# TrevorS/qwen3-tts-rs

Hardware: AMD Instinct MI355X
Metric: acoustic_frames_per_sec (higher is better)
Workload: dtype bf16

## Files before the change

include/q3tts.h:

```cpp
#ifndef Q3TTS_H
#define Q3TTS_H

#include <stddef.h>
#include <stdint.h>

#ifdef __cplusplus
extern "C" {
#endif

#define Q3_ABI_VERSION 1
#define Q3_MAX_BATCH 64

typedef enum q3_status {
    Q3_OK = 0,
    Q3_INVALID_ARG = 1,
    Q3_IO = 2,
    Q3_MISSING_WEIGHT = 3,
    Q3_KV_OVERFLOW = 4,
    Q3_HIP_ERROR = 5,
    Q3_RCCL_ERROR = 6,
    Q3_UNSUPPORTED = 7,
    Q3_OOM = 8
} q3_status;

// ... 141 lines not shown
q3_status q3_session_open_text(q3_session* s, int b);
q3_status q3_session_append_text(q3_session* s, int b, const uint32_t* ids, int n, int last);
q3_status q3_session_text_state(q3_session* s, int b, int* n_text, int* frames_committed, int* frames_runnable, int* closed,
                                int* frames_replayed);

enum {
    Q3_GET_PREFILL_EMBEDS = 0,
    Q3_GET_LAST_HIDDEN = 1,
    Q3_GET_LOGITS = 2,
    Q3_GET_TRAILING = 3,
    Q3_GET_PAD_EMBED = 4,
    Q3_GET_LOGITS_HIST = 5,
    Q3_GET_CP_LOGITS = 6,
    Q3_GET_TOKEN = 7,
    Q3_GET_CP_LOGITS_HIST = 8
};
q3_status q3_session_set_kv_dtype(q3_session* s, int dtype);
q3_status q3_session_set_debug(q3_session* s, int capture_logits);
q3_status q3_session_prefill_len(q3_session* s, int b, int* prefill_len, int* trailing_len);
q3_status q3_session_get(q3_session* s, int what, int b, void* out_host, size_t bytes);
q3_status q3_talker_step(q3_session* s, const float* embeds_host, float* hidden_host, float* logits_host);
q3_status q3_cp_generate(q3_session* s, const float* last_hidden_host, const float* sem_embed_host,
                         uint32_t* codes15_host, float* cp_logits_host );
q3_status q3_frame_embed(q3_model* m, uint32_t sem_token, const uint32_t* codes15, const float* text_add_host,
                         float* out_host);
q3_status q3_sample(int device, const float* logits_host, const uint8_t* seen_host, const float* u_host,
                    int rows, int vocab, const q3_options* opts, int token_count, uint32_t* tokens_host);
void      q3_rng_seed(uint64_t seed, uint64_t* state);
float     q3_rng_next(uint64_t* state);
q3_status q3_fused_residual_rmsnorm(int device, int dtype, const void* x_host, const void* res_host,
                                    const void* w_host, int rows, int cols, float eps,
                                    void* normed_host, void* sum_host);
q3_status q3_linear(int device, const float* x_host, const uint16_t* w_bf16_host, const float* bias_host,
                    int M, int N, int K, float* y_host);
typedef struct q3_linear_ex_args {
    int M, N, K, ldx, ldy, ldr, M_alloc;
    int epi, tiled, ksplit, use_ws, zero_n, zero_guard;
    float eps;
    const float* x; const uint16_t* w; const uint16_t* w2;
    const float* bias; const float* norm_w; const float* resid;
    float* y; float* zero_buf;
} q3_linear_ex_args;
q3_status q3_linear_ex(int device, const q3_linear_ex_args* args);
typedef struct q3_attn_step_args {
    int variant, B, nh, nkv, n_splits, max_seq;
    float eps; int reserved;
    const int* pos; const float* qkv; const float* q_norm_w; const float* k_norm_w;
    const float* rope_cos; const float* rope_sin;
    float* kcache; float* vcache; float* out;
} q3_attn_step_args;
q3_status q3_attn_step(int device, const q3_attn_step_args* args);
typedef struct q3_attn_step_ex_args {
    int variant, layout, B, nh, nkv, n_splits, max_seq, rows_per_seq;
    int n_layers, layer, n_slabs, kv_row_pages;
    int qkv_S, qkv_K, g_vocab, g_proj_dim, g_ldx, g_max_frames, g_code_slot, zero_n, zero_guard;
    float eps, qkv_eps; int reserved;
    const int* pos; const float* qkv; const float* q_norm_w; const float* k_norm_w;
    const float* rope_cos; const float* rope_sin;
    float* kcache; float* vcache; float* out;
    const int* page_slots; int* rot_used; long long* stray;
    const float* qkv_part; const float* qkv_ssq;
    const float* g_logits; const uint32_t* g_tok; const float* g_qkv_tab; const float* g_proj_tab;
    float* g_x; uint32_t* g_codes; const int* g_frame_idx;
    float* zero_buf;
} q3_attn_step_ex_args;
q3_status q3_attn_step_ex(int device, const q3_attn_step_ex_args* args);
q3_status q3_kv_pages_to_bf16_ex(int device, int n_layers, int nkv, int n_pages, const int* src_slots, const int* dst_slots,
                                 const float* src, uint16_t* dst, int* rot_used, long long* stray);
int         q3_conv_path(int cout, int cin, int L, int k, int dil, int phases, int packed, int has_resid, int planes, int aligned16);
int         q3_resunit_path(int C, int L, int dil, int packed, int ya_is_xa, int planes);
const char* q3_conv_path_name(int code);
typedef struct q3_conv_ex_args {
    int kind, cin, cout, L, k, dil, stride;
    int act, planes, packed, resid_in_place, snake_raw, y2_is_x;
    int y_front, y_elems;
    int* path;
    const float* x; const float* w; const float* b;
    const float* snake_a; const float* snake_b; const float* resid; const float* scale;
    const float* post_a; const float* post_ib;
    const float* w2; const float* b2; const float* mid_a; const float* mid_ib;
    float* y; float* y2;
} q3_conv_ex_args;
q3_status q3_conv_ex(int device, const q3_conv_ex_args* args);
int q3_gemm_path(int M, int N, int K, int epi, int norm, int w2, int planes, int* path);
typedef struct q3_gemm_ex_args {
    int M, N, K, ldx, ldy, ldr, M_alloc;
    int epi, geometry, k_split, sup_m, sup_n;
    float eps;
    int* path;
    const float* x; const uint16_t* w; const uint16_t* w2;
    const float* bias; const float* norm_w; const float* resid;
    float* y;
} q3_gemm_ex_args;
q3_status q3_gemm_ex(int device, const q3_gemm_ex_args* args);
int q3_attn_prefill_path(int nh, int nkv, int use_planes, int halves, int* path);
typedef struct q3_attn_prefill_ex_args {
    int n_seq, rps, base_pos, nh, nkv, max_seq, ld_qkv, ld_out;
    int kernel, halves, use_planes;
    float eps;
    int* path;
    const float* qkv; const float* q_norm_w; const float* k_norm_w;
    const float* rope_cos; const float* rope_sin;
    float* kcache; float* vcache; float* out;
} q3_attn_prefill_ex_args;
q3_status q3_attn_prefill_ex(int device, const q3_attn_prefill_ex_args* args);
int q3_attn_c_path(int hd, int kernel);
typedef struct q3_attn_c_ex_args {
    int mode, nh, hd, L, kernel, window;
    int N, n_rows, layers, layer, cap, n_blocks, n_tabs;
    float scale;
    const float* q; const float* k; const float* v;
    const int* rows; const float* caches;
    const int* tabs; const int* tab0; const int* tab_n;
    float* o;
} q3_attn_c_ex_args;
q3_status q3_attn_c_ex(int device, const q3_attn_c_ex_args* args);
q3_status q3_rope_c_ex(int device, float* q, float* k, const float* cs, const float* sn, const int* pos, int nh, int hd, int L, int n_pos);
q3_status q3_copy_cols_ex(int device, const float* src, size_t src_elems, float* dst, size_t dst_elems, int n, int C, const long long* s_off,
                          const long long* d_off, const int* sp, const int* dp, size_t src_off, size_t dst_off);
q3_status q3_copy_segs_ex(int device, const float* src, size_t src_elems, float* dst, size_t dst_elems, int n_segs, const unsigned long long* segs);
q3_status q3_gather_frames_ex(int device, const uint32_t* src, size_t src_elems, const long long* s_off, int n, uint32_t* dst, size_t dst_elems);
q3_status q3_rvq_embed_ex(int device, const uint32_t* frames, int n_frames, const float* first_cb, const float* rest_cbs, int cb_dim, int cb_size,
                          float* first_out, float* rest_out, int out_front, int out_elems);
q3_status q3_silu_mul_ex(int device, const float* g, const float* u, float* y, long long n, long long y_elems);
typedef struct q3_sample_rec {
    float inv_temp; int apply_temp, greedy;
    int top_k; float top_p; int use_top_p;
    float rep_pen, rep_inv; int use_rep;
    int eos_id, min_new_tokens, pad;
} q3_sample_rec;
q3_status q3_sample_row(const q3_options* opts, q3_sample_rec* out);
typedef struct q3_sample_ex_args {
    int B, vocab, ld, u_stride, u_elems, advance, token_count_static, hist_stride_b, hist_cap, codec_eos, use_suppress, guard;
    q3_sample_rec scalar;
    const float* logits; const float* u; const int* draw_idx; const q3_sample_rec* rows;
    const int* limit; const int* text_ready;
    uint32_t* tok; uint8_t* seen; int* token_count; int* frame_idx; int* pos; float* logits_hist;
} q3_sample_ex_args;
q3_status q3_sample_ex(int device, const q3_sample_ex_args* args);
typedef struct q3_frame_embed_ex_args {
    int B, H, n_sem, cp_vocab, max_frames, n_text_rows, guard, reserved;
    const uint16_t* codec_emb; const uint16_t* cp_embs; const uint32_t* tok; const float* cp_logits_last;
    const int* frame_idx; const float* text_rows; const int* trail_base; const int* trail_len; const int* pad_row; const int* text_ready;
    uint32_t* codes; float* out;
} q3_frame_embed_ex_args;
q3_status q3_frame_embed_ex(int device, const q3_frame_embed_ex_args* args);
typedef struct q3_cp_gather_ex_args {
    int pass, B, H, n_sem, cp_vocab, max_frames, proj_dim, qkv_dim, ld_out, ld_qkv_out, guard, reserved;
    const float* last_hidden; const uint16_t* codec_emb; const uint32_t* tok; const uint16_t* cp_emb; const float* cp_logits;
    const float* proj_tab; const float* qkv_tab; const int* frame_idx;
    uint32_t* codes; float* out; float* qkv_out;
} q3_cp_gather_ex_args;
q3_status q3_cp_gather_ex(int device, const q3_cp_gather_ex_args* args);
q3_status q3_rmsnorm_ex(int device, const float* x, long long x_elems, long long x_off, int ldx, const float* w, float* y, long long y_elems,
                        long long y_front, int ldy, int rows, int cols, float eps, const int* frame_idx, const int* text_ready);
q3_status q3_norm_c(int device, int layernorm, const float* x, const float* w, const float* b, int C, int L, float eps,
                    float* y, int y_front, int y_elems);
q3_status q3_dwconv7(int device, const float* x, const float* w, const float* b, int C, int L, float* y, int y_front, int y_elems);
q3_status q3_row_move(int device, void* src_host, size_t src_bytes, void* dst_host, size_t dst_bytes, int n_segs, const size_t* src_off,
                      const size_t* dst_off, const size_t* seg_bytes, const int* mode);
enum { Q3_DEC_QUANT = 0, Q3_DEC_PRECONV = 1, Q3_DEC_PRETRANS = 2, Q3_DEC_UP0 = 3, Q3_DEC_UP1 = 4,
       Q3_DEC_INIT = 5, Q3_DEC_BLK0 = 6, Q3_DEC_BLK1 = 7, Q3_DEC_BLK2 = 8, Q3_DEC_BLK3 = 9, Q3_DEC_N = 10 };
q3_status q3_decode_codes(q3_model* m, const uint32_t* frames_host, int n_frames, float* pcm_host,
                          float** taps_host);
typedef struct q3_codec_stream q3_codec_stream;
q3_status q3_codec_stream_create(q3_model* m, int rows, int max_frames, q3_codec_stream** out);
// ... 187 lines not shown
```

qwen3_tts_rs_amd/_lib.py:

```python
import ctypes
import os

from .config import CConfig

_HERE = os.path.dirname(os.path.abspath(__file__))
LIB_PATH = os.environ.get("Q3TTS_LIB") or os.path.join(_HERE, "libq3tts.so")

if not os.path.exists(LIB_PATH):
    raise ImportError(
        f"{LIB_PATH} not found: the gfx950 HIP library is not built. Run "
        "`python -c 'import __graft_entry__ as g; g.build()'` (or qwen3_tts_rs_amd/csrc/build.sh).")

lib = ctypes.CDLL(LIB_PATH)


class COptions(ctypes.Structure):
    _fields_ = [
        ("temperature", ctypes.c_double), ("top_p", ctypes.c_double), ("repetition_penalty", ctypes.c_double),
        ("seed", ctypes.c_uint64), ("max_length", ctypes.c_int32), ("top_k", ctypes.c_int32),
        ("eos_token_id", ctypes.c_int32), ("chunk_frames", ctypes.c_int32), ("min_new_tokens", ctypes.c_int32),
        ("has_seed", ctypes.c_int32),
    ]


# ... 170 lines not shown
    "q3_pcm_stage_tempo_lags": (c_int, [c_void_p, c_int, P(ctypes.c_int64), c_void_p, ctypes.c_size_t, P(ctypes.c_size_t)]),
    "q3_session_set_tempo": (c_int, [c_void_p, c_int, c_int]),
    "q3_batcher_ticket_tempo": (c_int, [c_void_p, ctypes.c_int64, c_int]),
    "q3_pcm_stage_set_pitch": (c_int, [c_void_p, c_int, c_int]),
    "q3_pcm_stage_pitch_plan": (c_int, [c_int, c_int, P(c_int), P(ctypes.c_double)]),
    "q3_pcm_stage_pitch_tables": (c_int, [c_void_p, ctypes.c_size_t, c_void_p, ctypes.c_size_t, P(c_int), P(c_int)]),
    "q3_pcm_stage_pitch_count": (c_int, [c_int, c_int, ctypes.c_size_t, c_int, P(ctypes.c_size_t)]),
    "q3_pcm_stage_bound_pitch": (c_int, [ctypes.c_uint32, c_int, c_int, c_int, ctypes.c_size_t, P(ctypes.c_size_t)]),
    "q3_session_set_pitch": (c_int, [c_void_p, c_int, c_int]),
    "q3_batcher_ticket_pitch": (c_int, [c_void_p, ctypes.c_int64, c_int]),
    "q3_pcm_stage_set_silence": (c_int, [c_void_p, c_int, c_int, c_int, c_int]),
    "q3_pcm_stage_silence": (c_int, [c_void_p, c_int] + [P(ctypes.c_int64)] * 5),
    "q3_pcm_stage_silence_hold": (c_int, [c_int, c_int, P(ctypes.c_size_t)]),
    "q3_pcm_stage_bound_silence": (c_int, [ctypes.c_uint32, c_int, c_int, c_int, c_int, c_int, ctypes.c_size_t, P(ctypes.c_size_t)]),
    "q3_silence_trim": (c_int, [c_void_p, ctypes.c_size_t, c_int, c_int, c_int, c_void_p, ctypes.c_size_t, P(ctypes.c_size_t), P(ctypes.c_int64)]),
    "q3_session_set_silence": (c_int, [c_void_p, c_int, c_int, c_int, c_int]),
    "q3_session_silence": (c_int, [c_void_p, c_int] + [P(ctypes.c_int64)] * 5),
    "q3_batcher_ticket_silence": (c_int, [c_void_p, ctypes.c_int64, c_int, c_int, c_int]),
    "q3_batcher_ticket_silence_read": (c_int, [c_void_p, ctypes.c_int64] + [P(ctypes.c_int64)] * 5),
    "q3_pcm_stage_set_level": (c_int, [c_void_p, c_int, c_int, c_int]),
    "q3_pcm_stage_level_coeffs": (c_int, [c_int, c_int, P(ctypes.c_float), P(ctypes.c_float)]),
    "q3_pcm_stage_level_count": (c_int, [ctypes.c_size_t, c_int, P(ctypes.c_size_t)]),
    "q3_pcm_stage_bound_level": (c_int, [ctypes.c_uint32, c_int, ctypes.c_size_t, P(ctypes.c_size_t)]),
    "q3_session_set_level": (c_int, [c_void_p, c_int, c_int, c_int]),
    "q3_batcher_ticket_level": (c_int, [c_void_p, ctypes.c_int64, c_int, c_int]),
    "q3_loudness_kweight": (c_int, [ctypes.c_uint32, P(ctypes.c_double), P(ctypes.c_double)]),
    "q3_pcm_stage_loudness_consts": (c_int, [c_int, c_int, P(ctypes.c_float), P(ctypes.c_float), P(ctypes.c_float), P(ctypes.c_float), P(ctypes.c_float)]),
    "q3_pcm_stage_set_loudness": (c_int, [c_void_p, c_int, c_int, c_int, c_int]),
    "q3_pcm_stage_loudness": (c_int, [c_void_p, c_int, P(ctypes.c_float), P(ctypes.c_float), P(c_int), P(c_int)]),
    "q3_pcm_stage_loudness_blocks": (c_int, [c_void_p, c_int, c_void_p, ctypes.c_size_t, P(ctypes.c_size_t)]),
    "q3_session_set_loudness": (c_int, [c_void_p, c_int, c_int, c_int, c_int]),
    "q3_session_loudness": (c_int, [c_void_p, c_int, P(ctypes.c_float), P(ctypes.c_float), P(c_int), P(c_int)]),
    "q3_batcher_ticket_loudness": (c_int, [c_void_p, ctypes.c_int64, c_int, c_int, c_int]),
    "q3_batcher_ticket_loudness_read": (c_int, [c_void_p, ctypes.c_int64, P(ctypes.c_float), P(ctypes.c_float), P(c_int), P(c_int)]),
    "q3_codec_stream_push_out": (c_int, [c_void_p, c_int, P(c_int), P(c_void_p), P(c_int), c_void_p, P(c_int), P(c_int), P(c_void_p),
                                         P(ctypes.c_size_t), P(ctypes.c_size_t)]),
    "q3_session_set_output": (c_int, [c_void_p, ctypes.c_uint32, c_int]),
    "q3_session_next_chunks_out": (c_int, [c_void_p, P(c_void_p), P(ctypes.c_size_t), P(ctypes.c_size_t), P(c_int)]),
    "q3_batcher_ticket_output": (c_int, [c_void_p, ctypes.c_int64, ctypes.c_uint32, c_int]),
    "q3_batcher_read_out": (c_int, [c_void_p, ctypes.c_int64, c_void_p, ctypes.c_size_t, P(ctypes.c_size_t), P(c_int)]),
    "q3_session_replace": (c_int, [c_void_p, c_int, c_void_p]),
    "q3_session_park_row": (c_int, [c_void_p, c_int, P(c_void_p)]),
    "q3_session_resume_row": (c_int, [c_void_p, c_int, c_void_p]),
    "q3_parked_free": (None, [c_void_p]),
    "q3_parked_info": (c_int, [c_void_p, P(c_int), P(c_int), P(c_int), P(c_int), P(ctypes.c_size_t)]),
    "q3_row_move": (c_int, [c_int, c_void_p, ctypes.c_size_t, c_void_p, ctypes.c_size_t, c_int, P(ctypes.c_size_t), P(ctypes.c_size_t),
                            P(ctypes.c_size_t), P(c_int)]),
    "q3_batcher_create": (c_int, [c_void_p, c_int, c_int, c_int, P(c_void_p)]),
    "q3_batcher_free": (None, [c_void_p]),
    "q3_batcher_submit": (c_int, [c_void_p, c_void_p, c_int, P(ctypes.c_int64)]),
    "q3_batcher_submit_streamed": (c_int, [c_void_p, c_void_p, P(ctypes.c_int64)]),
    "q3_batcher_read": (c_int, [c_void_p, ctypes.c_int64, c_void_p, ctypes.c_size_t, P(ctypes.c_size_t), P(c_int)]),
    "q3_batcher_stream_info": (c_int, [c_void_p, P(c_int), P(ctypes.c_size_t), P(c_int), P(c_int), P(c_int)]),
    "q3_batcher_submit_open": (c_int, [c_void_p, c_void_p, c_int, P(ctypes.c_int64)]),
    "q3_batcher_append_text": (c_int, [c_void_p, ctypes.c_int64, c_void_p, c_int, c_int]),
    "q3_batcher_text_state": (c_int, [c_void_p, ctypes.c_int64, P(c_int), P(c_int), P(c_int), P(c_int)]),
    "q3_batcher_cancel": (c_int, [c_void_p, ctypes.c_int64]),
    "q3_batcher_set_parking": (c_int, [c_void_p, c_int, c_int, c_int]),
    "q3_batcher_park": (c_int, [c_void_p, ctypes.c_int64]),
    "q3_batcher_unpark": (c_int, [c_void_p, ctypes.c_int64]),
    "q3_batcher_park_info": (c_int, [c_void_p, P(c_int), P(c_int), P(ctypes.c_longlong), P(ctypes.c_longlong), P(ctypes.c_longlong), P(c_int)]),
    "q3_batcher_step": (c_int, [c_void_p, c_int, c_int, P(c_int), P(c_int), P(c_int)]),
    "q3_batcher_poll": (c_int, [c_void_p, ctypes.c_int64, P(c_int), P(c_int), P(ctypes.c_size_t)]),
    "q3_batcher_fetch": (c_int, [c_void_p, ctypes.c_int64, c_void_p, c_int, c_void_p, ctypes.c_size_t]),
    "q3_session_set_debug": (c_int, [c_void_p, c_int]),
    "q3_session_prefill_len": (c_int, [c_void_p, c_int, P(c_int), P(c_int)]),
    "q3_session_get": (c_int, [c_void_p, c_int, c_int, c_void_p, ctypes.c_size_t]),
    "q3_talker_step": (c_int, [c_void_p, c_void_p, c_void_p, c_void_p]),
    "q3_cp_generate": (c_int, [c_void_p, c_void_p, c_void_p, c_void_p, c_void_p]),
    "q3_frame_embed": (c_int, [c_void_p, ctypes.c_uint32, c_void_p, c_void_p, c_void_p]),
    "q3_sample": (c_int, [c_int, c_void_p, c_void_p, c_void_p, c_int, c_int, P(COptions), c_int, c_void_p]),
    "q3_rng_seed": (None, [ctypes.c_uint64, P(ctypes.c_uint64)]),
    "q3_rng_next": (ctypes.c_float, [P(ctypes.c_uint64)]),
    "q3_fused_residual_rmsnorm": (c_int, [c_int, c_int, c_void_p, c_void_p, c_void_p, c_int, c_int, ctypes.c_float, c_void_p, c_void_p]),
    "q3_linear": (c_int, [c_int, c_void_p, c_void_p, c_void_p, c_int, c_int, c_int, c_void_p]),
    "q3_linear_ex": (c_int, [c_int, P(CLinearEx)]),
    "q3_attn_step": (c_int, [c_int, P(CAttnStep)]),
    "q3_attn_step_ex": (c_int, [c_int, P(CAttnStepEx)]),
    "q3_kv_pages_to_bf16_ex": (c_int, [c_int] * 4 + [c_void_p] * 6),
    "q3_conv_path": (c_int, [c_int] * 10),
    "q3_resunit_path": (c_int, [c_int] * 6),
    "q3_conv_path_name": (c_char_p, [c_int]),
    "q3_conv_ex": (c_int, [c_int, P(CConvEx)]),
    "q3_gemm_path": (c_int, [c_int] * 7 + [P(ctypes.c_int32)]),
    "q3_gemm_ex": (c_int, [c_int, P(CGemmEx)]),
    "q3_attn_prefill_path": (c_int, [c_int] * 4 + [P(ctypes.c_int32)]),
    "q3_attn_prefill_ex": (c_int, [c_int, P(CAttnPrefillEx)]),
    "q3_attn_c_path": (c_int, [c_int, c_int]),
    "q3_attn_c_ex": (c_int, [c_int, P(CAttnCEx)]),
    "q3_rope_c_ex": (c_int, [c_int, c_void_p, c_void_p, c_void_p, c_void_p, c_void_p, c_int, c_int, c_int, c_int]),
    "q3_copy_cols_ex": (c_int, [c_int, c_void_p, ctypes.c_size_t, c_void_p, ctypes.c_size_t, c_int, c_int, c_void_p, c_void_p, c_void_p, c_void_p,
                                ctypes.c_size_t, ctypes.c_size_t]),
    "q3_copy_segs_ex": (c_int, [c_int, c_void_p, ctypes.c_size_t, c_void_p, ctypes.c_size_t, c_int, c_void_p]),
    "q3_gather_frames_ex": (c_int, [c_int, c_void_p, ctypes.c_size_t, c_void_p, c_int, c_void_p, ctypes.c_size_t]),
    "q3_rvq_embed_ex": (c_int, [c_int, c_void_p, c_int, c_void_p, c_void_p, c_int, c_int, c_void_p, c_void_p, c_int, c_int]),
    "q3_silu_mul_ex": (c_int, [c_int, c_void_p, c_void_p, c_void_p, ctypes.c_longlong, ctypes.c_longlong]),
    "q3_sample_row": (c_int, [P(COptions), P(CSampleRow)]),
    "q3_sample_ex": (c_int, [c_int, P(CSampleEx)]),
    "q3_frame_embed_ex": (c_int, [c_int, P(CFrameEmbedEx)]),
    "q3_cp_gather_ex": (c_int, [c_int, P(CCpGatherEx)]),
    "q3_rmsnorm_ex": (c_int, [c_int, c_void_p, ctypes.c_longlong, ctypes.c_longlong, c_int, c_void_p, c_void_p, ctypes.c_longlong,
                              ctypes.c_longlong, c_int, c_int, c_int, ctypes.c_float, c_void_p, c_void_p]),
    "q3_norm_c": (c_int, [c_int, c_int, c_void_p, c_void_p, c_void_p, c_int, c_int, ctypes.c_float, c_void_p, c_int, c_int]),
    "q3_dwconv7": (c_int, [c_int, c_void_p, c_void_p, c_void_p, c_int, c_int, c_void_p, c_int, c_int]),
    "q3_decode_codes": (c_int, [c_void_p, c_void_p, c_int, c_void_p, P(c_void_p)]),
    "q3_codes_to_tensor": (None, [c_void_p, c_int, c_void_p]),
    "q3_session_set_profile": (c_int, [c_void_p, c_int]),
    "q3_session_profile_read": (c_int, [c_void_p, P(ctypes.c_double), P(ctypes.c_double), P(ctypes.c_long), c_int]),
    "q3_session_profile_shapes": (c_int, [c_void_p, P(c_int), c_int, P(c_int), c_int]),
    "q3_bench_linear": (c_int, [c_int] * 9 + [P(ctypes.c_double)]),
    "q3_session_stream": (c_int, [c_void_p, P(c_void_p)]),
    "q3_session_frame_bytes": (c_int, [c_void_p, c_int, P(ctypes.c_double), P(ctypes.c_double)]),
    "q3_session_submit_info": (c_int, [c_void_p, P(c_int), P(c_int)]),
    "q3_session_submit_fences": (c_int, [c_void_p, P(c_int), P(c_int)]),
    "q3_session_set_stream_mode": (c_int, [c_void_p, c_int]),
    "q3_session_open_text": (c_int, [c_void_p, c_int]),
    "q3_session_append_text": (c_int, [c_void_p, c_int, c_void_p, c_int, c_int]),
    "q3_session_text_state": (c_int, [c_void_p, c_int, P(c_int), P(c_int), P(c_int), P(c_int), P(c_int)]),
    "q3_model_config": (c_int, [c_void_p, P(CConfig)]),
    "q3_config_default": (c_int, [c_int, P(CConfig)]),
    "q3_config_from_json": (c_int, [c_char_p, P(CConfig), P(c_int)]),
    "q3_model_load": (c_int, [c_char_p, c_int, P(c_void_p), P(c_int)]),
    "q3_model_load_safetensors": (c_int, [c_void_p, c_char_p, P(c_int)]),
    "q3_safetensors_info": (c_int, [c_char_p, c_char_p, P(c_int), P(ctypes.c_int64), c_int, P(c_int)]),
    "q3_pcm16_from_f32": (c_int, [c_void_p, ctypes.c_int64, c_void_p]),
    "q3_wav_write_pcm16": (c_int, [c_char_p, c_void_p, ctypes.c_int64, ctypes.c_uint32]),
    "q3_g711_from_pcm16": (c_int, [c_void_p, ctypes.c_int64, c_int, c_void_p]),
    "q3_wav_write_g711": (c_int, [c_char_p, c_void_p, ctypes.c_int64, ctypes.c_uint32, c_int]),
    "q3_wav_read": (c_int, [c_char_p, c_void_p, ctypes.c_int64, P(ctypes.c_int64), P(ctypes.c_uint32)]),
    "q3_codes_write_bin": (c_int, [c_char_p, c_void_p, c_int, c_int]),
    "q3_codes_read_bin": (c_int, [c_char_p, c_void_p, c_int, c_int, P(c_int)]),
    "q3_audio_write_bin": (c_int, [c_char_p, c_void_p, ctypes.c_int64]),
    "q3_audio_read_bin": (c_int, [c_char_p, c_void_p, ctypes.c_int64, P(ctypes.c_int64)]),
    "q3_resample": (c_int, [c_void_p, ctypes.c_int64, ctypes.c_uint32, ctypes.c_uint32, c_void_p, ctypes.c_int64, P(ctypes.c_int64)]),
    "q3_dp_unique_id": (c_int, [c_void_p]),
    "q3_dp_init": (c_int, [c_int, c_int, c_void_p, c_int, P(c_void_p)]),
    "q3_dp_free": (None, [c_void_p]),
    "q3_dp_info": (c_int, [c_void_p, P(c_int), P(c_int)]),
    "q3_dp_broadcast_weights": (c_int, [c_void_p, c_void_p, c_int]),
    "q3_dp_allgather_f64": (c_int, [c_void_p, c_void_p, c_int, c_void_p]),
    "q3_spk_config_default": (c_int, [P(CSpkConfig)]),
    "q3_spk_config_from_json": (c_int, [c_char_p, P(CSpkConfig), P(c_int)]),
    "q3_spk_create": (c_int, [P(CSpkConfig), c_int, P(c_void_p)]),
    "q3_spk_free": (None, [c_void_p]),
    "q3_spk_get_config": (c_int, [c_void_p, P(CSpkConfig)]),
    "q3_spk_n_tensors": (c_int, [c_void_p]),
    "q3_spk_tensor_info": (c_int, [c_void_p, c_int, P(c_char_p), P(ctypes.c_int64)]),
    "q3_spk_set_tensor": (c_int, [c_void_p, c_char_p, c_void_p, c_int, ctypes.c_int64]),
    "q3_spk_finalize": (c_int, [c_void_p]),
    "q3_spk_load_safetensors": (c_int, [c_void_p, c_char_p]),
    "q3_spk_mel_frames": (c_int, [ctypes.c_int64]),
    "q3_spk_mel": (c_int, [c_void_p, c_void_p, ctypes.c_int64, c_void_p, ctypes.c_int64, P(c_int)]),
    "q3_spk_forward": (c_int, [c_void_p, c_void_p, c_int, c_void_p, P(c_void_p)]),
    "q3_spk_encode": (c_int, [c_void_p, c_void_p, ctypes.c_int64, ctypes.c_uint32, c_void_p]),
    "q3_mimi_config_default": (c_int, [P(CMimiConfig)]),
    "q3_mimi_create": (c_int, [P(CMimiConfig), c_int, P(c_void_p)]),
    "q3_mimi_free": (None, [c_void_p]),
    "q3_mimi_get_config": (c_int, [c_void_p, P(CMimiConfig)]),
    "q3_mimi_n_tensors": (c_int, [c_void_p]),
    "q3_mimi_tensor_info": (c_int, [c_void_p, c_int, P(c_char_p), P(ctypes.c_int64)]),
    "q3_mimi_set_tensor": (c_int, [c_void_p, c_char_p, c_void_p, c_int, ctypes.c_int64]),
    "q3_mimi_finalize": (c_int, [c_void_p]),
    "q3_mimi_load_safetensors": (c_int, [c_void_p, c_char_p]),
    "q3_mimi_frames": (c_int, [P(CMimiConfig), ctypes.c_int64]),
    "q3_mimi_encode": (c_int, [c_void_p, c_void_p, ctypes.c_int64, ctypes.c_uint32, c_void_p, c_int, P(c_int), P(c_void_p)]),
    "q3_wav_info": (c_int, [c_char_p, P(CWavDesc)]),
# ... 29 lines not shown
```

qwen3_tts_rs_amd/api.py:

```python
import ctypes
import enum
from dataclasses import dataclass
from typing import List, NamedTuple, Optional, Sequence, Tuple

import numpy as np

from . import _lib
from ._lib import lib, check, COptions, CRequest, CTiming
from .config import Q3Config
from . import synth

MAX_BATCH = 64
CODEC_EOS_TOKEN_ID = 2150
SAMPLES_PER_FRAME = 1920


class Language(enum.Enum):
    Chinese = 2055
    English = 2050
    Japanese = 2058
    Korean = 2064
    German = 2053
    French = 2061
    Russian = 2069
# ... 804 lines not shown
    def attach_speech_encoder(self, enc):
        self.speech_encoder = enc

    def has_speech_encoder(self) -> bool:
        return self.speech_encoder is not None

    def create_voice_clone_prompt(self, ref_audio: "AudioBuffer", ref_text_ids=None, ref_codes=None):
        from .speaker import VoiceClonePrompt
        if self.speaker_encoder is None:
            hint = {ModelType.CustomVoice: " CustomVoice models use preset speakers (synthesize_with_voice), not voice cloning. "
                                           "Use a Base model for voice cloning.",
                    ModelType.VoiceDesign: " VoiceDesign models use text-described voices, not voice cloning. "
                                           "Use a Base model for voice cloning."}.get(
                self.model_type, " Ensure model weights contain `speaker_encoder.*` keys (only Base models include a speaker encoder).")
            raise _lib.Q3Error(3, "Speaker encoder not available." + hint)
        if isinstance(ref_audio, RefAudio):
            emb = self.speaker_encoder.encode_ref(ref_audio)
            if ref_text_ids is None:
                return VoiceClonePrompt(emb)
            if ref_codes is None:
                if self.speech_encoder is None:
                    raise _lib.Q3Error(7, "ICL voice cloning requires a speech encoder, but it was not loaded. Ensure the speech tokenizer "
                                          "weights contain encoder keys, or use x_vector_only mode by passing ref_text=None.")
                ref_codes = self.speech_encoder.encode_ref(ref_audio)
            return VoiceClonePrompt(emb, np.ascontiguousarray(ref_codes, dtype=np.uint32), np.asarray(ref_text_ids, dtype=np.uint32))
        if ref_audio.sample_rate != 24000:
            ref_audio = resample_to_24k(ref_audio)
        emb = self.speaker_encoder.encode(ref_audio.samples, ref_audio.sample_rate)
        if ref_text_ids is None:
            return VoiceClonePrompt(emb)
        if ref_codes is None:
            if self.speech_encoder is None:
                raise _lib.Q3Error(7, "ICL voice cloning requires a speech encoder, but it was not loaded. Ensure the speech tokenizer "
                                      "weights contain encoder keys, or use x_vector_only mode by passing ref_text=None.")
            ref_codes = self.speech_encoder.encode(ref_audio.samples, ref_audio.sample_rate)
        return VoiceClonePrompt(emb, np.ascontiguousarray(ref_codes, dtype=np.uint32), np.asarray(ref_text_ids, dtype=np.uint32))

    def synthesize_voice_clone_prompt(self, text_ids, prompt, language: "Language", options=None):
        return self.synthesize_voice_clone(text_ids, prompt.speaker_embedding, language, options,
                                           ref_codes=prompt.ref_codes, ref_text_ids=prompt.ref_text_ids)

    def supports_preset_speakers(self) -> bool:
        return self.model_type in (None, ModelType.CustomVoice)

    def supports_voice_design(self) -> bool:
        return self.model_type == ModelType.VoiceDesign

    def close(self):
        if getattr(self, "_h", None):
            lib.q3_model_free(self._h); self._h = None

    __del__ = close

    def set_tensor(self, name: str, arr: np.ndarray, dtype: int):
        a = np.ascontiguousarray(arr)
        check(lib.q3_model_set_tensor(self._h, name.encode(), dtype, a.ctypes.data_as(ctypes.c_void_p), a.size))

    def finalize(self):
        check(lib.q3_model_finalize(self._h))

    @classmethod
    def from_synthetic(cls, config: Q3Config, device: int = 0, seed: int = synth.DEFAULT_SEED, sink=None) -> "Qwen3TTS":
        m = cls(config, device)
        for name, arr, dt in synth.synthetic_checkpoint(config, m._h, seed):
            m.set_tensor(name, arr, dt)
            if sink is not None:
                sink(name, arr, dt)
        m.finalize()
        return m

    @classmethod
    def from_tensors(cls, config: Q3Config, tensors, device: int = 0) -> "Qwen3TTS":
        m = cls(config, device)
        for name, (arr, dt) in tensors.items():
            m.set_tensor(name, arr, dt)
        m.finalize()
        return m

    def kv_pool_limit(self, max_pages: int):
        check(lib.q3_model_kv_pool_limit(self._h, int(max_pages)))

    def set_codec_planes(self, planes: int):
        check(lib.q3_model_set_codec_planes(self._h, int(planes)))

    def kv_pool_trim(self) -> int:
        n = ctypes.c_size_t()
        check(lib.q3_model_kv_pool_trim(self._h, ctypes.byref(n)))
        return n.value

    def kv_pool_info(self) -> dict:
        pp = ctypes.c_int(); pb = ctypes.c_size_t(); tot = ctypes.c_int(); use = ctypes.c_int(); peak = ctypes.c_int()
        check(lib.q3_model_kv_pool_info(self._h, ctypes.byref(pp), ctypes.byref(pb), ctypes.byref(tot), ctypes.byref(use), ctypes.byref(peak)))
        return {"page_positions": pp.value, "page_bytes": pb.value, "pages_total": tot.value, "pages_in_use": use.value, "pages_peak": peak.value}

    def prefix_cache(self, max_pages: int):
        check(lib.q3_model_prefix_cache(self._h, int(max_pages)))

    def prefix_cache_info(self) -> dict:
        mx = ctypes.c_int(); n = ctypes.c_int(); sh = ctypes.c_int()
        lk = ctypes.c_longlong(); hp = ctypes.c_longlong(); ev = ctypes.c_longlong()
        check(lib.q3_model_prefix_cache_info(self._h, ctypes.byref(mx), ctypes.byref(n), ctypes.byref(sh), ctypes.byref(lk), ctypes.byref(hp), ctypes.byref(ev)))
        return {"max_pages": mx.value, "pages_cached": n.value, "pages_shared": sh.value, "lookups": lk.value,
                "hit_positions": hp.value, "evictions": ev.value}

    def arena(self) -> Tuple[int, int]:
        p = ctypes.c_void_p(); n = ctypes.c_size_t()
        check(lib.q3_model_arena(self._h, ctypes.byref(p), ctypes.byref(n)))
        return p.value, n.value

    def mark_loaded(self):
        check(lib.q3_model_mark_loaded(self._h))

    def session(self, utts: Sequence[Utterance], options: Optional[SynthesisOptions] = None, debug: bool = False, kv_bf16: bool = False) -> Session:
        return Session(self, utts, options or SynthesisOptions(), debug, kv_bf16=kv_bf16)

    def synthesize(self, text_ids: Sequence[int], options: Optional[SynthesisOptions] = None) -> AudioBuffer:
        return self.synthesize_with_voice(text_ids, Speaker.Ryan, Language.English, options)

    def synthesize_with_voice(self, text_ids, speaker: Speaker, language: Language, options=None) -> AudioBuffer:
        audio, _ = self.synthesize_with_timing(text_ids, speaker, language, options)
        return audio

    def synthesize_with_timing(self, text_ids, speaker: Speaker, language: Language, options=None):
        s = self.session([Utterance(text_ids, speaker, language)], options)
        try:
            audio, timing = s.run()
        finally:
            s.close()
        return audio[0], timing

    def synthesize_voice_design(self, text_ids, instruct_ids, language: Language, options=None) -> AudioBuffer:
        s = self.session([Utterance(text_ids, language=language, instruct_ids=instruct_ids)], options)
        try:
            audio, _ = s.run()
        finally:
            s.close()
        return audio[0]

    def synthesize_voice_clone(self, text_ids, xvector, language: Language, options=None, ref_codes=None, ref_text_ids=None):
        s = self.session([Utterance(text_ids, language=language, xvector=xvector, ref_codes=ref_codes, ref_text_ids=ref_text_ids)], options)
        try:
            s.prefill(); s.generate(max(s._row_limit))
            return AudioBuffer(s.decode(0)), s.codes(0)
        finally:
            s.close()

    @staticmethod
    def prefill_shape(u: "Utterance") -> Tuple[int, int, int, int]:
        icl = u.ref_codes is not None and u.ref_text_ids is not None
        n_ins = len(u.instruct_ids) if u.instruct_ids is not None else 0
        n_icl = (len(np.asarray(u.ref_codes).reshape(-1, 16)) + 1) if icl else 0
        return (u.mode(), n_ins, 1 if (len(u.text_ids) > 0 and not icl) else 0, n_icl)

    def synthesize_batch(self, utts: Sequence[Utterance], options=None):
        audio: List[Optional[AudioBuffer]] = [None] * len(utts)
        tot = SynthesisTiming(0.0, 0.0, 0, 0.0)
        for k in range(0, len(utts), MAX_BATCH):
            part = list(range(k, min(k + MAX_BATCH, len(utts))))
            s = self.session([utts[i] for i in part], options)
            try:
                a, t = s.run()
            finally:
                s.close()
            for j, i in enumerate(part):
                audio[i] = a[j]
            tot = SynthesisTiming(tot.prefill_ms + t.prefill_ms, tot.generation_ms + t.generation_ms,
# ... 916 lines not shown
        rr = np.ascontiguousarray(rows, dtype=np.int32); assert rr.ndim == 2 and rr.shape[1] == 3
        cc = np.ascontiguousarray(caches, dtype=np.float32); assert cc.ndim == 5 and cc.shape[2] == 2 and cc.shape[3] == nh * hd
        a.N, a.n_rows, a.layers, a.cap = qq.shape[1], rr.shape[0], cc.shape[1], cc.shape[4]
        keep += [rr, cc]; a.rows, a.caches = _vp(rr), _vp(cc)
        if mode == 2:
            tt = np.ascontiguousarray(tabs, dtype=np.int32); t0 = np.ascontiguousarray(tab0, dtype=np.int32); tn = np.ascontiguousarray(tab_n, dtype=np.int32)
            assert tt.ndim == 1 and t0.shape == (rr.shape[0],) and tn.shape == t0.shape
            a.n_blocks, a.n_tabs = cc.shape[0], tt.size
            keep += [tt, t0, tn]; a.tabs, a.tab0, a.tab_n = _vp(tt), _vp(t0), _vp(tn)
        else:
            assert cc.shape[0] == rr.shape[0]
    check(lib.q3_attn_c_ex(device, ctypes.byref(a)))
    return o


def rope_c_ex(q_: np.ndarray, k: np.ndarray, cs: np.ndarray, sn: np.ndarray, nh: int, pos=None, device: int = 0):
    qq = np.array(q_, dtype=np.float32, order="C"); kk = np.array(k, dtype=np.float32, order="C")
    cs = np.ascontiguousarray(cs, dtype=np.float32); sn = np.ascontiguousarray(sn, dtype=np.float32)
    assert qq.ndim == 2 and kk.shape == qq.shape and qq.shape[0] % nh == 0 and cs.ndim == 2 and sn.shape == cs.shape
    hd = qq.shape[0] // nh; assert cs.shape[1] * 2 == hd
    pp = None if pos is None else np.ascontiguousarray(pos, dtype=np.int32)
    assert pp is None or pp.shape == (qq.shape[1],)
    check(lib.q3_rope_c_ex(device, _vp(qq), _vp(kk), _vp(cs), _vp(sn), _vp(pp), nh, hd, qq.shape[1], cs.shape[0]))
    return qq, kk


def copy_cols_ex(src: np.ndarray, dst: np.ndarray, C: int, s_off, d_off, sp, dp, src_off: int = 0, dst_off: int = 0, device: int = 0) -> np.ndarray:
    src = np.ascontiguousarray(src, dtype=np.float32)
    assert dst.dtype == np.float32 and dst.flags.c_contiguous and dst.ndim == 1 and src.ndim == 1
    so = np.ascontiguousarray(s_off, dtype=np.int64); do = np.ascontiguousarray(d_off, dtype=np.int64)
    spp = np.ascontiguousarray(sp, dtype=np.int32); dpp = np.ascontiguousarray(dp, dtype=np.int32)
    n = so.size; assert do.shape == (n,) and spp.shape == (n,) and dpp.shape == (n,)
    check(lib.q3_copy_cols_ex(device, _vp(src), src.size, _vp(dst), dst.size, n, C, _vp(so), _vp(do), _vp(spp), _vp(dpp), src_off, dst_off))
    return dst


def copy_segs_ex(src: np.ndarray, dst: np.ndarray, segs, device: int = 0) -> np.ndarray:
    src = np.ascontiguousarray(src, dtype=np.float32)
    assert dst.dtype == np.float32 and dst.flags.c_contiguous and dst.ndim == 1 and src.ndim == 1
    sg = np.ascontiguousarray(segs, dtype=np.uint64); assert sg.ndim == 2 and sg.shape[1] == 3
    check(lib.q3_copy_segs_ex(device, _vp(src), src.size, _vp(dst), dst.size, sg.shape[0], _vp(sg)))
    return dst


def gather_frames_ex(src: np.ndarray, s_off, dst: np.ndarray, device: int = 0) -> np.ndarray:
    src = np.ascontiguousarray(src, dtype=np.uint32)
    assert dst.dtype == np.uint32 and dst.flags.c_contiguous and dst.ndim == 1 and src.ndim == 1
    so = np.ascontiguousarray(s_off, dtype=np.int64); assert so.ndim == 1
    check(lib.q3_gather_frames_ex(device, _vp(src), src.size, _vp(so), so.size, _vp(dst), dst.size))
    return dst


def rvq_embed_ex(frames: np.ndarray, first_cb: np.ndarray, rest_cbs: np.ndarray, first_out: np.ndarray, rest_out: np.ndarray, out_front: int = 0,
                 device: int = 0):
    fr = np.ascontiguousarray(frames, dtype=np.uint32); assert fr.ndim == 2 and fr.shape[1] == 16
    fc = np.ascontiguousarray(first_cb, dtype=np.float32); rc = np.ascontiguousarray(rest_cbs, dtype=np.float32)
    assert fc.ndim == 2 and rc.shape == (15,) + fc.shape
    for buf in (first_out, rest_out):
        assert buf.dtype == np.float32 and buf.flags.c_contiguous and buf.ndim == 1 and buf.size == first_out.size
    check(lib.q3_rvq_embed_ex(device, _vp(fr), fr.shape[0], _vp(fc), _vp(rc), fc.shape[1], fc.shape[0], _vp(first_out), _vp(rest_out), out_front,
                              first_out.size))
    return first_out, rest_out


def silu_mul_ex(g: np.ndarray, u: np.ndarray, y: np.ndarray, device: int = 0) -> np.ndarray:
    g = np.ascontiguousarray(g, dtype=np.float32); u = np.ascontiguousarray(u, dtype=np.float32)
    assert g.ndim == 1 and u.shape == g.shape and y.dtype == np.float32 and y.flags.c_contiguous and y.ndim == 1
    check(lib.q3_silu_mul_ex(device, _vp(g), _vp(u), _vp(y), g.size, y.size))
    return y


def resunit_path(C: int, L: int, dil: int, packed: bool = True, ya_is_xa: bool = False, planes: int = 3) -> int:
    return lib.q3_resunit_path(C, L, dil, int(packed), int(ya_is_xa), planes)


def conv_path_name(code: int) -> str:
    return lib.q3_conv_path_name(code).decode()


def conv_ex(kind: int, x: np.ndarray, w: np.ndarray, *, dil: int = 1, stride: int = 1, b: Optional[np.ndarray] = None, snake=None,
            post=None, mid=None, resid: Optional[np.ndarray] = None, resid_in_place: bool = False, scale: Optional[np.ndarray] = None,
            act: int = 0, planes: int = 3, packed: bool = True, snake_raw: bool = False, w2: Optional[np.ndarray] = None,
            b2: Optional[np.ndarray] = None, y: Optional[np.ndarray] = None, y2: Optional[np.ndarray] = None, y_front: int = 0,
            y2_is_x: bool = False, device: int = 0):
    f = lambda a: np.ascontiguousarray(a, dtype=np.float32)
    x = f(x); w = f(w)
    assert x.ndim == 2 and w.ndim == 3
    cin, L = x.shape
    cout = w.shape[1] if kind == 1 else w.shape[0]
    assert (w.shape[0] if kind == 1 else w.shape[1]) == cin
    a = _lib.CConvEx()
    a.kind, a.cin, a.cout, a.L, a.k, a.dil, a.stride = kind, cin, cout, L, w.shape[2], dil, stride
    a.act, a.planes, a.packed, a.resid_in_place, a.snake_raw, a.y2_is_x = act, planes, int(packed), int(resid_in_place), int(snake_raw), int(y2_is_x)
    n_out = cout * L * (stride if kind == 1 else 1)
    if y is None:
        y = np.zeros(n_out, dtype=np.float32); y_front = 0
    for buf in (y, y2):
        assert buf is None or (buf.dtype == np.float32 and buf.flags.c_contiguous and buf.ndim == 1 and buf.size == y.size)
    a.y_front, a.y_elems = y_front, y.size
    path = ctypes.c_int32(0)
    a.path = ctypes.pointer(path)
    keep = [x, w]
    ptr = lambda arr: arr.ctypes.data_as(ctypes.c_void_p)
    a.x, a.w, a.y = ptr(x), ptr(w), ptr(y)
    if y2 is not None:
        a.y2 = ptr(y2)

    def opt(name, arr, n):
        if arr is not None:
            arr = f(arr); assert arr.size == n, (name, arr.size, n)
            keep.append(arr); setattr(a, name, ptr(arr))
    opt("b", b, cout); opt("b2", b2, cout); opt("scale", scale, cout); opt("resid", resid, n_out)
    if w2 is not None:
        opt("w2", w2, cout * cin)
    for (na, nb, pr, n) in (("snake_a", "snake_b", snake, cin), ("post_a", "post_ib", post, cout), ("mid_a", "mid_ib", mid, cout)):
        if pr is not None:
            opt(na, pr[0], n); opt(nb, pr[1], n)
    try:
        check(lib.q3_conv_ex(device, ctypes.byref(a)))
    except _lib.Q3Error as e:
        e.path = path.value
        raise
    return y, y2, path.value


def norm_c(x: np.ndarray, w: np.ndarray, b: Optional[np.ndarray] = None, eps: float = 1e-6, y: Optional[np.ndarray] = None,
           y_front: int = 0, device: int = 0) -> np.ndarray:
    x = np.ascontiguousarray(x, dtype=np.float32); C, L = x.shape
    w = np.ascontiguousarray(w, dtype=np.float32); assert w.shape == (C,)
    bb = None if b is None else np.ascontiguousarray(b, dtype=np.float32)
    if y is None:
        y = np.zeros(C * L, dtype=np.float32); y_front = 0
    assert y.dtype == np.float32 and y.flags.c_contiguous and y.ndim == 1
    ptr = lambda arr: arr.ctypes.data_as(ctypes.c_void_p)
    check(lib.q3_norm_c(device, 0 if bb is None else 1, ptr(x), ptr(w), None if bb is None else ptr(bb), C, L, eps, ptr(y), y_front, y.size))
    return y


def dwconv7(x: np.ndarray, w: np.ndarray, b: np.ndarray, y: Optional[np.ndarray] = None, y_front: int = 0, device: int = 0) -> np.ndarray:
    x = np.ascontiguousarray(x, dtype=np.float32); C, L = x.shape
    w = np.ascontiguousarray(w, dtype=np.float32); b = np.ascontiguousarray(b, dtype=np.float32)
    assert w.shape == (C, 7) and b.shape == (C,)
    if y is None:
        y = np.zeros(C * L, dtype=np.float32); y_front = 0
    assert y.dtype == np.float32 and y.flags.c_contiguous and y.ndim == 1
    ptr = lambda arr: arr.ctypes.data_as(ctypes.c_void_p)
    check(lib.q3_dwconv7(device, ptr(x), ptr(w), ptr(b), C, L, ptr(y), y_front, y.size))
    return y


def _io(arr, dtype, n, name):
    assert isinstance(arr, np.ndarray) and arr.dtype == dtype and arr.flags.c_contiguous and arr.ndim == 1 and arr.size == n, (name, n)
    return _vp(arr)


def sample_row(options: SynthesisOptions) -> "_lib.CSampleRow":
    r = _lib.CSampleRow(); o = options.to_c()
    check(lib.q3_sample_row(ctypes.byref(o), ctypes.byref(r)))
    return r


def sample_ex(logits: np.ndarray, u: np.ndarray, vocab: int, tok: np.ndarray, scalar, *, rows=None, seen: Optional[np.ndarray] = None,
              u_stride: int = 1, draw_idx=None, token_count: Optional[np.ndarray] = None, token_count_static: int = 0, advance: bool = False,
              frame_idx: Optional[np.ndarray] = None, pos: Optional[np.ndarray] = None, limit=None, text_ready=None,
              logits_hist: Optional[np.ndarray] = None, hist_stride_b: int = 0, hist_cap: int = 0, codec_eos: int = 2150,
              use_suppress: bool = True, guard: int = 0, device: int = 0) -> np.ndarray:
    lg = np.ascontiguousarray(logits, dtype=np.float32); assert lg.ndim == 2
    B, ld = lg.shape
    uu = np.ascontiguousarray(u, dtype=np.float32).reshape(-1)
    a = _lib.CSampleEx()
    a.B, a.vocab, a.ld, a.u_stride, a.u_elems, a.advance, a.token_count_static = B, vocab, ld, u_stride, uu.size, int(advance), token_count_static
    a.hist_stride_b, a.hist_cap, a.codec_eos, a.use_suppress, a.guard = hist_stride_b, hist_cap, codec_eos, int(use_suppress), guard
    a.scalar = scalar
    keep = [lg, uu]
    a.logits, a.u = _vp(lg), _vp(uu)
    a.tok = _io(tok, np.uint32, B + 2 * guard, "tok")
    if seen is not None:
        a.seen = _io(seen, np.uint8, B * vocab + 2 * guard, "seen")
    for name, arr in (("token_count", token_count), ("frame_idx", frame_idx), ("pos", pos)):
        if arr is not None:
            setattr(a, name, _io(arr, np.int32, B + 2 * guard, name))
    if logits_hist is not None:
        a.logits_hist = _io(logits_hist, np.float32, B * hist_stride_b + 2 * guard, "logits_hist")
    for name, arr in (("draw_idx", draw_idx), ("limit", limit), ("text_ready", text_ready)):
        if arr is not None:
            v = np.ascontiguousarray(arr, dtype=np.int32); assert v.shape == (B,), name
            keep.append(v); setattr(a, name, _vp(v))
    if rows is not None:
        assert len(rows) == B
        rr = (_lib.CSampleRow * B)(*rows); keep.append(rr)
        a.rows = ctypes.cast(rr, ctypes.c_void_p)
    check(lib.q3_sample_ex(device, ctypes.byref(a)))
    return tok


def frame_embed_ex(codec_emb: np.ndarray, cp_embs: np.ndarray, tok, cp_logits_last: np.ndarray, codes: np.ndarray, frame_idx, max_frames: int,
                   text_rows: np.ndarray, trail_base, trail_len, pad_row, out: np.ndarray, text_ready=None, guard: int = 0, device: int = 0):
    ce = np.ascontiguousarray(codec_emb, dtype=np.uint16); pe = np.ascontiguousarray(cp_embs, dtype=np.uint16)
    lg = np.ascontiguousarray(cp_logits_last, dtype=np.float32); tx = np.ascontiguousarray(text_rows, dtype=np.float32)
    assert ce.ndim == 2 and pe.ndim == 3 and pe.shape[0] == 15 and pe.shape[2] == ce.shape[1] and lg.ndim == 2 and lg.shape[1] == pe.shape[1]
    assert tx.ndim == 2 and tx.shape[1] == ce.shape[1]
    B, H = lg.shape[0], ce.shape[1]
# ... 98 lines not shown
```

qwen3_tts_rs_amd/csrc/q3_codec_run.hip:

```cpp
#include "q3_engine.h"

namespace {
struct DevCache {
    std::mutex mu;
    std::unordered_multimap<uint64_t, void*> free_blocks;
    std::unordered_map<void*, uint64_t> live;
    size_t cached = 0, cap = 0;
    DevCache() { const char* e = getenv("Q3_DEV_CACHE_MB"); cap = (size_t)(e ? atol(e) : 32768) << 20; }
    static uint64_t key(int dev, size_t bytes) { return ((uint64_t)dev << 48) | (uint64_t)bytes; }
    static size_t size_class(size_t bytes) {
        if (bytes <= 4096) return (bytes + 255) & ~(size_t)255;
        size_t p2 = 1; while ((p2 << 1) <= bytes) p2 <<= 1;
        const size_t step = p2 >> 4;
        return (bytes + step - 1) / step * step;
    }
    hipError_t get(void** p, size_t bytes) {
        bytes = size_class(bytes);
        int dev = 0; (void)hipGetDevice(&dev);
        const uint64_t k = key(dev, bytes);
        {
            std::lock_guard<std::mutex> g(mu);
            auto it = free_blocks.find(k);
            if (it != free_blocks.end()) { *p = it->second; free_blocks.erase(it); cached -= bytes; live[*p] = k; return hipSuccess; }
        }
        hipError_t e = hipMalloc(p, bytes);
        if (e != hipSuccess) {
            trim(0);
            e = hipMalloc(p, bytes);
            if (e != hipSuccess) return e;
        }
        std::lock_guard<std::mutex> g(mu);
        live[*p] = k;
        return hipSuccess;
    }
    void put(void* p) {
        if (!p) return;
        uint64_t k = 0; bool known = false;
        {
            std::lock_guard<std::mutex> g(mu);
            auto it = live.find(p);
            if (it != live.end()) { k = it->second; known = true; live.erase(it); }
            const size_t bytes = (size_t)(k & 0xffffffffffffull);
            if (known && cap && cached + bytes <= cap) { free_blocks.emplace(k, p); cached += bytes; return; }
        }
        (void)hipFree(p);
    }
    void trim(size_t keep) {
        std::vector<void*> drop;
        {
            std::lock_guard<std::mutex> g(mu);
            for (auto it = free_blocks.begin(); it != free_blocks.end() && cached > keep;) {
                cached -= (size_t)(it->first & 0xffffffffffffull); drop.push_back(it->second); it = free_blocks.erase(it);
            }
        }
        for (void* p : drop) (void)hipFree(p);
    }
};
DevCache& dev_cache() { static DevCache* c = new DevCache(); return *c; }
}
hipError_t dev_malloc(void** p, size_t bytes) { return dev_cache().get(p, bytes ? bytes : 4); }
void dev_free(void* p) { dev_cache().put(p); }

q3_status codec_reserve(const q3_model* m, CodecWS& ws, int T, int Tf) {
    if (Tf < T) Tf = T;
    if (T <= ws.cap_frames && Tf <= ws.cap_front) return Q3_OK;
    if (T < ws.cap_frames) T = ws.cap_frames;
    if (Tf < ws.cap_front) Tf = ws.cap_front;
    if (ws.bufA) HIPC(q3_hipDeviceSynchronize());
    ws.release();
    const q3_config& c = m->cfg;
    int up = 1; for (int i = 0; i < 2; ++i) up *= c.dec_up_ratios[i];
    size_t per = (size_t)4 * c.dec_latent * up;
    { size_t L = up; int C = c.dec_dim; per = per > (size_t)C * L ? per : (size_t)C * L;
      for (int b = 0; b < 4; ++b) { L *= c.dec_up_rates[b]; C /= 2; if ((size_t)C * L > per) per = (size_t)C * L; } }
    const int QDm = c.dec_heads * c.dec_head_dim;
    size_t per_front = (size_t)4 * QDm;
    if ((size_t)2 * c.dec_inter > per_front) per_front = (size_t)2 * c.dec_inter;
    if ((size_t)2 * c.dec_cb_dim > per_front) per_front = (size_t)2 * c.dec_cb_dim;
    if ((size_t)c.dec_latent > per_front) per_front = (size_t)c.dec_latent;
    if ((size_t)c.dec_q_dim > per_front) per_front = (size_t)c.dec_q_dim;
    size_t n = per * (size_t)T;
    if (per_front * (size_t)Tf > n) n = per_front * (size_t)Tf;
    HIPC(dev_malloc((void**)&ws.bufA, n * 4)); HIPC(dev_malloc((void**)&ws.bufB, n * 4)); HIPC(dev_malloc((void**)&ws.bufC, n * 4));
    HIPC(dev_malloc((void**)&ws.bufF, n * 4));
    const size_t small = (size_t)Tf * (size_t)(QDm > c.dec_latent ? QDm : c.dec_latent);
    HIPC(dev_malloc((void**)&ws.bufD, small * 4)); HIPC(dev_malloc((void**)&ws.bufE, small * 4));
    HIPC(dev_malloc((void**)&ws.cs, (size_t)Tf * 32 * 4)); HIPC(dev_malloc((void**)&ws.sn, (size_t)Tf * 32 * 4));
    HIPC(dev_malloc((void**)&ws.frames, (size_t)Tf * 16 * 4));
    size_t total_up = up; for (int b = 0; b < 4; ++b) total_up *= c.dec_up_rates[b];
    HIPC(dev_malloc((void**)&ws.pcm, (size_t)T * total_up * 4));
    Q3C(codec_rope_table(c, Tf, ws.cs, ws.sn));
    ws.cap_frames = T; ws.cap_front = Tf;
    return Q3_OK;
}
q3_status codec_rope_table(const q3_config& c, int n, float* cs_dev, float* sn_dev) {
    std::vector<float> cs((size_t)n * 32), sn((size_t)n * 32);
    for (int i = 0; i < 32; ++i) {
        const float inv = 1.0f / powf(c.dec_theta, (float)(2 * i) / (float)c.dec_head_dim);
        for (int t = 0; t < n; ++t) { const float f = (float)t * inv; cs[(size_t)t * 32 + i] = cosf(f); sn[(size_t)t * 32 + i] = sinf(f); }
    }
    HIPC(q3_hipMemcpy(cs_dev, cs.data(), cs.size() * 4, hipMemcpyHostToDevice));
    HIPC(q3_hipMemcpy(sn_dev, sn.data(), sn.size() * 4, hipMemcpyHostToDevice));
    return Q3_OK;
}

int samples_per_frame(const q3_config& c) {
    int u = 1; for (int i = 0; i < 2; ++i) u *= c.dec_up_ratios[i]; for (int i = 0; i < 4; ++i) u *= c.dec_up_rates[i];
    return u;
}

static thread_local const q3_model* tl_codec_model = nullptr;
static const void* packed_of(const float* w) { return tl_codec_model ? tl_codec_model->pk(w) : nullptr; }
static thread_local int tl_codec_planes = 3;
CodecScope::CodecScope(const q3_model* m) {
    static const int env_planes = [] { const char* e = getenv("Q3_CODEC_PLANES"); const int v = e ? atoi(e) : 0; return (v == 2 || v == 3) ? v : 0; }();
    planes = env_planes ? env_planes : m->codec_planes;
    tl_codec_model = m; tl_codec_planes = planes;
}
CodecScope::~CodecScope() { tl_codec_planes = 3; }
static hipError_t conv1(const float* x, const float* w, const float* b, float* y, int cin, int cout, int L, hipStream_t st,
                        const float* resid = nullptr, const float* scale = nullptr, int act = 0,
                        const float* sa = nullptr, const float* sib = nullptr) {
    ConvArgs a; a.x = x; a.w = w; a.b = b; a.y = y; a.cin = cin; a.cout = cout; a.L = L; a.k = 1; a.dil = 1;
    a.resid = resid; a.scale = scale; a.act = act; a.snake_a = sa; a.snake_b = sib; a.wpk = packed_of(w); a.planes = tl_codec_planes;
    return launch_conv1d(a, st);
}
static hipError_t convk(const float* x, const float* w, const float* b, float* y, int cin, int cout, int L, int k, int dil,
                        hipStream_t st, const float* sa = nullptr, const float* sib = nullptr, int act = 0) {
    ConvArgs a; a.x = x; a.w = w; a.b = b; a.y = y; a.cin = cin; a.cout = cout; a.L = L; a.k = k; a.dil = dil;
    a.snake_a = sa; a.snake_b = sib; a.act = act; a.wpk = packed_of(w); a.planes = tl_codec_planes;
    return launch_conv1d(a, st);
}

static q3_status tap_out(float** taps, int id, const float* dev, size_t n, hipStream_t st) {
    if (taps && taps[id]) { HIPC(hipStreamSynchronize(st)); HIPC(q3_hipMemcpy(taps[id], dev, n * 4, hipMemcpyDeviceToHost)); }
    return Q3_OK;
}
q3_status codec_front_quant(const q3_model* m, CodecWS& ws, int T, hipStream_t st) {
    const q3_config& c = m->cfg;
    const int CD = c.dec_cb_dim, Q = c.dec_q_dim;
    float *A = ws.bufA, *B = ws.bufB;
    float* e1 = A; float* e2 = A + (size_t)CD * T;
    HIPC(launch_rvq_embed(ws.frames, T, m->first_cb, m->rest_cbs_dev, e1, e2, CD, c.dec_cb_size, st));
    HIPC(conv1(e1, m->first_proj, nullptr, B, CD, Q, T, st));
    HIPC(conv1(e2, m->rest_proj, nullptr, B, CD, Q, T, st, B));
    return Q3_OK;
}
q3_status codec_front_preconv(const q3_model* m, const float* x, float* y, int L, hipStream_t st) {
    HIPC(convk(x, m->pre_w, m->pre_b, y, m->cfg.dec_q_dim, m->cfg.dec_latent, L, 3, 1, st));
    return Q3_OK;
}
q3_status codec_front_transformer(const q3_model* m, CodecWS& ws, int T, hipStream_t st, const CodecAttnFn& rope_attn) {
    const q3_config& c = m->cfg;
    const int LAT = c.dec_latent, DH = c.dec_hidden, QD = c.dec_heads * c.dec_head_dim, DI = c.dec_inter;
    float *A = ws.bufA, *B = ws.bufB, *C = ws.bufC, *D = ws.bufD, *E = ws.bufE;
    float* Hd = D;
    HIPC(conv1(C, m->inp_w, m->inp_b, Hd, LAT, DH, T, st));
    float* Nn = E;
    float* q = A; float* k = A + (size_t)QD * T; float* v = A + (size_t)2 * QD * T; float* ao = A + (size_t)3 * QD * T;
    float* g = B; float* u = B + (size_t)DI * T;
    for (int l = 0; l < c.dec_layers; ++l) {
        const DecLayerW& L = m->dl[l];
        HIPC(launch_rmsnorm_c(Hd, L.in_ln, Nn, DH, T, c.dec_eps, st));
        auto adjacent = [&](const float* w0, const float* w1, int cout, int cin) {
            const char* p0 = (const char*)m->pk(w0); const char* p1 = (const char*)m->pk(w1);
            return p0 && p1 && p1 == p0 + packed_conv_w_bytes(cout, cin, 1) && w1 == w0 + (size_t)cout * cin &&
                   cout % 32 == 0 && cin % 16 == 0;
        };
        static const bool no_fuse_qkv = getenv("Q3_CODEC_NO_QKV_FUSE") != nullptr || getenv("Q3_CONV_F32") != nullptr ||
                                        getenv("Q3_CONV_VALU") != nullptr;
        if (!no_fuse_qkv && adjacent(L.q, L.k, QD, DH) && adjacent(L.k, L.v, QD, DH)) {
            HIPC(conv1(Nn, L.q, nullptr, q, DH, 3 * QD, T, st));
        } else {
            HIPC(conv1(Nn, L.q, nullptr, q, DH, QD, T, st));
            HIPC(conv1(Nn, L.k, nullptr, k, DH, QD, T, st));
            HIPC(conv1(Nn, L.v, nullptr, v, DH, QD, T, st));
        }
        Q3C(rope_attn(l, q, k, v, ao));
        HIPC(conv1(ao, L.o, nullptr, Hd, QD, DH, T, st, Hd, L.attn_scale));
        HIPC(launch_rmsnorm_c(Hd, L.post_ln, Nn, DH, T, c.dec_eps, st));
        if (!no_fuse_qkv && adjacent(L.gate, L.up, DI, DH)) {
            HIPC(conv1(Nn, L.gate, nullptr, g, DH, 2 * DI, T, st));
        } else {
            HIPC(conv1(Nn, L.gate, nullptr, g, DH, DI, T, st));
            HIPC(conv1(Nn, L.up, nullptr, u, DH, DI, T, st));
        }
        HIPC(launch_silu_mul(g, u, g, (int64_t)DI * T, st));
        HIPC(conv1(g, L.down, nullptr, Hd, DI, DH, T, st, Hd, L.mlp_scale));
    }
    HIPC(launch_rmsnorm_c(Hd, m->dec_norm, Nn, DH, T, c.dec_eps, st));
    HIPC(conv1(Nn, m->outp_w, m->outp_b, C, DH, LAT, T, st));
    return Q3_OK;
}
q3_status codec_stack_dev(const q3_model* m, CodecWS& ws, float* cur, int L, hipStream_t st, float** taps, const CodecScope& scope) {
    const int NPL = scope.planes;
    const q3_config& c = m->cfg;
    const int LAT = c.dec_latent;
    auto TAP = [&](int id, const float* dev, size_t n) -> q3_status { return tap_out(taps, id, dev, n, st); };
    float *A = ws.bufA, *B = ws.bufB, *C = ws.bufC;
    for (int i = 0; i < 2; ++i) {
        const UpW& U = m->up[i];
        float* upo = (cur == C) ? A : C;
        HIPC(launch_transconv1d_taps(cur, U.tw, U.tb, upo, LAT, LAT, L, U.ratio, 1, nullptr, nullptr, st, nullptr, nullptr, nullptr, m->pk(U.tw), NPL));
        L *= U.ratio;
        float* dw = (upo == A) ? C : A;
        HIPC(launch_dwconv7(upo, U.dww, U.dwb, dw, LAT, L, st));
        float* ln = dw + (size_t)LAT * L;
        HIPC(launch_layernorm_c(dw, U.nw, U.nb, ln, LAT, L, 1e-6f, st));
        HIPC(conv1(ln, U.p1w, U.p1b, B, LAT, 4 * LAT, L, st, nullptr, nullptr, 1));
        HIPC(conv1(B, U.p2w, U.p2b, upo, 4 * LAT, LAT, L, st, upo, U.gamma));
        cur = upo;
        Q3C(TAP(Q3_DEC_UP0 + i, cur, (size_t)LAT * L));
    }
    int Cc = c.dec_dim;
    float* pool4[4] = {A, B, C, ws.bufF};
    auto other = [&](std::initializer_list<const float*> used) -> float* {
        for (float* p : pool4) { bool u = false; for (const float* q : used) if (q == p) u = true; if (!u) return p; }
        return nullptr;
    };
    float* xact = other({cur});
    {
        ConvArgs a; a.x = cur; a.w = m->init_w; a.wpk = m->pk(m->init_w); a.b = m->init_b; a.cin = LAT; a.cout = Cc; a.L = L; a.k = 7; a.dil = 1; a.planes = NPL;
        a.post_a = m->blk[0].a; a.post_ib = m->blk[0].ib;
        if (taps && taps[Q3_DEC_INIT]) { float* raw = other({cur, xact}); a.y = raw; a.y2 = xact; HIPC(launch_conv1d(a, st)); Q3C(TAP(Q3_DEC_INIT, raw, (size_t)Cc * L)); }
        else { a.y = xact; HIPC(launch_conv1d(a, st)); }
    }
    static const int dils[3] = {1, 3, 9};
    for (int b = 0; b < 4; ++b) {
        const DecBlockW& Bk = m->blk[b];
        float* Y = other({xact});
        float* YA = other({xact, Y});
        HIPC(launch_transconv1d_taps(xact, Bk.tw, Bk.tb, Y, Bk.cin, Bk.cout, L, Bk.rate, 2, nullptr, nullptr, st, Bk.res[0].a1, Bk.res[0].ib1, YA, m->pk(Bk.tw), NPL));
        L *= Bk.rate; Cc = Bk.cout;
        float* T2 = other({Y, YA});
        for (int uu = 0; uu < 3; ++uu) {
            const ResUnitW& R = Bk.res[uu];
            const float* nxt_a = uu < 2 ? Bk.res[uu + 1].a1 : (b < 3 ? m->blk[b + 1].a : m->fin_a);
            const float* nxt_ib = uu < 2 ? Bk.res[uu + 1].ib1 : (b < 3 ? m->blk[b + 1].ib : m->fin_ib);
            {
                ResUnitArgs r{};
                r.xa = YA; r.y = Y; r.ya = T2; r.w1pk = m->pk(R.c1w); r.w2pk = m->pk(R.c2w); r.b1 = R.c1b; r.b2 = R.c2b;
                r.mid_a = R.a2; r.mid_ib = R.ib2; r.post_a = nxt_a; r.post_ib = nxt_ib; r.C = Cc; r.L = L; r.dil = dils[uu]; r.planes = NPL;
                const hipError_t e = launch_resunit(r, st);
                if (e == hipSuccess) { float* t = YA; YA = T2; T2 = t; continue; }
                if (e != hipErrorNotSupported) HIPC(e);
            }
            {
                ConvArgs a; a.x = YA; a.w = R.c1w; a.wpk = m->pk(R.c1w); a.b = R.c1b; a.y = T2; a.cin = Cc; a.cout = Cc; a.L = L; a.k = 7; a.dil = dils[uu]; a.planes = NPL;
                a.post_a = R.a2; a.post_ib = R.ib2;
                HIPC(launch_conv1d(a, st));
            }
            {
                ConvArgs a; a.x = T2; a.w = R.c2w; a.wpk = m->pk(R.c2w); a.b = R.c2b; a.y = Y; a.y2 = YA; a.cin = Cc; a.cout = Cc; a.L = L; a.k = 1; a.dil = 1; a.resid = Y; a.planes = NPL;
                if (uu < 2) { a.post_a = Bk.res[uu + 1].a1; a.post_ib = Bk.res[uu + 1].ib1; }
                else if (b < 3) { a.post_a = m->blk[b + 1].a; a.post_ib = m->blk[b + 1].ib; }
                else { a.post_a = m->fin_a; a.post_ib = m->fin_ib; }
                HIPC(launch_conv1d(a, st));
            }
        }
        Q3C(TAP(Q3_DEC_BLK0 + b, Y, (size_t)Cc * L));
        xact = YA;
    }
    HIPC(convk(xact, m->fin_w, m->fin_b, ws.pcm, Cc, 1, L, 7, 1, st, nullptr, nullptr, 2));
    return Q3_OK;
}

q3_status codec_decode_dev(const q3_model* m, CodecWS& ws, int T, hipStream_t st, float** taps, int c0) {
    const q3_config& c = m->cfg;
    const CodecScope scope(m);
    const int Q = c.dec_q_dim, LAT = c.dec_latent;
    float *B = ws.bufB, *C = ws.bufC;
    Q3C(codec_front_quant(m, ws, T, st));
    Q3C(tap_out(taps, Q3_DEC_QUANT, B, (size_t)Q * T, st));
    Q3C(codec_front_preconv(m, B, C, T, st));
    Q3C(tap_out(taps, Q3_DEC_PRECONV, C, (size_t)LAT * T, st));
    const float scale = (float)pow((double)c.dec_head_dim, -0.5);
    Q3C(codec_front_transformer(m, ws, T, st, [&](int, float* q, float* k, float* v, float* ao) -> q3_status {
        HIPC(launch_rope_c(q, k, ws.cs, ws.sn, c.dec_heads, c.dec_head_dim, T, st));
        HIPC(launch_attn_c(q, k, v, ao, c.dec_heads, c.dec_head_dim, T, scale, st));
        return Q3_OK;
    }));
    Q3C(tap_out(taps, Q3_DEC_PRETRANS, C, (size_t)LAT * T, st));
    float* cur = C;
    int L = T;
    if (c0 > 0) {
        HIPC(launch_copy_rows(C + c0, T, ws.bufF, T - c0, LAT, T - c0, st));
        cur = ws.bufF; L = T - c0;
    }
    return codec_stack_dev(m, ws, cur, L, st, taps, scope);
}

extern "C" q3_status q3_decode_codes(q3_model* m, const uint32_t* frames_host, int n_frames, float* pcm_host, float** taps_host) {
    if (!m || !m->finalized) return set_err(Q3_INVALID_ARG, "model not finalized");
    if (n_frames < 0 || (n_frames > 0 && (!frames_host || !pcm_host))) return set_err(Q3_INVALID_ARG, "q3_decode_codes: bad argument");
    if (n_frames == 0) return Q3_OK;
    for (int f = 0; f < n_frames; ++f)
        for (int g = 1; g < 16; ++g)
            if (frames_host[(size_t)f * 16 + g] >= (uint32_t)m->cfg.dec_cb_size)
                return set_err(Q3_INVALID_ARG, "code %u out of range for codebook %d (frame %d)", frames_host[(size_t)f * 16 + g], g, f);
    HIPC(hipSetDevice(m->device));
    CodecWS ws;
    q3_status st = codec_reserve(m, ws, n_frames);
    if (st == Q3_OK) {
        hipError_t e = q3_hipMemcpy(ws.frames, frames_host, (size_t)n_frames * 16 * 4, hipMemcpyHostToDevice);
        if (e != hipSuccess) st = set_err(Q3_HIP_ERROR, "hipMemcpy frames: %s", hipGetErrorString(e));
    }
    if (st == Q3_OK) st = codec_decode_dev(m, ws, n_frames, 0, taps_host);
    if (st == Q3_OK) {
        hipError_t e = q3_hipDeviceSynchronize();
        if (e == hipSuccess) e = q3_hipMemcpy(pcm_host, ws.pcm, (size_t)n_frames * samples_per_frame(m->cfg) * 4, hipMemcpyDeviceToHost);
        if (e != hipSuccess) st = set_err(Q3_HIP_ERROR, "decode: %s", hipGetErrorString(e));
    }
    ws.release();
    return st;
}
```

qwen3_tts_rs_amd/csrc/q3_codec_stream.hip:

```cpp
#include "q3_engine.h"

struct CsRow { int pos = 0; float* kv = nullptr; float* lat = nullptr; float* hist = nullptr; std::vector<float*> blocks; };
struct q3_codec_stream {
    q3_model* m = nullptr; int R = 0, cap = 0;
    int bf = 0, max_blocks = 0;
    std::vector<float*> free_blocks; int blocks_total = 0, blocks_in_use = 0, blocks_peak = 0;
    hipStream_t st = nullptr; bool owns_stream = false;
    std::vector<CsRow> rows;
    CodecWS ws;
    float *cs = nullptr, *sn = nullptr;
    char* desc = nullptr; size_t desc_cap = 0;
    float* stage = nullptr; float* stage_host = nullptr; size_t stage_cap = 0;
};

static size_t kv_floats(const q3_codec_stream* cs) {
    const q3_config& c = cs->m->cfg;
    return (size_t)c.dec_layers * 2 * c.dec_heads * c.dec_head_dim * cs->cap;
}

static size_t block_floats(const q3_codec_stream* cs) {
    const q3_config& c = cs->m->cfg;
    return ((size_t)c.dec_layers * 2 * c.dec_heads * c.dec_head_dim + c.dec_latent) * cs->bf;
}

// ... 200 lines not shown
        cs->stage_cap = 0;
        HIPC(dev_malloc((void**)&cs->stage, (size_t)W * spf * 4));
        HIPC(hipHostMalloc((void**)&cs->stage_host, (size_t)W * spf * 4, hipHostMallocDefault));
        cs->stage_cap = (size_t)W * spf;
    }
    std::vector<PsSeg> psegs; std::vector<const CsPush*> pseg_of; std::vector<void*> pouts; PsPlan plan;
    if (ps) {
        for (int i = 0; i < nP; ++i)
            if (P[i].ps) { psegs.push_back({P[i].ps_row, cs->stage + (size_t)out0[i] * spf, (size_t)(P[i].n - P[i].skip) * spf, P[i].last}); pseg_of.push_back(&P[i]); }
        for (const CsPush* f : flush) { psegs.push_back({f->ps_row, nullptr, 0, 1}); pseg_of.push_back(f); }
        for (const CsPush* p : pseg_of) pouts.push_back(p->out_host);
        Q3C(pcm_stage_begin(ps, psegs, plan));
    }
    float *A = ws.bufA, *B = ws.bufB, *C = ws.bufC, *F = ws.bufF;
    float* knew = A + (size_t)QD * N;
    std::vector<int> pos(N);
    std::vector<AttnCsRow> arows(nP);
    std::vector<ColCopy> xin(Np), hist(2 * nP), compact(N), kvsc(N), latsc(N), latg(Lc), solog;
    std::vector<SegCopy> segs;
    std::vector<AttnCbRow> brows(bf ? nP : 0);
    std::vector<const float*> tabs;
    auto kv_col = [&](const CsRow& r, int f) { return bf ? r.blocks[f / bf] + f % bf : r.kv + f; };
    auto lat_col = [&](const CsRow& r, int f) { return bf ? r.blocks[f / bf] + lat_off + f % bf : r.lat + f; };
    std::vector<const uint32_t*> fsrc(on_dev ? N : 0);
    std::vector<uint32_t> fhost(on_dev ? 0 : (size_t)N * 16);
    for (int i = 0; i < nP; ++i) {
        const CsRow& r = cs->rows[P[i].row];
        const int f0 = r.pos, n = P[i].n, x0 = col0[i] + 2 * i;
        arows[i] = {r.kv, f0, f0 + n, col0[i]};
        if (bf) { brows[i] = {(int)tabs.size(), f0, f0 + n, col0[i]}; tabs.insert(tabs.end(), r.blocks.begin(), r.blocks.end()); }
        for (int h = 0; h < 2; ++h) xin[x0 + h] = {f0 - 2 + h >= 0 ? r.hist + h : nullptr, A + x0 + h, 2, Np};
        for (int h = 0; h < 2; ++h) hist[2 * i + h] = {A + x0 + n + h, r.hist + h, Np, 2};
        for (int j = 0; j < n; ++j) {
            const int col = col0[i] + j;
            pos[col] = f0 + j;
            xin[x0 + 2 + j] = {B + col, A + x0 + 2 + j, N, Np};
            compact[col] = {B + x0 + 2 + j, C + col, Np, N};
            kvsc[col] = {knew + col, kv_col(r, f0 + j), N, kp};
            latsc[col] = {C + col, lat_col(r, f0 + j), N, kp};
            if (on_dev) fsrc[col] = P[i].dev + (size_t)j * 16;
            else memcpy(&fhost[(size_t)col * 16], P[i].host + (size_t)j * 16, 64);
        }
    }
    {
        int l0 = 0;
        for (int i : conc) {
            const CsRow& r = cs->rows[P[i].row];
            const int a0 = r.pos + P[i].skip, c0 = a0 - CODEC_CTX_FRAMES, len = P[i].n - P[i].skip + CODEC_CTX_FRAMES;
            for (int j = 0; j < len; ++j) latg[l0 + j] = {lat_col(r, c0 + j), F + l0 + j, kp, Lc};
            segs.push_back({(unsigned long long)(l0 + CODEC_CTX_FRAMES) * spf, (unsigned long long)out0[i] * spf, (unsigned long long)(P[i].n - P[i].skip) * spf});
            l0 += len;
        }
        for (int i : solo) {
            const CsRow& r = cs->rows[P[i].row];
            const int e = r.pos + P[i].n;
            if (bf) for (int f = 0; f < e; ++f) solog.push_back({lat_col(r, f), F + f, kp, e});
            segs.push_back({(unsigned long long)(cs->rows[P[i].row].pos + P[i].skip) * spf, (unsigned long long)out0[i] * spf,
                            (unsigned long long)(P[i].n - P[i].skip) * spf});
        }
    }
    DescBlock db;
    const size_t o_pos = db.add(pos), o_arows = db.add(arows), o_xin = db.add(xin), o_hist = db.add(hist), o_compact = db.add(compact),
                 o_kvsc = db.add(kvsc), o_latsc = db.add(latsc), o_latg = db.add(latg), o_segs = db.add(segs), o_fsrc = db.add(fsrc),
                 o_brows = db.add(brows), o_tabs = db.add(tabs), o_solog = db.add(solog), o_ps = db.add(plan.desc);
    if (db.host.size() > cs->desc_cap) {
        HIPC(hipStreamSynchronize(st));
        dev_free(cs->desc); cs->desc = nullptr; cs->desc_cap = 0;
        HIPC(dev_malloc((void**)&cs->desc, db.host.size() * 2));
        cs->desc_cap = db.host.size() * 2;
    }
    struct Failed {
        q3_codec_stream* cs; const std::vector<CsPush>& P; bool armed = true;
        ~Failed() {
            if (!armed) return;
            (void)hipStreamSynchronize(cs->st);
            for (const CsPush& p : P) codec_stream_reset(cs, p.row);
        }
    } failed{cs, P};
    HIPC(q3_hipMemcpy(cs->desc, db.host.data(), db.host.size(), hipMemcpyHostToDevice));
    auto D = [&](size_t off) { return (const void*)(cs->desc + off); };
    if (on_dev) HIPC(launch_gather_frames((const uint32_t* const*)D(o_fsrc), ws.frames, N, st));
    else HIPC(q3_hipMemcpy(ws.frames, fhost.data(), fhost.size() * 4, hipMemcpyHostToDevice));

    const CodecScope scope(m);
    Q3C(codec_front_quant(m, ws, N, st));
    HIPC(launch_copy_cols((const ColCopy*)D(o_xin), Np, Q, 0, 0, st));
    HIPC(launch_copy_cols((const ColCopy*)D(o_hist), 2 * nP, Q, 0, 0, st));
    Q3C(codec_front_preconv(m, A, B, Np, st));
    HIPC(launch_copy_cols((const ColCopy*)D(o_compact), N, LAT, 0, 0, st));
    const float scale = (float)pow((double)c.dec_head_dim, -0.5);
    Q3C(codec_front_transformer(m, ws, N, st, [&](int l, float* q, float* k, float*, float* ao) -> q3_status {
        const size_t layer_off = (size_t)l * 2 * QD * kp;
        HIPC(launch_rope_c_pos(q, k, cs->cs, cs->sn, (const int*)D(o_pos), c.dec_heads, c.dec_head_dim, N, st));
        HIPC(launch_copy_cols((const ColCopy*)D(o_kvsc), N, 2 * QD, 0, layer_off, st));
        if (bf) HIPC(launch_attn_cb(q, ao, (const AttnCbRow*)D(o_brows), (const float* const*)D(o_tabs), nP, max_tiles, layer_off, c.dec_heads, c.dec_head_dim, N, bf, scale, st));
        else HIPC(launch_attn_cs(q, ao, (const AttnCsRow*)D(o_arows), nP, max_tiles, layer_off, c.dec_heads, c.dec_head_dim, N, cap, scale, st));
        return Q3_OK;
    }));
    HIPC(launch_copy_cols((const ColCopy*)D(o_latsc), N, LAT, 0, 0, st));
    const SegCopy* dsegs = (const SegCopy*)D(o_segs);
    if (!conc.empty()) {
        size_t max_n = 0; for (int i : conc) max_n = std::max(max_n, (size_t)(P[i].n - P[i].skip) * spf);
        HIPC(launch_copy_cols((const ColCopy*)D(o_latg), Lc, LAT, 0, 0, st));
        Q3C(codec_stack_dev(m, ws, F, Lc, st, nullptr, scope));
        HIPC(launch_copy_segs(ws.pcm, cs->stage, dsegs, (int)conc.size(), max_n, st));
    }
    for (size_t k = 0, g0 = 0; k < solo.size(); ++k) {
        const int i = solo[k]; const CsRow& r = cs->rows[P[i].row];
        const int e = r.pos + P[i].n;
        if (bf) { HIPC(launch_copy_cols((const ColCopy*)D(o_solog) + g0, e, LAT, 0, 0, st)); g0 += (size_t)e; }
        else HIPC(launch_copy_rows(r.lat, cap, F, e, LAT, e, st));
        Q3C(codec_stack_dev(m, ws, F, e, st, nullptr, scope));
        HIPC(launch_copy_segs(ws.pcm, cs->stage, dsegs + conc.size() + k, 1, (size_t)(P[i].n - P[i].skip) * spf, st));
    }
    bool raw = false;
    for (int i = 0; i < nP; ++i) raw = raw || !P[i].ps;
    if (W > 0 && raw) HIPC(hipMemcpyAsync(cs->stage_host, cs->stage, (size_t)W * spf * 4, hipMemcpyDeviceToHost, st));
    if (ps) Q3C(pcm_stage_run(ps, psegs, plan, (const PsDesc*)D(o_ps), st));
    HIPC(hipStreamSynchronize(st));
    if (ps) pcm_stage_finish(ps, psegs, plan, pouts.data(), nullptr);
    for (size_t k = 0; k < psegs.size(); ++k) if (pseg_of[k]->n_out) *pseg_of[k]->n_out = plan.count[k];
    for (int i = 0; i < nP; ++i) {
        if (P[i].pcm_host && !P[i].ps) memcpy(P[i].pcm_host, cs->stage_host + (size_t)out0[i] * spf, (size_t)(P[i].n - P[i].skip) * spf * 4);
        cs->rows[P[i].row].pos += P[i].n;
    }
    failed.armed = false; untake.armed = false;
    cs->blocks_peak = std::max(cs->blocks_peak, cs->blocks_in_use);
    return Q3_OK;
}

extern "C" q3_status q3_codec_stream_push(q3_codec_stream* cs, int n_rows, const int* rows, const uint32_t* const* frames_host,
                                          const int* n_frames, float* const* pcm_host, const size_t* cap) {
    if (!cs) return set_err(Q3_INVALID_ARG, "q3_codec_stream_push: null stream");
    if (n_rows < 0 || (n_rows > 0 && (!rows || !frames_host || !n_frames || !pcm_host || !cap)))
        return set_err(Q3_INVALID_ARG, "q3_codec_stream_push: null argument");
    const int spf = samples_per_frame(cs->m->cfg);
    std::vector<char> seen(cs->R, 0);
    std::vector<CsPush> P;
    for (int i = 0; i < n_rows; ++i) {
        const int r = rows[i], n = n_frames[i];
        if (r < 0 || r >= cs->R) return set_err(Q3_INVALID_ARG, "q3_codec_stream_push: row %d out of range (%d rows)", r, cs->R);
        if (seen[r]) return set_err(Q3_INVALID_ARG, "q3_codec_stream_push: row %d listed twice", r);
        seen[r] = 1;
        if (n < 0) return set_err(Q3_INVALID_ARG, "q3_codec_stream_push: negative frame count for row %d", r);
        if (n == 0) continue;
        if (cs->rows[r].pos + n > cs->cap)
            return set_err(Q3_INVALID_ARG, "q3_codec_stream_push: row %d would reach %d frames, the stream holds %d", r, cs->rows[r].pos + n, cs->cap);
        if (!frames_host[i] || !pcm_host[i]) return set_err(Q3_INVALID_ARG, "q3_codec_stream_push: null frames or pcm pointer for row %d", r);
        if (cap[i] < (size_t)n * spf) return set_err(Q3_INVALID_ARG, "q3_codec_stream_push: pcm buffer of row %d too small (%zu < %zu samples)", r, cap[i], (size_t)n * spf);
        for (int f = 0; f < n; ++f)
            for (int g = 1; g < 16; ++g)
                if (frames_host[i][(size_t)f * 16 + g] >= (uint32_t)cs->m->cfg.dec_cb_size)
                    return set_err(Q3_INVALID_ARG, "code %u out of range for codebook %d (row %d, frame %d)", frames_host[i][(size_t)f * 16 + g], g, r, f);
        P.push_back({r, n, 0, frames_host[i], nullptr, pcm_host[i]});
    }
    return codec_stream_push(cs, P);
}

extern "C" q3_status q3_codec_stream_push_out(q3_codec_stream* cs, int n_rows, const int* rows, const uint32_t* const* frames_host, const int* n_frames,
                                              q3_pcm_stage* ps, const int* ps_rows, const int* last,
                                              void* const* out_host, const size_t* cap_samples, size_t* n_samples) {
    if (!cs) return set_err(Q3_INVALID_ARG, "q3_codec_stream_push_out: null stream");
    if (!ps) return set_err(Q3_INVALID_ARG, "q3_codec_stream_push_out: null stage");
    if (n_rows < 0 || (n_rows > 0 && (!rows || !frames_host || !n_frames || !ps_rows || !out_host || !cap_samples || !n_samples)))
        return set_err(Q3_INVALID_ARG, "q3_codec_stream_push_out: null argument");
    Q3C(pcm_stage_check_rows(ps, "q3_codec_stream_push_out", n_rows, ps_rows));
    const int spf = samples_per_frame(cs->m->cfg);
// ... 40 lines not shown
```

qwen3_tts_rs_amd/csrc/q3_engine.h:

```cpp
#pragma once
#include "../../include/q3tts.h"
#include "q3_kernels.h"

#include <math.h>
#include <stdarg.h>
#include <stdio.h>
#include <string.h>

#include <algorithm>
#include <atomic>
#include <chrono>
#include <functional>
#include <memory>
#include <string>
#include <thread>
#include <mutex>
#include <unordered_map>
#include <vector>

#include "q3_internal.h"
#include "q3_aql.h"

using namespace q3;
#define Q3_HIDDEN __attribute__((visibility("hidden")))
// ... 268 lines not shown
enum { PARK_MAX_SEGS = 24, PARK_PAYLOAD_INTS = 8 };
constexpr size_t PARK_DESC_BYTES = (size_t)PARK_MAX_SEGS * 32 + (size_t)PARK_PAYLOAD_INTS * 16;
struct ProfShape { int M, N, K, epi, rms, produce, tiled, count; };

struct q3_session {
    q3_model* m = nullptr; int B = 0;
    hipStream_t stream = nullptr; bool owns_stream = true;
    DevPool pool;
    std::vector<SeqInfo> seq;
    q3_options opts{};
    int max_frames = 0, max_seq = 0, prefill_len = 0, n_splits = 1;
    int* limit = nullptr;
    SampleRow* sample_rows = nullptr;
    int row_cap = 0, repl_base = 0;
    LmBuf tb{}, cb{};
    float *LASTH = nullptr, *LOGITS = nullptr, *CP_IN = nullptr, *CP_LOGITS = nullptr;
    float* wide_ws = nullptr; size_t wide_ws_bytes = 0;
    float *kcache = nullptr, *vcache = nullptr, *ckcache = nullptr, *cvcache = nullptr;
    size_t kv_layer_stride = 0, ckv_layer_stride = 0;
    bool paged = false; unsigned long long* kv_table = nullptr; std::vector<std::vector<float*>> kv_rows;
    std::vector<BatReq> ragged;
    bool regrouped = false;
    bool prefix_common = false;
    int kv_overflow_row = -1;
    bool kv_bf16 = false, kv_in_bf16 = false; unsigned long long* kv_conv = nullptr;
    float *rows = nullptr, *embeds = nullptr, *xvec = nullptr; int n_rows_total = 0;
    uint32_t* ids_dev = nullptr; int *tr_dev = nullptr, *ci_dev = nullptr; float *proj_e = nullptr, *proj_h = nullptr;
    uint32_t* ref_codes_dev = nullptr;
    int *trail_base = nullptr, *trail_len = nullptr, *pad_row = nullptr;
    int* text_ready = nullptr;
    uint32_t* app_ids = nullptr; float *app_e = nullptr, *app_h = nullptr, *app_out = nullptr;
    int* flush_buf = nullptr; size_t flush_cap = 0;
    uint32_t* tok = nullptr; uint8_t* seen = nullptr; int *frame_idx = nullptr, *pos = nullptr, *token_count = nullptr;
    float* U = nullptr; uint32_t* codes = nullptr;
    float* logits_hist = nullptr; float* cp_logits_hist = nullptr; bool debug = false;
    bool prefilled = false; int frames_run = 0;
    uint64_t uid = 0; char* park_desc = nullptr; std::shared_ptr<ParkShelf> shelf;
    hipGraphExec_t graph_exec = nullptr; hipGraph_t graph = nullptr;
    q3::AqlProgram* aql = nullptr; int aql_mode = 0; bool aql_tried = false, aql_failed = false;
    bool precapture = false;
    CodecWS cws;
    q3_codec_stream* cstream = nullptr;
    q3_pcm_stage* ostage = nullptr; uint32_t out_rate = 24000; int out_fmt = Q3_PCM_F32; bool out_started = false;
    std::vector<int> out_tempo;
    std::vector<int> out_level;
    std::vector<int> out_pitch;
    std::vector<int> out_loud;
    std::vector<int> out_sil;
    hipStream_t dec_stream = nullptr; hipEvent_t dec_ev = nullptr;
    std::vector<CodecWS> par_ws; std::vector<hipStream_t> par_streams;
    CodecWS seg_ws;
    std::vector<uint32_t> codes_host; bool codes_host_valid = false;
    int stream_pos = 0;
    int stream_mode = 0;
    bool profile = false; ProfAcc prof_linear;
    bool legacy_attn = getenv("Q3_LEGACY_ATTN") != nullptr;
    bool proj_tables = getenv("Q3_NO_PROJ_TABLES") == nullptr;
    bool qkv_tables = getenv("Q3_NO_QKV_TABLES") == nullptr;
    bool ksplit = getenv("Q3_NO_KSPLIT") == nullptr;
    bool cp_attn = getenv("Q3_NO_CP_ATTN") == nullptr;
    bool no_chunk = getenv("Q3_NO_CHUNK") != nullptr;
    std::vector<std::pair<hipEvent_t, hipEvent_t>> prof_events; std::vector<double> prof_event_bytes;
    std::vector<hipEvent_t> prof_pool; size_t prof_pool_next = 0;
    std::vector<ProfShape> prof_shapes;
#ifdef Q3_TRACE
    unsigned long long* trace_buf = nullptr; int trace_node = 0, trace_cap = 0;
    struct TraceMeta { int kind, a, b, c, d, e, f; };
    std::vector<TraceMeta> trace_meta;
    unsigned long long* trace_next(int kind, int a, int b, int c, int d = 0, int e = 0, int f = 0) {
        if (!trace_buf || trace_node >= trace_cap) return nullptr;
        trace_meta.push_back({kind, a, b, c, d, e, f});
        return trace_buf + (size_t)(trace_node++) * TRACE_NODE;
    }
#endif
    ~q3_session();
};


Q3_HIDDEN void model_destroy(q3_model* m);
Q3_HIDDEN void retile_bf16(const uint16_t* src, int N, int K, uint16_t* dst, int mode);
Q3_HIDDEN q3_status codec_reserve(const q3_model* m, CodecWS& ws, int T, int Tf = 0);
Q3_HIDDEN int samples_per_frame(const q3_config& c);
Q3_HIDDEN q3_status codec_decode_dev(const q3_model* m, CodecWS& ws, int T, hipStream_t st, float** taps, int c0 = 0);
struct Q3_HIDDEN CodecScope { int planes; explicit CodecScope(const q3_model* m); ~CodecScope(); CodecScope(const CodecScope&) = delete; };
using CodecAttnFn = std::function<q3_status(int layer, float* q, float* k, float* v, float* ao)>;
Q3_HIDDEN q3_status codec_rope_table(const q3_config& c, int n, float* cs_dev, float* sn_dev);
Q3_HIDDEN q3_status codec_front_quant(const q3_model* m, CodecWS& ws, int T, hipStream_t st);
Q3_HIDDEN q3_status codec_front_preconv(const q3_model* m, const float* x, float* y, int L, hipStream_t st);
Q3_HIDDEN q3_status codec_front_transformer(const q3_model* m, CodecWS& ws, int T, hipStream_t st, const CodecAttnFn& rope_attn);
Q3_HIDDEN q3_status codec_stack_dev(const q3_model* m, CodecWS& ws, float* cur, int L, hipStream_t st, float** taps, const CodecScope& scope);
struct CsPush {
    int row; int n; int skip; const uint32_t* host; const uint32_t* dev; float* pcm_host;
    q3_pcm_stage* ps = nullptr; int ps_row = -1; int last = 0; void* out_host = nullptr; size_t* n_out = nullptr;
};
Q3_HIDDEN q3_status codec_stream_create(q3_model* m, int rows, int max_frames, hipStream_t st, q3_codec_stream** out, int block_frames = 0,
                                        int max_blocks = 0);
Q3_HIDDEN q3_status codec_stream_push(q3_codec_stream* cs, const std::vector<CsPush>& pushes);
Q3_HIDDEN int codec_stream_pos(const q3_codec_stream* cs, int row);
Q3_HIDDEN void codec_stream_blocks(const q3_codec_stream* cs, int row, int upto, int* held, int* need);
Q3_HIDDEN void codec_stream_reset(q3_codec_stream* cs, int row);
struct PsSeg { int row; const float* dev; size_t n; int last; };
struct PsDesc {
    const float* src; const float* tail_in; float* tail_out; const float* taps; void* out;
    long long base, i0;
    int n_new, n_out, L, M, fmt, pad;
};
struct PsPlan { std::vector<PsDesc> desc; std::vector<size_t> off, count; size_t bytes = 0; bool late = false; };
Q3_HIDDEN void resampler_taps(int L, int M, std::vector<float>& out);
Q3_HIDDEN int pcm_stage_rows(const q3_pcm_stage* ps);
Q3_HIDDEN size_t pcm_stage_sample_bytes(const q3_pcm_stage* ps, int row);
Q3_HIDDEN void pcm_stage_reset(q3_pcm_stage* ps, int row);
Q3_HIDDEN q3_status pcm_stage_pitch_checked(const char* who, int tempo_permille, int cents);
Q3_HIDDEN q3_status pcm_stage_loud_checked(const char* who, int mode, int target_mB, int prior_mB);
Q3_HIDDEN q3_status pcm_stage_check_rows(const q3_pcm_stage* ps, const char* who, int n_rows, const int* rows);
Q3_HIDDEN size_t pcm_stage_count(const q3_pcm_stage* ps, int row, size_t n, int last);
Q3_HIDDEN q3_status pcm_stage_silence_checked(const char* who, int threshold_mB, int edge_ms, int pause_ms);
Q3_HIDDEN q3_status pcm_stage_begin(q3_pcm_stage* ps, const std::vector<PsSeg>& segs, PsPlan& plan);
Q3_HIDDEN q3_status pcm_stage_run(q3_pcm_stage* ps, const std::vector<PsSeg>& segs, PsPlan& plan, const PsDesc* desc_dev, hipStream_t st);
Q3_HIDDEN void pcm_stage_finish(q3_pcm_stage* ps, const std::vector<PsSeg>& segs, const PsPlan& plan, void* const* out_host, size_t* n_samples);
Q3_HIDDEN q3_status pcm_stage_push_dev(q3_pcm_stage* ps, const std::vector<PsSeg>& segs, hipStream_t st, void* const* out_host, size_t* n_samples);
Q3_HIDDEN hipError_t sync_frames(q3_session* s);
Q3_HIDDEN q3_status kv_reserve_row(q3_session* s, int b, int n_pos);
Q3_HIDDEN q3_status kv_reserve_frames(q3_session* s, int frames);
Q3_HIDDEN void kv_release_row(q3_session* s, int b);
Q3_HIDDEN LmDims talker_dims(const q3_config& c);
Q3_HIDDEN LmDims cp_dims(const q3_config& c);
Q3_HIDDEN q3_status talker_step(q3_session* s, const int* pos_dev, int pos_static, bool with_head, int rows_per_seq = 1,
                                const int* text_ready = nullptr);
Q3_HIDDEN SampleRow sample_row(const q3_options& o);
Q3_HIDDEN void request_shape(const q3_request& r, int* prefill_len, int* limit);
Q3_HIDDEN long row_worst_units(int prefill_len, int limit, bool bf16);
Q3_HIDDEN q3_request idle_request(int chunk_frames);
Q3_HIDDEN q3_status session_create(q3_model* m, const q3_request* reqs, int batch, int frame_budget, int prompt_budget, q3_session** out,
                                   hipStream_t borrow = nullptr);
Q3_HIDDEN q3_status lm_layer(q3_session* s, const LmDims& d, const LayerW& w, LmBuf& b, float* kc, float* vc, int max_seq,
                             const int* pos_dev, int pos_static, int n_splits, int rows_per_seq = 1, bool skip_qkv = false,
                             const CpGatherArgs* fold = nullptr, int paged_layer = -1);
struct TextPiece { int b; const uint32_t* ids; int n; bool last; };
Q3_HIDDEN q3_status session_text_enable(q3_session* s);
Q3_HIDDEN q3_status session_append_many(q3_session* s, const std::vector<TextPiece>& pieces);
Q3_HIDDEN int session_row_remaining(const q3_session* s, int b);
Q3_HIDDEN int session_row_committed(const q3_session* s, int b);
Q3_HIDDEN q3_status session_refresh_codes(q3_session* s);
enum { ROW_MOVE_COPY = 0, ROW_MOVE_EXCHANGE = 1 };
struct RowSeg { void* src; void* dst; unsigned long long bytes; int mode; int pad; };
Q3_HIDDEN hipError_t launch_row_move(const RowSeg* segs_dev, int n_segs, size_t max_bytes, hipStream_t st);
Q3_HIDDEN int parked_frames(const q3_parked* p, const uint32_t** codes);
Q3_HIDDEN int parked_committed(const q3_parked* p);
Q3_HIDDEN int parked_pages(const q3_parked* p);
Q3_HIDDEN bool parked_done(const q3_parked* p);
Q3_HIDDEN const SeqInfo& parked_seq(const q3_parked* p);
Q3_HIDDEN q3_status transplant_row(q3_session* s, int b, q3_session* side, int j, int limit);
Q3_HIDDEN q3_status transplant_check(q3_session* s, q3_session* side, int j, int limit_req, int* limit_out);
```

qwen3_tts_rs_amd/csrc/q3_kernels.h:

```cpp
#pragma once
#include <hip/hip_runtime.h>
#include <stdint.h>

namespace q3 {

constexpr int HEAD_DIM = 128;
constexpr int MAX_SPLITS = 64;
constexpr int PART_STRIDE = HEAD_DIM + 2;
constexpr int KV_PAGE_POS = 128, KV_PAGE_SHIFT = 7, KV_MAX_PAGES = 64;

#ifdef Q3_TRACE
constexpr int TRACE_SLOTS = 8, TRACE_WGS = 512, TRACE_DWGS = 16, TRACE_WAVES = 16;
constexpr int TRACE_NODE = TRACE_SLOTS * (TRACE_WGS + TRACE_DWGS * TRACE_WAVES);
#define Q3_TRACE_FIELD unsigned long long* trace = nullptr;
#if defined(__HIPCC__)
#define Q3T_DECL unsigned long long q3t_[q3::TRACE_SLOTS] = {0, 0, 0, 0, 0, 0, 0, 0};
#define Q3T(i) do { q3t_[i] = (unsigned long long)wall_clock64(); } while (0)
#define Q3T_W(i) do { asm volatile("s_waitcnt vmcnt(0)" ::: "memory"); q3t_[i] = (unsigned long long)wall_clock64(); } while (0)
#define Q3T_K(i, val) do { asm volatile("s_waitcnt lgkmcnt(0)" :: "s"(val) : "memory"); q3t_[i] = (unsigned long long)wall_clock64(); } while (0)
#define Q3T_FLUSH(a, wg) do { if ((a).trace && threadIdx.x == 0 && (int)(wg) < q3::TRACE_WGS) { \
        _Pragma("unroll") for (int q3i_ = 0; q3i_ < q3::TRACE_SLOTS; ++q3i_) (a).trace[(size_t)(wg) * q3::TRACE_SLOTS + q3i_] = q3t_[q3i_]; } \
    if ((a).trace && (threadIdx.x & 63) == 0 && (int)(wg) < q3::TRACE_DWGS && (int)(threadIdx.x >> 6) < q3::TRACE_WAVES) { \
        _Pragma("unroll") for (int q3i_ = 0; q3i_ < q3::TRACE_SLOTS; ++q3i_) \
            (a).trace[(size_t)q3::TRACE_SLOTS * (q3::TRACE_WGS + (wg) * q3::TRACE_WAVES + (threadIdx.x >> 6)) + q3i_] = q3t_[q3i_]; } } while (0)
// ... 134 lines not shown
int attn_prefill_rows_wg(int kernel, int nrep);
hipError_t launch_attn_prefill(const AttnArgs& a, hipStream_t st);
hipError_t launch_attn_prefill(const AttnArgs& a, const AttnPrefillPick& p, hipStream_t st);
hipError_t launch_attn_fused(const AttnArgs& a, hipStream_t st);
bool attn_cp_ok(const AttnArgs& a);
hipError_t launch_attn_cp(const AttnArgs& a, hipStream_t st);

hipError_t launch_gather_rows_bf16(const uint16_t* table, const uint32_t* ids, float* out, int n_rows, int dim,
                                   hipStream_t st);
hipError_t launch_assemble_rows(const float* rows, const int* text_row, const uint16_t* codec_emb, const int* codec_id,
                                const float* xvec, float* out, int n, int H, hipStream_t st,
                                const uint32_t* ref_codes = nullptr, const uint16_t* const* cp_embs = nullptr);
hipError_t launch_copy_rows(const float* src, int lds, float* dst, int ldd, int rows, int cols, hipStream_t st);
hipError_t launch_scatter_rows(const float* src, const int* dst_row, float* rows, int n_src, int cols, hipStream_t st);
hipError_t launch_publish_text(const int* ent, int n, int* trail_len, int* text_ready, int* limit, hipStream_t st);

struct CpGatherArgs {
    int pass;
    const float* last_hidden; int H;
    const uint16_t* codec_emb;
    const uint32_t* tok;
    const uint16_t* cp_emb;
    const float* cp_logits;
    int cp_vocab;
    uint32_t* codes;
    const int* frame_idx;
    int max_frames;
    float* out; int ld_out;
    const float* proj_tab = nullptr; int proj_dim = 0;
    const float* qkv_tab = nullptr; int qkv_dim = 0; float* qkv_out = nullptr; int ld_qkv_out = 0;
    int B;
};
hipError_t launch_cp_gather(const CpGatherArgs& a, hipStream_t st);

struct FrameEmbedArgs {
    const uint16_t* codec_emb; const uint16_t* cp_embs[15];
    const uint32_t* tok; const float* cp_logits_last; int cp_vocab;
    uint32_t* codes; const int* frame_idx; int max_frames;
    const float* text_rows; const int* trail_base; const int* trail_len; const int* pad_row;
    float* out; int H; int B; int n_acoustic;
    const int* text_ready = nullptr;
};
hipError_t launch_frame_embed(const FrameEmbedArgs& a, hipStream_t st);

struct SampleRow {
    float inv_temp; int apply_temp; int greedy;
    int top_k; float top_p; int use_top_p;
    float rep_pen, rep_inv; int use_rep;
    int eos_id; int min_new_tokens; int pad;
};
struct SampleArgs {
    const float* logits; int ld;
    uint8_t* seen;
    const float* u; int u_stride;
    const int* draw_idx;
    uint32_t* tok;
    int* token_count;
    int token_count_static;
    int* frame_idx; int* pos;
    int advance;
    const SampleRow* rows;
    const int* limit;
    float* logits_hist; int hist_stride_b; int hist_cap;
    int vocab, B;
    float inv_temp; int apply_temp; int greedy;
    int top_k; float top_p; int use_top_p;
    float rep_pen, rep_inv; int use_rep;
    int eos_id; int min_new_tokens; int codec_eos; int use_suppress;
    const int* text_ready;
};
hipError_t launch_sample(const SampleArgs& a, hipStream_t st);

struct ConvArgs {
    const float* x; const float* w; const float* b; float* y;
    int cin, cout, L, k, dil;
    const float* snake_a = nullptr; const float* snake_b = nullptr;
    const float* resid = nullptr;
    const float* scale = nullptr;
    int act = 0;
    const float* post_a = nullptr; const float* post_ib = nullptr;
    float* y2 = nullptr;
    const void* wpk = nullptr;
    int planes = 3;
};
hipError_t launch_pack_conv_w(const float* w, void* out, int cout, int cin, int K, hipStream_t st);
size_t packed_conv_w_bytes(int cout, int cin, int K);
enum ConvKernel {
    CK_NONE = 0,
    CK_OUT1 = 1, CK_OUT1_V4 = 2,
    CK_LIN_SMALL_4W = 3, CK_LIN_SMALL_8W = 4,
    CK_BF16X3_96x128_TM4 = 5,
    CK_BF16X3_4Wx32x128 = 6,
    CK_BF16X3_4Wx32x256 = 7,
    CK_BF16X3_64x128 = 8,
    CK_BF16X3_64x64 = 9,
    CK_BF16X3_128x128 = 10,
    CK_BF16X3_96x128_6W = 11,
    CK_MFMA_F32_64 = 12, CK_MFMA_F32_32 = 13,
    CK_VALU = 14,
    CK_RESUNIT_3W = 15, CK_RESUNIT_6W = 16,
    CK_COUNT = 17
};
enum { CP_KERNEL_MASK = 31, CP_PRE = 32, CP_SEG = 64, CP_CIS128 = 128, CP_NP2 = 256 };
struct ConvPath {
    int kernel = CK_NONE;
    int co_m = 0, t_m = 0, wco = 0, wt = 0;
    bool pre = false, seg = false;
    int cis = 0, np = 0;
    hipError_t refusal = hipSuccess;
};
ConvPath conv_pick(int cout, int cin, int L, int k, int dil, int phases, bool packed, bool has_resid, int planes, bool aligned16,
                   bool transposed = false);
ConvPath resunit_pick(int C, int L, int dil, bool complete, bool ya_is_xa, int planes);
int conv_path_code(const ConvPath& p);
const char* conv_path_name(int code);
hipError_t launch_conv1d(const ConvArgs& a, hipStream_t st, int* path = nullptr);
struct ResUnitArgs {
    const float* xa; float* y; float* ya;
    const void* w1pk; const void* w2pk; const float* b1; const float* b2;
    const float* mid_a; const float* mid_ib; const float* post_a; const float* post_ib;
    int C, L, dil;
    int planes = 3;
};
hipError_t launch_resunit(const ResUnitArgs& r, hipStream_t st, int* path = nullptr);
hipError_t launch_transconv1d_taps(const float* x, const float* wp, const float* b, float* y, int cin, int cout, int L,
                                   int stride, int taps, const float* snake_a, const float* snake_ib, hipStream_t st,
                                   const float* post_a = nullptr, const float* post_ib = nullptr, float* y2 = nullptr,
                                   const void* wpk = nullptr,
                                   int planes = 3, int* path = nullptr);
void transconv_phase_weights(const float* w, int cin, int cout, int k, int stride, float* out);
hipError_t launch_snake_tables(const float* alpha, const float* beta, float* a, float* ib, int C, hipStream_t st);
hipError_t launch_dwconv7(const float* x, const float* w, const float* b, float* y, int C, int L, hipStream_t st);
hipError_t launch_layernorm_c(const float* x, const float* w, const float* b, float* y, int C, int L, float eps,
                              hipStream_t st);
hipError_t launch_rmsnorm_c(const float* x, const float* w, float* y, int C, int L, float eps, hipStream_t st);
hipError_t launch_rope_c(float* q, float* k, const float* cs, const float* sn, int nh, int hd, int L, hipStream_t st);
enum { ATTN_C_VALU = 0, ATTN_C_MFMA = 1 };
int attn_c_pick();
hipError_t launch_attn_c(const float* q, const float* k, const float* v, float* o, int nh, int hd, int L, float scale,
                         hipStream_t st);
hipError_t launch_attn_c(const float* q, const float* k, const float* v, float* o, int nh, int hd, int L, float scale, int kernel,
                         hipStream_t st);
hipError_t launch_mimi_attn(const float* q, const float* k, const float* v, float* o, int nh, int hd, int T, int window, float scale,
                            hipStream_t st);
struct AttnCsRow { const float* kv; int a0, e, qcol; };
struct AttnCbRow { int tab0, a0, e, qcol; };
struct ColCopy { const float* src; float* dst; int sp, dp; };
struct SegCopy { unsigned long long src, dst, n; };
hipError_t launch_rope_c_pos(float* q, float* k, const float* cs, const float* sn, const int* pos, int nh, int hd, int L, hipStream_t st);
hipError_t launch_attn_cs(const float* q, float* o, const AttnCsRow* rows, int n_rows, int max_tiles, size_t layer_off, int nh, int hd,
                          int N, int cap, float scale, hipStream_t st);
hipError_t launch_attn_cb(const float* q, float* o, const AttnCbRow* rows, const float* const* tabs, int n_rows, int max_tiles, size_t layer_off,
                          int nh, int hd, int N, int bf, float scale, hipStream_t st);
hipError_t launch_copy_cols(const ColCopy* d, int n, int C, size_t src_off, size_t dst_off, hipStream_t st);
hipError_t launch_copy_segs(const float* src, float* dst, const SegCopy* segs, int n_segs, size_t max_n, hipStream_t st);
hipError_t launch_gather_frames(const uint32_t* const* src, uint32_t* dst, int n, hipStream_t st);
hipError_t launch_silu_mul(const float* g, const float* u, float* y, int64_t n, hipStream_t st);
hipError_t launch_rvq_embed(const uint32_t* frames, int n_frames, const float* first_cb, const float* const* rest_cbs,
                            float* first_out, float* rest_out, int cb_dim, int cb_size, hipStream_t st);
hipError_t launch_norm_codebook(const float* esum, const float* usage, float* out, int rows, int dim, hipStream_t st);

#if defined(__HIPCC__)
__device__ __forceinline__ float mul_rn(float a, float b) {
#pragma clang fp contract(off)
    return a * b;
}
__device__ __forceinline__ float add_rn(float a, float b) {
#pragma clang fp contract(off)
    return a + b;
}
__device__ __forceinline__ float sub_rn(float a, float b) {
#pragma clang fp contract(off)
    return a - b;
}
typedef __attribute__((ext_vector_type(4))) float act_f4_t;
typedef __attribute__((ext_vector_type(2))) float act_f2_t;
constexpr int ACT_SC1 = 16;
__device__ __forceinline__ __amdgpu_buffer_rsrc_t act_rsrc(const void* p) {
    return __builtin_amdgcn_make_buffer_rsrc(const_cast<void*>(p), 0, 0x7fffffff, 0x00020000);
}
__device__ __forceinline__ float4 act_ld4(__amdgpu_buffer_rsrc_t r, int byte_off) {
    const act_f4_t v = __builtin_bit_cast(act_f4_t, __builtin_amdgcn_raw_buffer_load_b128(r, byte_off, 0, ACT_SC1));
    return float4{v[0], v[1], v[2], v[3]};
}
__device__ __forceinline__ float2 act_ld2(__amdgpu_buffer_rsrc_t r, int byte_off) {
    const act_f2_t v = __builtin_bit_cast(act_f2_t, __builtin_amdgcn_raw_buffer_load_b64(r, byte_off, 0, ACT_SC1));
    return float2{v[0], v[1]};
}
__device__ __forceinline__ float act_ld1(__amdgpu_buffer_rsrc_t r, int byte_off) {
    return __builtin_bit_cast(float, __builtin_amdgcn_raw_buffer_load_b32(r, byte_off, 0, ACT_SC1));
}
__device__ __forceinline__ void act_st4(__amdgpu_buffer_rsrc_t r, int byte_off, const float4& v) {
    typedef __attribute__((ext_vector_type(4))) unsigned int u4;
    const act_f4_t f = {v.x, v.y, v.z, v.w};
    __builtin_amdgcn_raw_buffer_store_b128(__builtin_bit_cast(u4, f), r, byte_off, 0, ACT_SC1);
}
__device__ __forceinline__ void act_st2(__amdgpu_buffer_rsrc_t r, int byte_off, const float2& v) {
    typedef __attribute__((ext_vector_type(2))) unsigned int u2;
    const act_f2_t f = {v.x, v.y};
    __builtin_amdgcn_raw_buffer_store_b64(__builtin_bit_cast(u2, f), r, byte_off, 0, ACT_SC1);
}
__device__ __forceinline__ void act_st1(__amdgpu_buffer_rsrc_t r, int byte_off, float v) {
    __builtin_amdgcn_raw_buffer_store_b32(__builtin_bit_cast(unsigned, v), r, byte_off, 0, ACT_SC1);
}
__device__ __forceinline__ void act_drain() { asm volatile("s_waitcnt vmcnt(0)" ::: "memory"); }

template <typename V, int NC>
__device__ __forceinline__ void qkv_from_slices(const AttnArgs& a, int b, const int (&col)[NC], V (&out)[NC]) {
    const int plane = a.B * a.ld_qkv;
    const __amdgpu_buffer_rsrc_t p0 = act_rsrc(a.qkv_part + (size_t)b * a.ld_qkv), qs = act_rsrc(a.qkv_ssq);
    V x[NC][8]; float q[8];
#pragma unroll
// ... 39 lines not shown
```

qwen3_tts_rs_amd/csrc/q3_kernels_codec.hip:

```cpp
#include "q3_kernels.h"

#include <math.h>
#include <stdio.h>
#include <stdlib.h>

namespace q3 {

__device__ __forceinline__ float sin_sq(float x) {
    if (fabsf(x) >= 8192.0f) { const float s = sinf(x); return s * s; }
    const float k = rintf(x * 0.31830988618379067154f);
    float r = fmaf(-k, 3.140625f, x);
    r = fmaf(-k, 9.67502593994140625e-4f, r);
    r = fmaf(-k, 1.509957990978376432e-7f, r);
    const float z = r * r;
    float p = fmaf(z, -2.50521083854417188e-8f, 2.75573192239858907e-6f);
    p = fmaf(z, p, -1.98412698412698413e-4f);
    p = fmaf(z, p, 8.33333333333333333e-3f);
    p = fmaf(z, p, -1.66666666666666667e-1f);
    const float s = fmaf(r * z, p, r);
    return s * s;
}
__device__ __forceinline__ float snake_f(float x, float a, float ib) { return add_rn(x, mul_rn(sin_sq(x * a), ib)); }

constexpr int CV_CO = 32, CV_T = 128, CV_CI = 16, CV_MAXK = 7, CV_MAXHALO = 54;

__device__ __forceinline__ float conv_act(float v, int act) {
    if (act == 1) return 0.5f * v * (1.0f + erff(v * 0.70710678118654752440f));
    if (act == 3) return fmaxf(v, 0.0f);
    if (act == 4) return tanhf(fmaxf(v, 0.0f));
    if (act == 5) return 1.0f / (expf(-v) + 1.0f);
    if (act == 6) return v > 0.0f ? v : expf(v) - 1.0f;
    return v;
}

struct ConvDev {
    const float* x; const float* w; const float* b; float* y;
    int cin, cout, L, k, dil;
    const float* snake_a; const float* snake_ib;
    const float* resid; const float* scale;
    int act;
    int ostride, ooff, oL;
    size_t w_phase_stride;
    int ooff_phase;
    const float* post_a; const float* post_ib;
    float* y2;
    const void* wpk;
    size_t wpk_phase_stride;
    int phases;
    int planes;
};

__global__ __launch_bounds__(256) void k_conv1d(ConvDev a) {
    __shared__ float xs[CV_CI][CV_T + CV_MAXHALO + 2];
    __shared__ __attribute__((aligned(16))) float ws[CV_CI][CV_MAXK][CV_CO];
    const int tid = threadIdx.x, tx = tid & 31, ty = tid >> 5;
    const int t0 = blockIdx.x * CV_T, co0 = blockIdx.y * CV_CO;
    const float* w = a.w + (size_t)blockIdx.z * a.w_phase_stride;
    const int ooff = a.ooff + (int)blockIdx.z * a.ooff_phase;
    const int halo = (a.k - 1) * a.dil;
    const int W = CV_T + halo;
    float acc[4][4];
#pragma unroll
    for (int i = 0; i < 4; ++i)
#pragma unroll
        for (int j = 0; j < 4; ++j) acc[i][j] = 0.0f;

    for (int ci0 = 0; ci0 < a.cin; ci0 += CV_CI) {
        __syncthreads();
        for (int e = tid; e < CV_CI * W; e += 256) {
            const int ci = e / W, tt = e - ci * W;
            const int c = ci0 + ci, t = t0 - halo + tt;
            float v = 0.0f;
            if (c < a.cin && t >= 0 && t < a.L) {
                v = a.x[(size_t)c * a.L + t];
                if (a.snake_a) v = snake_f(v, a.snake_a[c], a.snake_ib[c]);
            }
            xs[ci][tt] = v;
        }
        for (int e = tid; e < CV_CI * a.k * CV_CO; e += 256) {
            const int co = e % CV_CO, r = e / CV_CO, kk = r % a.k, ci = r / a.k;
            const int c = ci0 + ci, o = co0 + co;
            ws[ci][kk][co] = (c < a.cin && o < a.cout) ? w[((size_t)o * a.cin + c) * a.k + kk] : 0.0f;
        }
        __syncthreads();
        const int nci = (a.cin - ci0) < CV_CI ? (a.cin - ci0) : CV_CI;
        for (int ci = 0; ci < nci; ++ci) {
            for (int kk = 0; kk < a.k; ++kk) {
                const float4 wv = *reinterpret_cast<const float4*>(&ws[ci][kk][ty * 4]);
                const int xo = tx + kk * a.dil;
                float xv[4];
#pragma unroll
                for (int j = 0; j < 4; ++j) xv[j] = xs[ci][xo + 32 * j];
#pragma unroll
                for (int j = 0; j < 4; ++j) {
                    acc[0][j] = fmaf(wv.x, xv[j], acc[0][j]);
                    acc[1][j] = fmaf(wv.y, xv[j], acc[1][j]);
                    acc[2][j] = fmaf(wv.z, xv[j], acc[2][j]);
                    acc[3][j] = fmaf(wv.w, xv[j], acc[3][j]);
                }
            }
        }
    }
#pragma unroll
    for (int i = 0; i < 4; ++i) {
        const int o = co0 + ty * 4 + i;
        if (o >= a.cout) continue;
        const float bias = a.b ? a.b[o] : 0.0f;
        const float sc = a.scale ? a.scale[o] : 1.0f;
#pragma unroll
        for (int j = 0; j < 4; ++j) {
            const int t = t0 + tx + 32 * j;
            if (t >= a.L) continue;
            float v = acc[i][j] + bias;
            v = conv_act(v, a.act);
            if (a.scale) v = v * sc;
            const size_t oi = (size_t)o * a.oL + (size_t)t * a.ostride + ooff;
            if (a.resid) v = a.resid[oi] + v;
            if (a.act == 2) v = fminf(fmaxf(v, -1.0f), 1.0f);
            if (a.post_a) {
                const float va = snake_f(v, a.post_a[o], a.post_ib[o]);
                if (a.y2) { a.y[oi] = v; a.y2[oi] = va; } else a.y[oi] = va;
            } else {
                a.y[oi] = v;
            }
        }
    }
}

typedef __attribute__((ext_vector_type(16))) float f32x16_t;

template <int K, int CO_W, int CI_T>
__global__ __launch_bounds__(256) void k_conv1d_mfma(ConvDev a) {
// ... 79 lines not shown
        dim3 grid((a.L + 127) / 128, a.cout / 64, phases);
        hipLaunchKernelGGL((k_conv1d_mfma<K, 2, 16>), grid, dim3(256), 0, st, a);
    } else {
        dim3 grid((a.L + 255) / 256, (a.cout + 31) / 32, phases);
        hipLaunchKernelGGL((k_conv1d_mfma<K, 1, 16>), grid, dim3(256), 0, st, a);
    }
    return hipGetLastError();
}
static bool conv_pick_mfma(ConvPath& p, int cout, int k) {
    static const bool off = getenv("Q3_CONV_VALU") != nullptr;
    if (off || cout < 32) return false;
    if (k != 1 && k != 2 && k != 3 && k != 7) return false;
    p.kernel = cout % 64 == 0 ? CK_MFMA_F32_64 : CK_MFMA_F32_32;
    return true;
}
static hipError_t launch_conv_mfma(const ConvPath& p, const ConvDev& a, int phases, hipStream_t st) {
    switch (a.k) {
        case 1: return launch_conv_mfma_k<1>(p, a, phases, st);
        case 2: return launch_conv_mfma_k<2>(p, a, phases, st);
        case 3: return launch_conv_mfma_k<3>(p, a, phases, st);
        case 7: return launch_conv_mfma_k<7>(p, a, phases, st);
        default: return hipErrorInvalidValue;
    }
}

typedef __attribute__((ext_vector_type(8))) __bf16 cbf16x8_t;
typedef __attribute__((ext_vector_type(4))) unsigned int cu32x4_t;
typedef __attribute__((ext_vector_type(2))) __bf16 cbf16x2_t;
typedef __attribute__((ext_vector_type(2))) float cf32x2_t;
constexpr int XP = 80;

__device__ __forceinline__ uint32_t cpk_bf16(float lo, float hi) {
    const cf32x2_t v = {lo, hi};
    return __builtin_bit_cast(uint32_t, __builtin_convertvector(v, cbf16x2_t));
}
__device__ __forceinline__ void split3_pair(float a, float b, uint32_t& h, uint32_t& m, uint32_t& l) {
    h = cpk_bf16(a, b);
    const float ra = a - __uint_as_float(h << 16), rb = b - __uint_as_float(h & 0xffff0000u);
    m = cpk_bf16(ra, rb);
    const float sa = ra - __uint_as_float(m << 16), sb = rb - __uint_as_float(m & 0xffff0000u);
    l = cpk_bf16(sa, sb);
}

__global__ __launch_bounds__(256) void k_pack_conv_w(const float* __restrict__ w, cu32x4_t* __restrict__ out, int cout, int cin, int K) {
    const int nc16 = cin >> 4;
    const size_t slot = (size_t)blockIdx.x * 256 + threadIdx.x;
    const size_t n_slots = (size_t)(cout >> 5) * K * nc16 * 64;
    if (slot >= n_slots) return;
    const int lane = (int)(slot & 63);
    size_t tile = slot >> 6;
    const int c16 = (int)(tile % nc16); tile /= nc16;
    const int kk = (int)(tile % K); const int co32 = (int)(tile / K);
    const int co = co32 * 32 + (lane & 31), ci = c16 * 16 + (lane >> 5) * 8;
    cu32x4_t h, m, l;
#pragma unroll
    for (int e = 0; e < 4; ++e) {
        const float a = w[((size_t)co * cin + ci + 2 * e) * K + kk], b = w[((size_t)co * cin + ci + 2 * e + 1) * K + kk];
        uint32_t hh, mm, ll; split3_pair(a, b, hh, mm, ll);
        h[e] = hh; m[e] = mm; l[e] = ll;
    }
    cu32x4_t* o = out + ((slot >> 6) * 3) * 64 + lane;
    o[0] = h; o[64] = m; o[128] = l;
}

hipError_t launch_pack_conv_w(const float* w, void* out, int cout, int cin, int K, hipStream_t st) {
    if (cout % 32 || cin % 16 || K < 1) return hipErrorInvalidValue;
    const size_t n_slots = (size_t)(cout / 32) * K * (cin / 16) * 64;
    hipLaunchKernelGGL(k_pack_conv_w, dim3((unsigned)((n_slots + 255) / 256)), dim3(256), 0, st, w, (cu32x4_t*)out, cout, cin, K);
    return hipGetLastError();
}
size_t packed_conv_w_bytes(int cout, int cin, int K) { return (size_t)(cout / 32) * K * (cin / 16) * 3 * 1024; }

template <int NP>
__device__ __forceinline__ f32x16_t mfmaP(const cu32x4_t (&A)[NP], const cu32x4_t (&B)[NP], f32x16_t acc) {
#define Q3_MF(ap, bp) acc = __builtin_amdgcn_mfma_f32_32x32x16_bf16(__builtin_bit_cast(cbf16x8_t, A[ap]), __builtin_bit_cast(cbf16x8_t, B[bp]), acc, 0, 0, 0)
    if constexpr (NP == 3) { Q3_MF(1, 1); Q3_MF(2, 0); Q3_MF(0, 2); }
    Q3_MF(1, 0); Q3_MF(0, 1); Q3_MF(0, 0);
#undef Q3_MF
    return acc;
}

__host__ __device__ __forceinline__ bool conv_segmented(int k, int cin) { return k == 1 && (cin & 511) == 0; }

template <int K, int CO_M, int T_M, int WCO, int WT, bool PRE = false, bool SEG = false, int CIS = 32, int NP = 3>
__global__ __launch_bounds__(64 * WCO * WT, (CO_M == 2 || T_M >= 8) ? 2 : 3) void k_conv_bf16x3(ConvDev a) {
    constexpr int NT = 64 * WCO * WT;
    constexpr int CO_WG = 32 * CO_M * WCO, T_WG = 32 * T_M * WT;
    constexpr int XPB = CIS * 2 + 16, NOCT = CIS / 8;
    constexpr int NA = (NP == 2 || K == 1) ? 3 : 2;
    extern __shared__ __attribute__((aligned(16))) unsigned char smem[];
    __shared__ float s_prm[4][CO_WG];
    const int tid = threadIdx.x, lane = tid & 63;
    const int wave = __builtin_amdgcn_readfirstlane(tid >> 6);
    const int li = lane & 31, lk = lane >> 5;
    const int wco = wave % WCO, wt = wave / WCO;
    int bx, by, bz;
    {
        const int P = a.phases, nco = a.cout / CO_WG, per = nco * P, nt = (int)gridDim.x / per, nt8 = nt & ~7, lin = (int)blockIdx.x;
        int r, tt;
        if (lin < nt8 * per) { r = lin >> 3; tt = (r / per) * 8 + (lin & 7); r = r % per; }
        else { const int rem = lin - nt8 * per; tt = nt8 + rem / per; r = rem % per; }
        bx = tt; bz = r % P; by = r / P;
    }
    const int t0 = bx * T_WG, co0 = by * CO_WG + wco * (32 * CO_M);
    for (int i = tid; i < CO_WG; i += NT) {
        const int o = by * CO_WG + i;
        const bool ok = o < a.cout;
        s_prm[0][i] = (a.b && ok) ? a.b[o] : 0.0f;
        s_prm[1][i] = (a.scale && ok) ? a.scale[o] : 1.0f;
        s_prm[2][i] = (a.post_a && ok) ? a.post_a[o] : 0.0f;
        s_prm[3][i] = (a.post_a && ok) ? a.post_ib[o] : 0.0f;
    }
    const int halo = (K - 1) * a.dil, W = T_WG + halo;
    const size_t plane = (size_t)W * XPB;
    const unsigned plane32 = (unsigned)W * XPB, bfrag = (unsigned)((wt * (32 * T_M) + li) * XPB + lk * 16);
    const cu32x4_t* __restrict__ wpk = reinterpret_cast<const cu32x4_t*>(a.wpk) + (size_t)bz * a.wpk_phase_stride;
    const int ooff = a.ooff + bz * a.ooff_phase;
    const int nc16 = a.cin >> 4;

    f32x16_t acc[CO_M][T_M];
#pragma unroll
    for (int i = 0; i < CO_M; ++i)
#pragma unroll
        for (int j = 0; j < T_M; ++j)
#pragma unroll
            for (int r = 0; r < 16; ++r) acc[i][j][r] = 0.0f;
    constexpr int SM = SEG ? CO_M : 1, SN = SEG ? T_M : 1;
    f32x16_t tot[SM][SN];
    constexpr bool seg = SEG;
    if (SEG) {
#pragma unroll
        for (int i = 0; i < SM; ++i)
#pragma unroll
            for (int j = 0; j < SN; ++j)
#pragma unroll
                for (int r = 0; r < 16; ++r) tot[i][j][r] = 0.0f;
    }

    const uint64_t wpa = reinterpret_cast<uint64_t>(wpk);
    const uint64_t wpu = ((uint64_t)(uint32_t)__builtin_amdgcn_readfirstlane((int)(wpa >> 32)) << 32) | (uint32_t)__builtin_amdgcn_readfirstlane((int)wpa);
    const __amdgpu_buffer_rsrc_t wrs = __builtin_amdgcn_make_buffer_rsrc(reinterpret_cast<void*>(wpu), 0, 0x7fffffff, 0x00020000);
    const int co32 = __builtin_amdgcn_readfirstlane(co0 >> 5);
    auto load_A = [&](cu32x4_t (&A)[CO_M][NP], int ci0, int kk, int c16l) {
#pragma unroll
        for (int cm = 0; cm < CO_M; ++cm) {
            const int tile = ((co32 + cm) * K + kk) * nc16 + (ci0 >> 4) + c16l;
#pragma unroll
            for (int pl = 0; pl < NP; ++pl)
                A[cm][pl] = __builtin_bit_cast(cu32x4_t, __builtin_amdgcn_raw_buffer_load_b128(wrs, lane * 16, (tile * 3 + pl) * 1024, 0));
        }
    };
    for (int ci0 = 0; ci0 < a.cin; ci0 += CIS) {
        const int n16 = (a.cin - ci0) >= CIS ? CIS / 16 : (a.cin - ci0) >> 4;
        const int n_steps = K * n16;
        cu32x4_t A[NA][CO_M][NP];
        load_A(A[0], ci0, 0, 0);
        if constexpr (NA == 3) load_A(A[1], ci0, (n_steps > 1 ? 1 : 0) / n16, (n_steps > 1 ? 1 : 0) % n16);
        __syncthreads();
        constexpr int NCHK = (T_WG + (K - 1) * 9 + 63) / 64, NBF = (NOCT * NCHK + WCO * WT - 1) / (WCO * WT);
        constexpr int NB = NBF < 1 ? 1 : (NBF > 4 ? 4 : NBF);
        const int n_items = NOCT * ((W + 63) >> 6);
        for (int c0 = wave; c0 < n_items; c0 += NB * WCO * WT) {
            float v[NB][8];
            bool ok[NB];
#pragma unroll
            for (int i = 0; i < NB; ++i) {
                const int c = c0 + i * WCO * WT;
                const int q = c % NOCT, tt = (c / NOCT) * 64 + lane;
                const int ca = ci0 + q * 8, t = t0 - halo + tt;
                ok[i] = c < n_items && tt < W && ca < a.cin && t >= 0 && t < a.L;
                const int cc = ca < a.cin ? ca : a.cin - 8, tc = t < 0 ? 0 : (t < a.L ? t : a.L - 1);
                const float* xr = a.x + (size_t)cc * a.L + tc;
#pragma unroll
                for (int e = 0; e < 8; ++e) v[i][e] = xr[(size_t)e * a.L];
            }
#pragma unroll
            for (int i = 0; i < NB; ++i) {
                const int c = c0 + i * WCO * WT;
                if (c >= n_items) break;
                const int q = c % NOCT, tt = (c / NOCT) * 64 + lane;
                const int ca = ci0 + q * 8;
                if (a.snake_a && ca < a.cin) {
#pragma unroll
                    for (int e = 0; e < 8; ++e) v[i][e] = snake_f(v[i][e], a.snake_a[ca + e], a.snake_ib[ca + e]);
                }
#pragma unroll
                for (int e = 0; e < 8; ++e) v[i][e] = ok[i] ? v[i][e] : 0.0f;
                if (tt < W) {
                    cu32x4_t h, m, l;
#pragma unroll
                    for (int e = 0; e < 4; ++e) { uint32_t hh, mm, ll; split3_pair(v[i][2 * e], v[i][2 * e + 1], hh, mm, ll); h[e] = hh; m[e] = mm; l[e] = ll; }
                    unsigned char* row = smem + (unsigned)tt * XPB + q * 16;
                    *reinterpret_cast<cu32x4_t*>(row) = h;
                    *reinterpret_cast<cu32x4_t*>(row + plane) = m;
                    if constexpr (NP == 3) *reinterpret_cast<cu32x4_t*>(row + 2 * plane) = l;
                }
            }
        }
        __syncthreads();
        auto do_step = [&](const cu32x4_t (&A)[CO_M][NP], int s) {
            const int kk = s / n16, c16l = s - kk * n16;
            cu32x4_t B[T_M][NP];
            const unsigned so = (unsigned)(kk * a.dil * XPB + c16l * 32);
            const unsigned char* bp0 = smem + (bfrag + so);
            const unsigned char* bp1 = smem + (bfrag + so + plane32);
            const unsigned char* bp2 = smem + (bfrag + so + 2 * plane32);
#pragma unroll
            for (int tm = 0; tm < T_M; ++tm) {
                B[tm][0] = *reinterpret_cast<const cu32x4_t*>(bp0 + tm * (32 * XPB));
                B[tm][1] = *reinterpret_cast<const cu32x4_t*>(bp1 + tm * (32 * XPB));
                if constexpr (NP == 3) B[tm][2] = *reinterpret_cast<const cu32x4_t*>(bp2 + tm * (32 * XPB));
            }
#pragma unroll
            for (int cm = 0; cm < CO_M; ++cm)
#pragma unroll
                for (int tm = 0; tm < T_M; ++tm) acc[cm][tm] = mfmaP<NP>(A[cm], B[tm], acc[cm][tm]);
        };
        const int last = n_steps - 1;
        auto fetch = [&](cu32x4_t (&Ad)[CO_M][NP], int sp) {
            sp = sp < last ? sp : last;
            __builtin_amdgcn_sched_barrier(0); load_A(Ad, ci0, sp / n16, sp % n16); __builtin_amdgcn_sched_barrier(0);
        };
        int st = 0;
        if constexpr (NA == 3) {
            for (; st + 2 < n_steps; st += 3) {
                fetch(A[2], st + 2); do_step(A[0], st);
                fetch(A[0], st + 3); do_step(A[1], st + 1);
                fetch(A[1], st + 4); do_step(A[2], st + 2);
            }
            if (st < n_steps) do_step(A[0], st);
            if (st + 1 < n_steps) do_step(A[1], st + 1);
        } else {
            for (; st + 1 < n_steps; st += 2) {
                fetch(A[1], st + 1); do_step(A[0], st);
                fetch(A[0], st + 2); do_step(A[1], st + 1);
            }
            if (st < n_steps) do_step(A[0], st);
        }
        if (SEG && ((ci0 + CIS) & 127) == 0) {
#pragma unroll
            for (int i = 0; i < SM; ++i)
#pragma unroll
                for (int j = 0; j < SN; ++j)
#pragma unroll
                    for (int r = 0; r < 16; ++r) { tot[i][j][r] = tot[i][j][r] + acc[i][j][r]; acc[i][j][r] = 0.0f; }
        }
    }
    if (SEG) {
#pragma unroll
        for (int i = 0; i < SM; ++i)
#pragma unroll
            for (int j = 0; j < SN; ++j) acc[i][j] = tot[i][j];
    }
#pragma unroll
    for (int cm = 0; cm < CO_M; ++cm) {
        float rs[PRE ? T_M : 1][16];
        if constexpr (PRE) {
#pragma unroll
            for (int reg = 0; reg < 16; ++reg) {
                const int o = co0 + cm * 32 + (reg & 3) + 8 * (reg >> 2) + 4 * lk;
#pragma unroll
                for (int tm = 0; tm < T_M; ++tm) {
                    const int t = t0 + wt * (32 * T_M) + tm * 32 + li;
                    rs[tm][reg] = (a.resid && o < a.cout && t < a.L) ? a.resid[(size_t)o * a.oL + (size_t)t * a.ostride + ooff] : 0.0f;
                }
            }
        }
#pragma unroll
        for (int reg = 0; reg < 16; ++reg) {
            const int o = co0 + cm * 32 + (reg & 3) + 8 * (reg >> 2) + 4 * lk;
            const bool ook = o < a.cout;
            const int pi = o - by * CO_WG;
            const float bias = s_prm[0][pi], sc = s_prm[1][pi], pa = s_prm[2][pi], pib = s_prm[3][pi];
#pragma unroll
            for (int tm = 0; tm < T_M; ++tm) {
                const int t = t0 + wt * (32 * T_M) + tm * 32 + li;
                if (ook && t < a.L) {
                    float v = acc[cm][tm][reg] + bias;
                    v = conv_act(v, a.act);
                    if (a.scale) v = v * sc;
                    const size_t oi = (size_t)o * a.oL + (size_t)t * a.ostride + ooff;
                    if (a.resid) v = (PRE ? rs[PRE ? tm : 0][reg] : a.resid[oi]) + v;
                    if (a.act == 2) v = fminf(fmaxf(v, -1.0f), 1.0f);
                    if (a.post_a) {
                        const float va = snake_f(v, pa, pib);
                        if (a.y2) { a.y[oi] = v; a.y2[oi] = va; } else a.y[oi] = va;
                    } else {
                        a.y[oi] = v;
                    }
                }
            }
        }
    }
}

struct ResUnitDev {
    const float* xa;
    float* y;
    float* ya;
    const void* w1pk; const void* w2pk;
    const float* b1; const float* b2;
    const float* mid_a; const float* mid_ib;
    const float* post_a; const float* post_ib;
    int C, L, dil;
};

template <int NW, int NP = 3>
__global__ __launch_bounds__(64 * NW, 3) void k_resunit_bf16x3(ResUnitDev a) {
    constexpr int K = 7, T_M = 4, NT = 64 * NW, C = 32 * NW, T_WG = 128;
    constexpr int XPB = 80, NOCT = 4;
    constexpr int XP2 = C * 2 + 16;
    extern __shared__ __attribute__((aligned(16))) unsigned char smem[];
    __shared__ float s_prm[6][C];
    const int tid = threadIdx.x, lane = tid & 63;
    const int wave = __builtin_amdgcn_readfirstlane(tid >> 6);
    const int li = lane & 31, lk = lane >> 5;
    const int t0 = (int)blockIdx.x * T_WG;
    for (int i = tid; i < C; i += NT) {
        s_prm[0][i] = a.b1 ? a.b1[i] : 0.0f; s_prm[1][i] = a.mid_a[i]; s_prm[2][i] = a.mid_ib[i];
        s_prm[3][i] = a.b2 ? a.b2[i] : 0.0f;
        s_prm[4][i] = a.post_a ? a.post_a[i] : 0.0f; s_prm[5][i] = a.post_a ? a.post_ib[i] : 0.0f;
    }
    const int halo = (K - 1) * a.dil, W = T_WG + halo;
    const unsigned plane32 = (unsigned)W * XPB, bfrag = (unsigned)(li * XPB + lk * 16);
    constexpr int nc16 = C / 16;

    f32x16_t acc[T_M];
#pragma unroll
    for (int j = 0; j < T_M; ++j)
#pragma unroll
        for (int r = 0; r < 16; ++r) acc[j][r] = 0.0f;

    auto rsrc = [&](const void* p) {
        const uint64_t pa = reinterpret_cast<uint64_t>(p);
        const uint64_t pu = ((uint64_t)(uint32_t)__builtin_amdgcn_readfirstlane((int)(pa >> 32)) << 32) | (uint32_t)__builtin_amdgcn_readfirstlane((int)pa);
// ... 198 lines not shown
    float tot[NR];
#pragma unroll
    for (int j = 0; j < NR; ++j) tot[j] = 0.0f;
    for (int s0 = 0; s0 < nseg; s0 += W) {
        const int seg = s0 + wave;
        if (seg < nseg) {
            cu32x4_t A[8][NP];
            float xv[8][8];
#pragma unroll
            for (int i = 0; i < 8; ++i) {
                const size_t tile = (size_t)co32 * nc16 + seg * 8 + i;
#pragma unroll
                for (int pl = 0; pl < NP; ++pl) A[i][pl] = wpk[(tile * 3 + pl) * 64 + lane];
            }
#pragma unroll
            for (int i = 0; i < 8; ++i)
#pragma unroll
                for (int e = 0; e < 8; ++e) {
                    const int ci = seg * 128 + i * 16 + lk * 8 + e;
                    xv[i][e] = tok ? x[(size_t)ci * a.L + tc] : 0.0f;
                }
            if (a.snake_a) {
#pragma unroll
                for (int i = 0; i < 8; ++i)
#pragma unroll
                    for (int e = 0; e < 8; ++e) {
                        const int ci = seg * 128 + i * 16 + lk * 8 + e;
                        if (tok) xv[i][e] = snake_f(xv[i][e], a.snake_a[ci], a.snake_ib[ci]);
                    }
            }
            f32x16_t acc;
#pragma unroll
            for (int r = 0; r < 16; ++r) acc[r] = 0.0f;
#pragma unroll
            for (int i = 0; i < 8; ++i) {
                cu32x4_t B[NP];
#pragma unroll
                for (int e = 0; e < 4; ++e) { uint32_t h, m, l; split3_pair(xv[i][2 * e], xv[i][2 * e + 1], h, m, l); B[0][e] = h; B[1][e] = m; if constexpr (NP == 3) B[2][e] = l; }
                acc = mfmaP<NP>(A[i], B, acc);
            }
#pragma unroll
            for (int r = 0; r < 16; ++r) part[wave][r][lane] = acc[r];
        }
        __syncthreads();
        const int n = (nseg - s0) < W ? (nseg - s0) : W;
#pragma unroll
        for (int j = 0; j < NR; ++j)
            for (int q = 0; q < n; ++q) tot[j] = tot[j] + part[q][wave + j * W][lane];
        __syncthreads();
    }
#pragma unroll
    for (int j = 0; j < NR; ++j) {
        const int reg = wave + j * W;
        const int o = co0 + (reg & 3) + 8 * (reg >> 2) + 4 * lk;
        if (o < a.cout && tok) {
            float v = tot[j] + (a.b ? a.b[o] : 0.0f);
            v = conv_act(v, a.act);
            if (a.scale) v = v * a.scale[o];
            const size_t oi = (size_t)o * a.oL + (size_t)tc * a.ostride + a.ooff;
            if (a.resid) v = a.resid[oi] + v;
            if (a.act == 2) v = fminf(fmaxf(v, -1.0f), 1.0f);
            if (a.post_a) {
                const float va = snake_f(v, a.post_a[o], a.post_ib[o]);
                if (a.y2) { a.y[oi] = v; a.y2[oi] = va; } else a.y[oi] = va;
            } else {
                a.y[oi] = v;
            }
        }
    }
}

template <int K, int CO_M, int T_M, int WCO, int WT, int NP>
static hipError_t launch_bf16x3_vp(const ConvPath& p, const ConvDev& a, int phases, hipStream_t st) {
    constexpr int CO_WG = 32 * CO_M * WCO, T_WG = 32 * T_M * WT;
    constexpr bool K1 = K == 1;
    constexpr int CIS1 = T_WG <= 64 ? 128 : 32;
    if ((p.cis != 32 && !(K1 && p.cis == CIS1)) || (!K1 && (p.pre || p.seg)) || (p.pre && CO_M != 1)) return hipErrorInvalidValue;
    const bool wide = p.cis > 32;
    const size_t lds = (size_t)NP * (T_WG + (K - 1) * a.dil) * (p.cis * 2 + 16);
    dim3 grid(((a.L + T_WG - 1) / T_WG) * (a.cout / CO_WG) * phases);
    ConvDev ap = a; ap.phases = phases;
    const bool segm = p.seg;
    const dim3 blk(64 * WCO * WT);
    if constexpr (K1) {
        const bool pre = p.pre;
#define Q3_CV(P, S, C) hipLaunchKernelGGL((k_conv_bf16x3<K, CO_M, T_M, WCO, WT, P, S, C, NP>), grid, blk, lds, st, ap)
        if (wide) {
            if (segm) { if (pre) Q3_CV(CO_M == 1, true, CIS1); else Q3_CV(false, true, CIS1); }
            else { if (pre) Q3_CV(CO_M == 1, false, CIS1); else Q3_CV(false, false, CIS1); }
        } else {
            if (segm) { if (pre) Q3_CV(CO_M == 1, true, 32); else Q3_CV(false, true, 32); }
            else { if (pre) Q3_CV(CO_M == 1, false, 32); else Q3_CV(false, false, 32); }
        }
#undef Q3_CV
    } else {
        hipLaunchKernelGGL((k_conv_bf16x3<K, CO_M, T_M, WCO, WT, false, false, 32, NP>), grid, blk, lds, st, ap);
    }
    return hipGetLastError();
}
static bool conv_two_plane_taps(int k) { return k == 1 || k == 2 || k == 7; }
template <int K, int CO_M, int T_M, int WCO, int WT>
static hipError_t launch_bf16x3_v(const ConvPath& p, const ConvDev& a, int phases, hipStream_t st) {
    if constexpr (K == 1 || K == 2 || K == 7)
        if (p.np == 2) return launch_bf16x3_vp<K, CO_M, T_M, WCO, WT, 2>(p, a, phases, st);
    if (p.np != 3) return hipErrorInvalidValue;
    return launch_bf16x3_vp<K, CO_M, T_M, WCO, WT, 3>(p, a, phases, st);
}
template <int K>
static hipError_t launch_bf16x3_k(const ConvPath& p, const ConvDev& a, int phases, hipStream_t st) {
    switch (p.kernel) {
        case CK_BF16X3_96x128_TM4: return launch_bf16x3_v<K, 1, 4, 3, 1>(p, a, phases, st);
        case CK_BF16X3_4Wx32x128: return launch_bf16x3_v<K, 1, 4, 4, 1>(p, a, phases, st);
        case CK_BF16X3_4Wx32x256: return launch_bf16x3_v<K, 1, 8, 4, 1>(p, a, phases, st);
        case CK_BF16X3_64x128: return launch_bf16x3_v<K, 1, 2, 2, 2>(p, a, phases, st);
        case CK_BF16X3_64x64: return launch_bf16x3_v<K, 1, 1, 2, 2>(p, a, phases, st);
        case CK_BF16X3_128x128: return launch_bf16x3_v<K, 2, 2, 2, 2>(p, a, phases, st);
        case CK_BF16X3_96x128_6W: return launch_bf16x3_v<K, 1, 2, 3, 2>(p, a, phases, st);
        default: return hipErrorInvalidValue;
    }
}
static int conv_pick_geometry(int K, int cout, int L, int phases, bool has_resid) {
    const long big_tiles = (long)((L + 127) / 128) * (cout / 128) * phases;
    static const int geo = [] { const char* e = getenv("Q3_CONV_TM4"); return e ? atoi(e) : 2; }();
    if (geo && K >= 2 && L >= 4096 && (cout == 192 || cout == 96)) return CK_BF16X3_96x128_TM4;
    if (geo >= 2 && K >= 2 && L >= 4096 && cout % 128 == 0 && big_tiles >= 192) {
        if (geo == 2) return CK_BF16X3_4Wx32x128;
        if (geo == 3) return CK_BF16X3_4Wx32x256;
    }
    if (K == 1 && has_resid && cout % 64 == 0 && cout != 96 && big_tiles >= 192) return CK_BF16X3_64x128;
    {
        static const int pw = [] { const char* e = getenv("Q3_CONV_PW1_GEO"); return e ? atoi(e) : 2; }();
        if (pw && K == 1 && !has_resid && cout % 128 == 0 && big_tiles >= 192 && big_tiles < 1024) {
            if (pw == 1) return CK_BF16X3_64x128;
            return CK_BF16X3_64x64;
        }
    }
    if (cout % 128 == 0 && big_tiles >= 192) return CK_BF16X3_128x128;
    if (cout == 192) return CK_BF16X3_96x128_6W;
    if (cout == 96) return CK_BF16X3_96x128_6W;
    if (cout % 64 == 0) return CK_BF16X3_64x64;
    return CK_NONE;
}
static bool conv_pick_bf16x3(ConvPath& p, int cout, int cin, int L, int k, int phases, bool packed, bool has_resid, int np) {
    static const bool off = getenv("Q3_CONV_F32") != nullptr;
    if (off || !packed || cin % 16 || cout % 32) return false;
    static const bool no_small = getenv("Q3_CONV_NO_SMALL") != nullptr;
    static const bool no_small_tiles = getenv("Q3_CONV_NO_SMALL_TILES") != nullptr;
    const long small_wgs = (long)(cout / 32) * ((L + 31) / 32);
    const bool small_tiles = L > 32 && cin >= 1024 && small_wgs <= 512 && !no_small_tiles;
    if (conv_segmented(k, cin) && (L <= 32 || small_tiles) && phases == 1 && cout % 64 == 0 && !no_small) {
        p.kernel = cin >= 1024 ? CK_LIN_SMALL_8W : CK_LIN_SMALL_4W;
        p.co_m = 1; p.t_m = 1; p.wco = 1; p.wt = 1; p.seg = true; p.np = np;
        return true;
    }
    if (k != 1 && k != 2 && k != 3 && k != 5 && k != 7) return false;
    const int g = conv_pick_geometry(k, cout, L, phases, has_resid);
    if (g == CK_NONE) return false;
    static const int GEO[7][4] = {{1, 4, 3, 1}, {1, 4, 4, 1}, {1, 8, 4, 1}, {1, 2, 2, 2}, {1, 1, 2, 2}, {2, 2, 2, 2}, {1, 2, 3, 2}};
    const int* q = GEO[g - CK_BF16X3_96x128_TM4];
    p.kernel = g; p.co_m = q[0]; p.t_m = q[1]; p.wco = q[2]; p.wt = q[3];
    p.np = conv_two_plane_taps(k) ? np : 3;
    p.cis = 32;
    if (k == 1) {
        static const bool cis32 = getenv("Q3_CONV_CIS32") != nullptr;
        const int cis1 = 32 * p.t_m * p.wt <= 64 ? 128 : 32;
        if (cis1 > 32 && !cis32 && cin >= 2 * cis1) p.cis = cis1;
// ... 7 lines not shown
    ConvPath p;
    if (k < 1 || k > CV_MAXK || (k - 1) * dil > CV_MAXHALO || L <= 0 || cout < 1 || cin < 1 || phases < 1) { p.refusal = hipErrorInvalidValue; return p; }
    if (cout == 1 && !transposed) {
        p.kernel = (k == 7 && dil == 1 && L % 4 == 0 && aligned16) ? CK_OUT1_V4 : CK_OUT1;
        return p;
    }
    if (conv_pick_bf16x3(p, cout, cin, L, k, phases, packed, has_resid, conv_planes(planes))) return p;
    if (conv_pick_mfma(p, cout, k)) return p;
    p.kernel = CK_VALU;
    return p;
}

int conv_path_code(const ConvPath& p) {
    return p.kernel | (p.pre ? CP_PRE : 0) | (p.seg ? CP_SEG : 0) | (p.cis == 128 ? CP_CIS128 : 0) | (p.np == 2 ? CP_NP2 : 0);
}
const char* conv_path_name(int code) {
    static const char* const KN[CK_COUNT] = {
        "none", "k_conv_out1", "k_conv_out1_v4", "k_lin_small_bf16x3<4>", "k_lin_small_bf16x3<8>",
        "k_conv_bf16x3<96co x 128t, 3 waves, T_M=4>", "k_conv_bf16x3<4 waves x 32co x 128t>", "k_conv_bf16x3<4 waves x 32co x 256t>",
        "k_conv_bf16x3<64co x 128t>", "k_conv_bf16x3<64co x 64t>", "k_conv_bf16x3<128co x 128t>", "k_conv_bf16x3<96co x 128t, 6 waves>",
        "k_conv1d_mfma<CO_W=2>", "k_conv1d_mfma<CO_W=1>", "k_conv1d", "k_resunit_bf16x3<3>", "k_resunit_bf16x3<6>"};
    static thread_local char buf[96];
    const int k = code & CP_KERNEL_MASK;
    if (code < 0 || k >= CK_COUNT || (code & ~(CP_KERNEL_MASK | CP_PRE | CP_SEG | CP_CIS128 | CP_NP2))) return "invalid";
    snprintf(buf, sizeof buf, "%s%s%s%s%s", KN[k], (code & CP_PRE) ? " PRE" : "", (code & CP_SEG) ? " SEG" : "", (code & CP_CIS128) ? " CIS=128" : "",
             (code & CP_NP2) ? " NP=2" : "");
    return buf;
}

__global__ __launch_bounds__(256) void k_conv_out1(ConvDev a) {
    const int t = blockIdx.x * 256 + threadIdx.x;
    if (t >= a.L) return;
    float acc = 0.0f;
    for (int c = 0; c < a.cin; ++c) {
        const float sa = a.snake_a ? a.snake_a[c] : 0.0f, sib = a.snake_a ? a.snake_ib[c] : 0.0f;
        for (int kk = 0; kk < a.k; ++kk) {
            const int ts = t - (a.k - 1 - kk) * a.dil;
            if (ts < 0) continue;
            float v = a.x[(size_t)c * a.L + ts];
            if (a.snake_a) v = snake_f(v, sa, sib);
            acc = fmaf(a.w[(size_t)c * a.k + kk], v, acc);
        }
    }
    float v = acc + (a.b ? a.b[0] : 0.0f);
    if (a.act == 2) v = fminf(fmaxf(v, -1.0f), 1.0f);
    a.y[t] = v;
}

__global__ __launch_bounds__(256) void k_conv_out1_v4(ConvDev a) {
    const int t = (blockIdx.x * 256 + threadIdx.x) * 4;
    if (t >= a.L) return;
    float acc[4] = {0.0f, 0.0f, 0.0f, 0.0f};
    for (int c = 0; c < a.cin; ++c) {
        const float* xr = a.x + (size_t)c * a.L + t;
        const float4 z = make_float4(0.f, 0.f, 0.f, 0.f);
        const float4 p0 = t >= 8 ? *reinterpret_cast<const float4*>(xr - 8) : z;
        const float4 p1 = t >= 4 ? *reinterpret_cast<const float4*>(xr - 4) : z;
        const float4 p2 = *reinterpret_cast<const float4*>(xr);
        float v[12] = {p0.x, p0.y, p0.z, p0.w, p1.x, p1.y, p1.z, p1.w, p2.x, p2.y, p2.z, p2.w};
        if (a.snake_a) {
            const float sa = a.snake_a[c], sib = a.snake_ib[c];
#pragma unroll
            for (int i = 2; i < 12; ++i) v[i] = snake_f(v[i], sa, sib);
        }
        float w[7];
#pragma unroll
        for (int kk = 0; kk < 7; ++kk) w[kk] = a.w[(size_t)c * 7 + kk];
#pragma unroll
        for (int j = 0; j < 4; ++j)
#pragma unroll
            for (int kk = 0; kk < 7; ++kk) acc[j] = fmaf(w[kk], v[j + kk + 2], acc[j]);
    }
    float o[4];
#pragma unroll
    for (int j = 0; j < 4; ++j) {
        float v = acc[j] + (a.b ? a.b[0] : 0.0f);
        if (a.act == 2) v = fminf(fmaxf(v, -1.0f), 1.0f);
        o[j] = v;
    }
    *reinterpret_cast<float4*>(a.y + t) = make_float4(o[0], o[1], o[2], o[3]);
}

static hipError_t launch_conv_path(const ConvPath& p, const ConvDev& a, int phases, hipStream_t st) {
    switch (p.kernel) {
        case CK_NONE: return p.refusal != hipSuccess ? p.refusal : hipErrorInvalidValue;
        case CK_OUT1_V4: hipLaunchKernelGGL(k_conv_out1_v4, dim3((a.L / 4 + 255) / 256), dim3(256), 0, st, a); break;
        case CK_OUT1: hipLaunchKernelGGL(k_conv_out1, dim3((a.L + 255) / 256), dim3(256), 0, st, a); break;
        case CK_LIN_SMALL_4W:
        case CK_LIN_SMALL_8W: {
            const dim3 grid(a.cout / 32, (a.L + 31) / 32);
            if (p.np == 2) {
                if (p.kernel == CK_LIN_SMALL_8W) hipLaunchKernelGGL((k_lin_small_bf16x3<8, 2>), grid, dim3(512), 0, st, a);
                else hipLaunchKernelGGL((k_lin_small_bf16x3<4, 2>), grid, dim3(256), 0, st, a);
            } else {
                if (p.kernel == CK_LIN_SMALL_8W) hipLaunchKernelGGL((k_lin_small_bf16x3<8, 3>), grid, dim3(512), 0, st, a);
                else hipLaunchKernelGGL((k_lin_small_bf16x3<4, 3>), grid, dim3(256), 0, st, a);
            }
            break;
        }
        case CK_MFMA_F32_64:
        case CK_MFMA_F32_32: return launch_conv_mfma(p, a, phases, st);
        case CK_VALU: {
            dim3 grid((a.L + CV_T - 1) / CV_T, (a.cout + CV_CO - 1) / CV_CO, phases);
            hipLaunchKernelGGL(k_conv1d, grid, dim3(256), 0, st, a);
            break;
        }
        default:
            switch (a.k) {
                case 1: return launch_bf16x3_k<1>(p, a, phases, st);
                case 2: return launch_bf16x3_k<2>(p, a, phases, st);
                case 3: return launch_bf16x3_k<3>(p, a, phases, st);
                case 5: return launch_bf16x3_k<5>(p, a, phases, st);
                case 7: return launch_bf16x3_k<7>(p, a, phases, st);
                default: return hipErrorInvalidValue;
            }
    }
    return hipGetLastError();
}

hipError_t launch_conv1d(const ConvArgs& c, hipStream_t st, int* path) {
    const ConvPath p = conv_pick(c.cout, c.cin, c.L, c.k, c.dil, 1, c.wpk != nullptr, c.resid != nullptr, c.planes,
                                 (((uintptr_t)c.x | (uintptr_t)c.y) & 15) == 0, false);
    if (path) *path = conv_path_code(p);
    if (p.kernel == CK_NONE) return p.refusal;
    ConvDev a{};
    a.x = c.x; a.w = c.w; a.b = c.b; a.y = c.y; a.cin = c.cin; a.cout = c.cout; a.L = c.L; a.k = c.k; a.dil = c.dil;
    a.snake_a = c.snake_a; a.snake_ib = c.snake_b; a.resid = c.resid; a.scale = c.scale; a.act = c.act;
    a.ostride = 1; a.ooff = 0; a.oL = c.L; a.w_phase_stride = 0; a.ooff_phase = 0;
    a.post_a = c.post_a; a.post_ib = c.post_ib; a.y2 = c.y2;
    a.wpk = c.wpk; a.wpk_phase_stride = 0; a.planes = conv_planes(c.planes);
    return launch_conv_path(p, a, 1, st);
}

hipError_t launch_transconv1d_taps(const float* x, const float* wp, const float* b, float* y, int cin, int cout, int L,
                                   int stride, int taps, const float* snake_a, const float* snake_ib, hipStream_t st,
                                   const float* post_a, const float* post_ib, float* y2, const void* wpk, int planes, int* path) {
    const ConvPath p = conv_pick(cout, cin, L, taps, 1, stride, wpk != nullptr, false, planes, false, true);
    if (path) *path = conv_path_code(p);
    if (p.kernel == CK_NONE) return p.refusal;
    ConvDev a{};
    a.planes = conv_planes(planes);
    a.wpk = wpk; a.wpk_phase_stride = packed_conv_w_bytes(cout, cin, taps) / 16;
    a.post_a = post_a; a.post_ib = post_ib; a.y2 = y2;
    a.x = x; a.w = wp; a.b = b; a.y = y; a.cin = cin; a.cout = cout; a.L = L; a.k = taps; a.dil = 1;
    a.snake_a = snake_a; a.snake_ib = snake_ib; a.resid = nullptr; a.scale = nullptr; a.act = 0;
    a.ostride = stride; a.ooff = 0; a.oL = L * stride;
    a.w_phase_stride = (size_t)cout * cin * taps; a.ooff_phase = 1;
    return launch_conv_path(p, a, stride, st);
}

void transconv_phase_weights(const float* w, int cin, int cout, int k, int stride, float* out) {
    const int taps = k / stride;
    for (int ph = 0; ph < stride; ++ph)
        for (int co = 0; co < cout; ++co)
            for (int ci = 0; ci < cin; ++ci)
                for (int tp = 0; tp < taps; ++tp) {
                    const int kk = ph + (taps - 1 - tp) * stride;
                    out[(((size_t)ph * cout + co) * cin + ci) * taps + tp] = w[((size_t)ci * cout + co) * k + kk];
                }
}

__global__ __launch_bounds__(256) void k_dwconv7(const float* x, const float* w, const float* b, float* y, int L) {
    const int c = blockIdx.y, t = blockIdx.x * 256 + threadIdx.x;
    if (t >= L) return;
    const float* xr = x + (size_t)c * L;
    float acc = 0.0f;
#pragma unroll
    for (int kk = 0; kk < 7; ++kk) {
        const int ts = t - 6 + kk;
        if (ts >= 0) acc = fmaf(w[c * 7 + kk], xr[ts], acc);
    }
    y[(size_t)c * L + t] = acc + b[c];
}
hipError_t launch_dwconv7(const float* x, const float* w, const float* b, float* y, int C, int L, hipStream_t st) {
    hipLaunchKernelGGL(k_dwconv7, dim3((L + 255) / 256, C), dim3(256), 0, st, x, w, b, y, L);
    return hipGetLastError();
}

template <bool LAYERNORM>
__global__ __launch_bounds__(256) void k_norm_c(const float* __restrict__ x, const float* __restrict__ w, const float* __restrict__ b,
                                                float* __restrict__ y, int C, int L, float eps) {
    __shared__ float s1[8][32], s2[8][32];
    const int tx = threadIdx.x & 31, cg = threadIdx.x >> 5;
    const int t = blockIdx.x * 32 + tx;
    float a = 0.0f, q = 0.0f;
    if (t < L) {
        int c = cg;
        for (; c + 56 < C; c += 64) {
            float v[8];
#pragma unroll
            for (int u = 0; u < 8; ++u) v[u] = x[(size_t)(c + 8 * u) * L + t];
#pragma unroll
            for (int u = 0; u < 8; ++u) { a += v[u]; q += v[u] * v[u]; }
        }
        for (; c < C; c += 8) { const float v = x[(size_t)c * L + t]; a += v; q += v * v; }
    }
    s1[cg][tx] = a; s2[cg][tx] = q;
    __syncthreads();
    float sum = 0.0f, sq = 0.0f;
#pragma unroll
    for (int g = 0; g < 8; ++g) { sum += s1[g][tx]; sq += s2[g][tx]; }
    if (t >= L) return;
    if (LAYERNORM) {
        const float mean = sum / (float)C, var = sq / (float)C - mean * mean;
        const float inv = 1.0f / sqrtf(var + eps);
#pragma unroll 8
        for (int c = cg; c < C; c += 8) y[(size_t)c * L + t] = (x[(size_t)c * L + t] - mean) * inv * w[c] + b[c];
    } else {
        const float den = sqrtf(sq / (float)C + eps);
#pragma unroll 8
        for (int c = cg; c < C; c += 8) y[(size_t)c * L + t] = x[(size_t)c * L + t] / den * w[c];
    }
}
template <bool LAYERNORM, int CPT>
__global__ __launch_bounds__(256) void k_norm_c2(const float* __restrict__ x, const float* __restrict__ w, const float* __restrict__ b,
                                                 float* __restrict__ y, int C, int L, float eps) {
    __shared__ float s1[16][16], s2[16][16];
    const int tx = threadIdx.x & 15, cg = threadIdx.x >> 4;
    const int t = blockIdx.x * 16 + tx;
    const bool in = t < L;
    float v[CPT];
#pragma unroll
    for (int u = 0; u < CPT; ++u) v[u] = in ? x[(size_t)(cg + 16 * u) * L + t] : 0.0f;
    float wv[CPT], bv[LAYERNORM ? CPT : 1];
#pragma unroll
    for (int u = 0; u < CPT; ++u) { wv[u] = w[cg + 16 * u]; if (LAYERNORM) bv[u] = b[cg + 16 * u]; }
// ... 336 lines not shown
```

qwen3_tts_rs_amd/csrc/q3_testapi.hip:

```cpp
#include "q3_engine.h"

extern "C" q3_status q3_talker_step(q3_session* s, const float* embeds_host, float* hidden_host, float* logits_host) {
    if (!s || !embeds_host) return set_err(Q3_INVALID_ARG, "null argument");
    if (!s->prefilled) return set_err(Q3_INVALID_ARG, "session not prefilled");
    const q3_config& c = s->m->cfg;
    HIPC(hipSetDevice(s->m->device));
    std::vector<int> posv(s->B);
    HIPC(sync_frames(s));
    HIPC(q3_hipMemcpy(posv.data(), s->pos, s->B * 4, hipMemcpyDeviceToHost));
    for (int p : posv) if (p >= s->max_seq) return set_err(Q3_KV_OVERFLOW, "KV cache full (%d)", s->max_seq);
    for (int b = 0; b < s->B; ++b) Q3C(kv_reserve_row(s, b, posv[(size_t)b] + 1));
    HIPC(hipMemcpyAsync(s->tb.X, embeds_host, (size_t)s->B * c.hidden * 4, hipMemcpyHostToDevice, s->stream));
    Q3C(talker_step(s, s->pos, 0, true));
    HIPC(sync_frames(s));
    for (int& p : posv) p += 1;
    HIPC(q3_hipMemcpy(s->pos, posv.data(), s->B * 4, hipMemcpyHostToDevice));
    if (hidden_host) HIPC(q3_hipMemcpy(hidden_host, s->LASTH, (size_t)s->B * c.hidden * 4, hipMemcpyDeviceToHost));
    if (logits_host) HIPC(q3_hipMemcpy(logits_host, s->LOGITS, (size_t)s->B * c.codec_vocab * 4, hipMemcpyDeviceToHost));
    return Q3_OK;
}

extern "C" q3_status q3_cp_generate(q3_session* s, const float* last_hidden_host, const float* sem_embed_host,
                                    uint32_t* codes15_host, float* cp_logits_host) {
    if (!s || !last_hidden_host || !codes15_host) return set_err(Q3_INVALID_ARG, "null argument");
// ... 483 lines not shown
        if (e == hipSuccess && p->n_splits > 1) e = launch_attn_merge(t, 0);
    } else if (variant == 1) {
        e = launch_qknorm_rope_kv(t, 0);
        if (e == hipSuccess) e = launch_attn_decode(t, 0);
        if (e == hipSuccess) e = launch_attn_merge(t, 0);
    } else if (variant == 2) e = launch_attn_cp(t, 0);
    else e = launch_attn_first2(t, 0);
    if (e == hipErrorInvalidValue || e == hipErrorNotSupported) {
        (void)hipGetLastError();
        (void)q3_hipDeviceSynchronize();
        return set_err(Q3_UNSUPPORTED, "q3_attn_step_ex: the launcher refused variant=%d layout=%d nh=%d nkv=%d splits=%d rows_per_seq=%d (%s)", variant, layout, nh, nkv,
                       p->n_splits, rps, hipGetErrorString(e));
    }
    HIPC(e);
    HIPC(q3_hipDeviceSynchronize());
    HIPC(q3_hipMemcpy(p->out, out, (size_t)B * QD * 4, hipMemcpyDeviceToHost));
    if (layout != 0) {
        std::vector<std::vector<uint32_t>> got;
        HIPC(slabs.download(got));
        each_row([&](int slot, size_t elem, float* row) { slabs.get_row(got, slot, elem, row); slabs.copy_row(slabs.img, got, slot, elem); });
        slabs.strays(got, p->stray);
    } else {
        HIPC(q3_hipMemcpy(p->kcache, kv, cn * 4, hipMemcpyDeviceToHost)); HIPC(q3_hipMemcpy(p->vcache, kv + cn, cn * 4, hipMemcpyDeviceToHost));
        if (p->stray) { p->stray[0] = 0; p->stray[1] = -1; }
    }
    if (t.g_x) HIPC(q3_hipMemcpy(p->g_x, t.g_x, gx_rows * p->g_ldx * 4, hipMemcpyDeviceToHost));
    if (t.g_codes) HIPC(q3_hipMemcpy(p->g_codes, t.g_codes, (size_t)B * p->g_max_frames * 16 * 4, hipMemcpyDeviceToHost));
    if (t.zero) HIPC(q3_hipMemcpy(p->zero_buf, t.zero, zn * 4, hipMemcpyDeviceToHost));
    return Q3_OK;
}

extern "C" q3_status q3_kv_pages_to_bf16_ex(int device, int n_layers, int nkv, int n_pages, const int* src_slots, const int* dst_slots,
                                            const float* src, uint16_t* dst, int* rot_used, long long* stray) {
    if (!src_slots || !dst_slots || !src || !dst || !stray) return set_err(Q3_INVALID_ARG, "q3_kv_pages_to_bf16_ex: null argument");
    if (n_layers < 1 || n_layers > 4 || nkv < 1 || nkv > 8 || n_pages < 1 || n_pages > KvPool::SLAB_SLOTS)
        return set_err(Q3_INVALID_ARG, "q3_kv_pages_to_bf16_ex: bad shape (n_layers 1..4, nkv 1..8, n_pages 1..%d)", KvPool::SLAB_SLOTS);
    if (!slots_ok(src_slots, n_pages, KvPool::SLAB_SLOTS) || !slots_ok(dst_slots, n_pages, KvPool::SLAB_SLOTS))
        return set_err(Q3_INVALID_ARG, "q3_kv_pages_to_bf16_ex: the slots of a list must be distinct slots of 0 .. %d", KvPool::SLAB_SLOTS - 1);
    HIPC(hipSetDevice(device));
    DevPool pool;
    TestSlabs a, b;
    a.shape(n_layers, nkv, 4); b.shape(n_layers, nkv, 2);
    HIPC(a.add_slab(pool)); HIPC(b.add_slab(pool));
    a.fill_pattern(); b.fill_pattern();
    auto each_row = [&](auto&& f) {
        for (int pg = 0; pg < n_pages; ++pg) for (int l = 0; l < n_layers; ++l) for (int v = 0; v < 2; ++v) for (int g = 0; g < nkv; ++g) for (int pp = 0; pp < KV_PAGE_POS; ++pp)
            f(pg, l, v, g, pp, (((((size_t)pg * n_layers + l) * 2 + v) * nkv + g) * KV_PAGE_POS + pp) * HEAD_DIM);
    };
    each_row([&](int pg, int l, int v, int g, int pp, size_t at) { a.put_row(a.img, src_slots[pg], a.row_elem(src_slots[pg], l, v, g, pp), src + at); });
    HIPC(a.upload()); HIPC(b.upload());
    std::vector<unsigned long long> lists((size_t)2 * n_pages);
    for (int pg = 0; pg < n_pages; ++pg) { lists[(size_t)pg] = a.page(src_slots[pg]); lists[(size_t)n_pages + pg] = b.page(dst_slots[pg]); }
    if (rot_used)
        for (int pg = 0; pg < n_pages; ++pg) for (int g = 0; g < nkv; ++g) {
            rot_used[(size_t)pg * nkv + g] = kv_rot(lists[(size_t)pg], g);
            rot_used[((size_t)n_pages + pg) * nkv + g] = kv_rot(lists[(size_t)n_pages + pg], g);
        }
    unsigned long long* dl; HIPC(pool.alloc(&dl, lists.size()));
    HIPC(q3_hipMemcpy(dl, lists.data(), lists.size() * 8, hipMemcpyHostToDevice));
    HIPC(q3_hipDeviceSynchronize());
    HIPC(launch_kv_pages_to_bf16(dl, dl + n_pages, n_pages, n_layers, nkv, a.geo.layer_stride(), a.geo.v_delta(), 0));
    HIPC(q3_hipDeviceSynchronize());
    std::vector<std::vector<uint32_t>> got;
    HIPC(b.download(got));
    std::vector<float> row((size_t)HEAD_DIM);
    each_row([&](int pg, int l, int v, int g, int pp, size_t at) {
        const size_t elem = b.row_elem(dst_slots[pg], l, v, g, pp);
        b.get_row(got, dst_slots[pg], elem, row.data());
        for (int dd = 0; dd < HEAD_DIM; ++dd) { uint32_t u; memcpy(&u, &row[(size_t)dd], 4); dst[at + dd] = (uint16_t)(u >> 16); }
        b.copy_row(b.img, got, dst_slots[pg], elem);
    });
    b.strays(got, stray);
    return Q3_OK;
}

extern "C" int q3_conv_path(int cout, int cin, int L, int k, int dil, int phases, int packed, int has_resid, int planes, int aligned16) {
    return conv_path_code(conv_pick(cout, cin, L, k, dil, phases, packed != 0, has_resid != 0, planes, aligned16 != 0, phases > 1));
}
extern "C" int q3_resunit_path(int C, int L, int dil, int packed, int ya_is_xa, int planes) {
    return conv_path_code(resunit_pick(C, L, dil, packed != 0, ya_is_xa != 0, planes));
}
extern "C" const char* q3_conv_path_name(int code) { return conv_path_name(code); }

extern "C" q3_status q3_conv_ex(int device, const q3_conv_ex_args* p) {
    if (!p || !p->x || !p->w || !p->y) return set_err(Q3_INVALID_ARG, "q3_conv_ex: null argument");
    if (p->path) *p->path = 0;
    const int kind = p->kind, cin = p->cin, cout = p->cout, L = p->L, k = p->k, dil = p->dil;
    if (kind < 0 || kind > 2) return set_err(Q3_INVALID_ARG, "q3_conv_ex: kind 0..2");
    if (cin < 1 || cin > 8192 || cout < 1 || cout > 8192 || L < 1 || L > (1 << 22) || k < 1 || k > 64 || dil < 1 || dil > 64 || p->act < 0 || p->act > 6)
        return set_err(Q3_INVALID_ARG, "q3_conv_ex: bad shape (channels 1..8192, L 1..2^22, k 1..64, dil 1..64, act 0..6)");
    const int stride = kind == 1 ? p->stride : 1;
    if (kind == 1 && (stride < 1 || stride > 16 || k % stride)) return set_err(Q3_INVALID_ARG, "q3_conv_ex: transposed conv needs 1 <= stride <= 16 and k %% stride == 0");
    const int taps = k / stride;
    if (kind == 2 && (cin != cout || k != 7 || !p->w2 || !p->mid_a || !p->mid_ib)) return set_err(Q3_INVALID_ARG, "q3_conv_ex: residual unit needs cin == cout, k == 7, w2 and the middle snake pair");
    if (!p->snake_a != !p->snake_b || !p->post_a != !p->post_ib || !p->mid_a != !p->mid_ib) return set_err(Q3_INVALID_ARG, "q3_conv_ex: half a snake pair");
    if (kind != 0 && (p->resid || p->resid_in_place || p->scale || p->act)) return set_err(Q3_INVALID_ARG, "q3_conv_ex: resid / scale / act belong to kind 0");
    if (kind != 0 && kind != 2 && p->y2_is_x) return set_err(Q3_INVALID_ARG, "q3_conv_ex: y2_is_x belongs to kind 2");
    if ((p->resid && p->resid_in_place) || (p->y2 && p->y2_is_x)) return set_err(Q3_INVALID_ARG, "q3_conv_ex: two residuals / two y2");
    const size_t out_n = (size_t)cout * L * stride, xn = (size_t)cin * L, wn = (size_t)cout * cin * k;
    if (p->y_front < 0 || p->y_front % 4 || p->y_elems < 0 || (size_t)p->y_elems < (size_t)p->y_front + out_n)
        return set_err(Q3_INVALID_ARG, "q3_conv_ex: y must hold y_front (a multiple of 4) + cout * L * stride floats");
    HIPC(hipSetDevice(device));
    DevPool pool;
    float *x, *w, *w2 = nullptr, *b = nullptr, *b2 = nullptr, *res = nullptr, *scale = nullptr, *y, *y2 = nullptr;
    void *wpk = nullptr, *w2pk = nullptr;
    HIPC(pool.alloc(&x, xn)); HIPC(q3_hipMemcpy(x, p->x, xn * 4, hipMemcpyHostToDevice));
    HIPC(pool.alloc(&w, wn));
    if (kind == 1) {
        std::vector<float> wp(wn);
        transconv_phase_weights(p->w, cin, cout, k, stride, wp.data());
        HIPC(q3_hipMemcpy(w, wp.data(), wn * 4, hipMemcpyHostToDevice));
    } else HIPC(q3_hipMemcpy(w, p->w, wn * 4, hipMemcpyHostToDevice));
    if (kind == 2) { HIPC(pool.alloc(&w2, (size_t)cout * cin)); HIPC(q3_hipMemcpy(w2, p->w2, (size_t)cout * cin * 4, hipMemcpyHostToDevice)); }
    auto vec = [&](const float* h, int n, float** d) -> q3_status {
        *d = nullptr;
        if (!h) return Q3_OK;
        HIPC(pool.alloc(d, (size_t)n)); HIPC(q3_hipMemcpy(*d, h, (size_t)n * 4, hipMemcpyHostToDevice));
        return Q3_OK;
    };
    auto pair = [&](const float* ha, const float* hb, int n, float** da, float** db) -> q3_status {
        Q3C(vec(ha, n, da)); Q3C(vec(hb, n, db));
        if (ha && p->snake_raw) {
            float *ta, *tb;
            HIPC(pool.alloc(&ta, (size_t)n)); HIPC(pool.alloc(&tb, (size_t)n));
            HIPC(launch_snake_tables(*da, *db, ta, tb, n, 0));
            *da = ta; *db = tb;
        }
        return Q3_OK;
    };
    float *sa, *sb, *pa, *pb, *ma, *mb;
    Q3C(vec(p->b, cout, &b)); Q3C(vec(p->b2, cout, &b2)); Q3C(vec(p->scale, cout, &scale)); Q3C(vec(p->resid, (int)out_n, &res));
    Q3C(pair(p->snake_a, p->snake_b, cin, &sa, &sb)); Q3C(pair(p->post_a, p->post_ib, cout, &pa, &pb)); Q3C(pair(p->mid_a, p->mid_ib, cout, &ma, &mb));
    const size_t yn = (size_t)p->y_elems;
    HIPC(pool.alloc(&y, yn)); HIPC(q3_hipMemcpy(y, p->y, yn * 4, hipMemcpyHostToDevice));
    if (p->y2) { HIPC(pool.alloc(&y2, yn)); HIPC(q3_hipMemcpy(y2, p->y2, yn * 4, hipMemcpyHostToDevice)); }
    float* yr = y + p->y_front; float* y2r = y2 ? y2 + p->y_front : nullptr;
    if (p->packed) {
        const int pk = kind == 1 ? taps : k;
        if (cout % 32 || cin % 16 || pk < 1) return set_err(Q3_UNSUPPORTED, "q3_conv_ex: cout %d / cin %d cannot be packed (cout %% 32, cin %% 16)", cout, cin);
        const size_t per = packed_conv_w_bytes(cout, cin, pk);
        char* d; HIPC(pool.alloc(&d, per * (size_t)stride)); wpk = d;
        for (int ph = 0; ph < stride; ++ph) HIPC(launch_pack_conv_w(w + (size_t)ph * cout * cin * pk, d + (size_t)ph * per, cout, cin, pk, 0));
        if (kind == 2) {
            char* d2; HIPC(pool.alloc(&d2, packed_conv_w_bytes(cout, cin, 1))); w2pk = d2;
            HIPC(launch_pack_conv_w(w2, d2, cout, cin, 1, 0));
        }
    }
    HIPC(q3_hipDeviceSynchronize());
    hipError_t e;
    int path = 0;
    if (kind == 0) {
        ConvArgs a;
        a.x = x; a.w = w; a.b = b; a.y = yr; a.cin = cin; a.cout = cout; a.L = L; a.k = k; a.dil = dil;
        a.snake_a = sa; a.snake_b = sb; a.resid = p->resid_in_place ? yr : res; a.scale = scale; a.act = p->act;
        a.post_a = pa; a.post_ib = pb; a.y2 = y2r; a.wpk = wpk; a.planes = p->planes;
        e = launch_conv1d(a, 0, &path);
    } else if (kind == 1) {
        e = launch_transconv1d_taps(x, w, b, yr, cin, cout, L, stride, taps, sa, sb, 0, pa, pb, y2r, wpk, p->planes, &path);
    } else {
        ResUnitArgs r{};
        r.xa = x; r.y = yr; r.ya = p->y2_is_x ? x : y2r; r.w1pk = wpk; r.w2pk = w2pk; r.b1 = b; r.b2 = b2;
        r.mid_a = ma; r.mid_ib = mb; r.post_a = pa; r.post_ib = pb; r.C = cout; r.L = L; r.dil = dil; r.planes = p->planes;
        e = launch_resunit(r, 0, &path);
    }
    if (p->path) *p->path = path;
    if (e == hipErrorInvalidValue || e == hipErrorNotSupported) {
        (void)hipGetLastError();
        return set_err(Q3_UNSUPPORTED, "q3_conv_ex: the launcher refused kind=%d cin=%d cout=%d L=%d k=%d dil=%d stride=%d packed=%d planes=%d (%s)", kind, cin, cout,
                       L, k, dil, stride, p->packed, p->planes, hipGetErrorString(e));
    }
    HIPC(e);
    HIPC(q3_hipDeviceSynchronize());
    HIPC(q3_hipMemcpy(p->y, y, yn * 4, hipMemcpyDeviceToHost));
    if (y2) HIPC(q3_hipMemcpy(p->y2, y2, yn * 4, hipMemcpyDeviceToHost));
    return Q3_OK;
}

static q3_status check_cl_out(const char* who, const void* x, const void* w, const void* y, int C, int L, int y_front, int y_elems) {
    if (!x || !w || !y) return set_err(Q3_INVALID_ARG, "%s: null argument", who);
    if (C < 1 || C > 8192 || L < 1 || L > (1 << 22)) return set_err(Q3_INVALID_ARG, "%s: bad shape (C 1..8192, L 1..2^22)", who);
    if (y_front < 0 || y_elems < 0 || (size_t)y_elems < (size_t)y_front + (size_t)C * L) return set_err(Q3_INVALID_ARG, "%s: y must hold y_front + C * L floats", who);
    return Q3_OK;
}

extern "C" q3_status q3_norm_c(int device, int layernorm, const float* x_host, const float* w_host, const float* b_host, int C, int L, float eps,
                               float* y_host, int y_front, int y_elems) {
    Q3C(check_cl_out("q3_norm_c", x_host, w_host, y_host, C, L, y_front, y_elems));
    if (layernorm && !b_host) return set_err(Q3_INVALID_ARG, "q3_norm_c: LayerNorm needs a bias");
    HIPC(hipSetDevice(device));
    DevPool pool;
    float *x, *w, *b = nullptr, *y;
    const size_t n = (size_t)C * L;
    HIPC(pool.alloc(&x, n)); HIPC(pool.alloc(&w, (size_t)C)); HIPC(pool.alloc(&y, (size_t)y_elems));
    HIPC(q3_hipMemcpy(x, x_host, n * 4, hipMemcpyHostToDevice)); HIPC(q3_hipMemcpy(w, w_host, (size_t)C * 4, hipMemcpyHostToDevice));
    HIPC(q3_hipMemcpy(y, y_host, (size_t)y_elems * 4, hipMemcpyHostToDevice));
    if (layernorm) { HIPC(pool.alloc(&b, (size_t)C)); HIPC(q3_hipMemcpy(b, b_host, (size_t)C * 4, hipMemcpyHostToDevice)); }
    HIPC(q3_hipDeviceSynchronize());
    if (layernorm) HIPC(launch_layernorm_c(x, w, b, y + y_front, C, L, eps, 0));
    else HIPC(launch_rmsnorm_c(x, w, y + y_front, C, L, eps, 0));
    HIPC(q3_hipDeviceSynchronize());
    HIPC(q3_hipMemcpy(y_host, y, (size_t)y_elems * 4, hipMemcpyDeviceToHost));
    return Q3_OK;
}

extern "C" q3_status q3_dwconv7(int device, const float* x_host, const float* w_host, const float* b_host, int C, int L, float* y_host, int y_front,
                                int y_elems) {
    Q3C(check_cl_out("q3_dwconv7", x_host, w_host, y_host, C, L, y_front, y_elems));
    if (!b_host) return set_err(Q3_INVALID_ARG, "q3_dwconv7: null argument");
    HIPC(hipSetDevice(device));
    DevPool pool;
    float *x, *w, *b, *y;
    const size_t n = (size_t)C * L;
    HIPC(pool.alloc(&x, n)); HIPC(pool.alloc(&w, (size_t)C * 7)); HIPC(pool.alloc(&b, (size_t)C)); HIPC(pool.alloc(&y, (size_t)y_elems));
    HIPC(q3_hipMemcpy(x, x_host, n * 4, hipMemcpyHostToDevice)); HIPC(q3_hipMemcpy(w, w_host, (size_t)C * 7 * 4, hipMemcpyHostToDevice));
    HIPC(q3_hipMemcpy(b, b_host, (size_t)C * 4, hipMemcpyHostToDevice)); HIPC(q3_hipMemcpy(y, y_host, (size_t)y_elems * 4, hipMemcpyHostToDevice));
    HIPC(q3_hipDeviceSynchronize());
    HIPC(launch_dwconv7(x, w, b, y + y_front, C, L, 0));
    HIPC(q3_hipDeviceSynchronize());
    HIPC(q3_hipMemcpy(y_host, y, (size_t)y_elems * 4, hipMemcpyDeviceToHost));
    return Q3_OK;
}

static hipError_t fill_ff(void* dev, size_t bytes) {
    std::vector<unsigned char> h(bytes, 0xFF);
    return q3_hipMemcpy(dev, h.data(), bytes, hipMemcpyHostToDevice);
}
static void gemm_path_out(const GemmPick& p, int* path) {
    if (!path) return;
    path[0] = p.geometry; path[1] = p.geometry == GEMM_G3 ? p.k_ranges : 1; path[2] = p.geometry == GEMM_G3 ? p.k_split : 1;
    path[3] = p.geometry == GEMM_G2 ? p.n_split : 1;
}
static size_t gemm_ex_ws_bytes(int M, int N, int Kpad, int epi) {
    if (Kpad % 128 || (Kpad >> 6) % 16) return 0;
    return (size_t)8 * (epi == EPI_SWIGLU ? 2 : 1) * M * N * sizeof(float);
}

extern "C" int q3_gemm_path(int M, int N, int K, int epi, int norm, int w2, int planes, int* path) {
    if (path) path[0] = path[1] = path[2] = path[3] = 0;
    if (M < 1 || N < 1 || K < 4) return -1;
    static float dummy[4];
    GemmArgs g;
    g.W = reinterpret_cast<const uint16_t*>(dummy); g.W2 = w2 ? g.W : nullptr; g.x = dummy; g.ldx = up32(K); g.y = dummy; g.ldy = N;
    g.norm_w = norm ? dummy : nullptr; g.den = norm ? dummy : nullptr;
    g.M = M; g.N = N; g.K = K; g.Kpad = up32(K); g.epi = epi;
    if (planes) { g.xp = g.W; g.xp_plane = (size_t)up128(M) * g.Kpad; g.splitk_ws_bytes = gemm_ex_ws_bytes(M, N, g.Kpad, epi); g.splitk_ws = g.splitk_ws_bytes ? dummy : nullptr; }
    if (g.K % 4 || g.N % 64 || (planes && K % 8)) return -1;
    const bool rms = norm != 0;
    if (epi < EPI_NONE || epi > EPI_SWIGLU || ((epi == EPI_RESID || epi == EPI_SILU) && rms) || (epi == EPI_SWIGLU && (!rms || !w2))) return -1;
    const GemmPick p = lm_gemm_pick(g);
    gemm_path_out(p, path);
    return p.geometry;
}

extern "C" q3_status q3_gemm_ex(int device, const q3_gemm_ex_args* p) {
    if (!p || !p->x || !p->w || !p->y) return set_err(Q3_INVALID_ARG, "q3_gemm_ex: null argument");
    if (p->path) p->path[0] = p->path[1] = p->path[2] = p->path[3] = 0;
    const int M = p->M, N = p->N, K = p->K;
    if (M < 1 || M > 8192 || N < 1 || N > 16384 || K < 4 || K > 16384) return set_err(Q3_INVALID_ARG, "q3_gemm_ex: bad shape (M 1..8192, N 1..16384, K 4..16384)");
// ... 708 lines not shown
```

Before: 2841.

## Pass codec decoder activations between convs as pre-split bf16 planes

The producer convolutions in the codec decoder stack can now emit their snake-activated outputs directly as channel-octet bf16 hi/mid/lo planes. The next transposed conv or k=7 conv reads those planes instead of fp32 activations, so it no longer has to re-split each input in its loader. A mask chosen per block by kernel-path eligibility (env-overridable) picks which stages use planes, and the workspace is enlarged to hold the plane buffers. This aims to cut activation memory traffic and split work per conv, at the cost of extra kernel template instantiations and more complex buffer aliasing.

```diff
diff --git a/include/q3tts.h b/include/q3tts.h
--- a/include/q3tts.h
+++ b/include/q3tts.h
@@ -247,6 +247,8 @@
     float* y; float* y2;
 } q3_conv_ex_args;
 q3_status q3_conv_ex(int device, const q3_conv_ex_args* args);
+q3_status q3_conv_planes_ex(int device, const q3_conv_ex_args* args, const uint16_t* x_planes, uint16_t* y_planes);
+int q3_codec_planes_used(const q3_model* m, int n_frames);
 int q3_gemm_path(int M, int N, int K, int epi, int norm, int w2, int planes, int* path);
 typedef struct q3_gemm_ex_args {
     int M, N, K, ldx, ldy, ldr, M_alloc;
diff --git a/qwen3_tts_rs_amd/_lib.py b/qwen3_tts_rs_amd/_lib.py
--- a/qwen3_tts_rs_amd/_lib.py
+++ b/qwen3_tts_rs_amd/_lib.py
@@ -276,6 +276,8 @@
     "q3_resunit_path": (c_int, [c_int] * 6),
     "q3_conv_path_name": (c_char_p, [c_int]),
     "q3_conv_ex": (c_int, [c_int, P(CConvEx)]),
+    "q3_conv_planes_ex": (c_int, [c_int, P(CConvEx), c_void_p, c_void_p]),
+    "q3_codec_planes_used": (c_int, [c_void_p, c_int]),
     "q3_gemm_path": (c_int, [c_int] * 7 + [P(ctypes.c_int32)]),
     "q3_gemm_ex": (c_int, [c_int, P(CGemmEx)]),
     "q3_attn_prefill_path": (c_int, [c_int] * 4 + [P(ctypes.c_int32)]),
diff --git a/qwen3_tts_rs_amd/api.py b/qwen3_tts_rs_amd/api.py
--- a/qwen3_tts_rs_amd/api.py
+++ b/qwen3_tts_rs_amd/api.py
@@ -910,6 +910,9 @@
 
     def set_codec_planes(self, planes: int):
         check(lib.q3_model_set_codec_planes(self._h, int(planes)))
+
+    def codec_planes_used(self, n_frames: int) -> int:
+        return int(lib.q3_codec_planes_used(self._h, int(n_frames)))
 
     def kv_pool_trim(self) -> int:
         n = ctypes.c_size_t()
@@ -1992,7 +1995,7 @@
             post=None, mid=None, resid: Optional[np.ndarray] = None, resid_in_place: bool = False, scale: Optional[np.ndarray] = None,
             act: int = 0, planes: int = 3, packed: bool = True, snake_raw: bool = False, w2: Optional[np.ndarray] = None,
             b2: Optional[np.ndarray] = None, y: Optional[np.ndarray] = None, y2: Optional[np.ndarray] = None, y_front: int = 0,
-            y2_is_x: bool = False, device: int = 0):
+            y2_is_x: bool = False, device: int = 0, x_planes: Optional[np.ndarray] = None, y_planes: Optional[np.ndarray] = None):
     f = lambda a: np.ascontiguousarray(a, dtype=np.float32)
     x = f(x); w = f(w)
     assert x.ndim == 2 and w.ndim == 3
@@ -2026,8 +2029,14 @@
     for (na, nb, pr, n) in (("snake_a", "snake_b", snake, cin), ("post_a", "post_ib", post, cout), ("mid_a", "mid_ib", mid, cout)):
         if pr is not None:
             opt(na, pr[0], n); opt(nb, pr[1], n)
+    for buf, C, Lp in ((x_planes, cin, L), (y_planes, cout, n_out // cout)):
+        assert buf is None or (buf.dtype == np.uint16 and buf.flags.c_contiguous and buf.shape == (3, C // 8, Lp, 8) and C % 8 == 0)
     try:
-        check(lib.q3_conv_ex(device, ctypes.byref(a)))
+        if x_planes is None and y_planes is None:
+            check(lib.q3_conv_ex(device, ctypes.byref(a)))
+        else:
+            check(lib.q3_conv_planes_ex(device, ctypes.byref(a), ptr(x_planes) if x_planes is not None else None,
+                                        ptr(y_planes) if y_planes is not None else None))
     except _lib.Q3Error as e:
         e.path = path.value
         raise
diff --git a/qwen3_tts_rs_amd/csrc/q3_codec_run.hip b/qwen3_tts_rs_amd/csrc/q3_codec_run.hip
--- a/qwen3_tts_rs_amd/csrc/q3_codec_run.hip
+++ b/qwen3_tts_rs_amd/csrc/q3_codec_run.hip
@@ -72,7 +72,9 @@
     int up = 1; for (int i = 0; i < 2; ++i) up *= c.dec_up_ratios[i];
     size_t per = (size_t)4 * c.dec_latent * up;
     { size_t L = up; int C = c.dec_dim; per = per > (size_t)C * L ? per : (size_t)C * L;
-      for (int b = 0; b < 4; ++b) { L *= c.dec_up_rates[b]; C /= 2; if ((size_t)C * L > per) per = (size_t)C * L; } }
+      auto planes_fit = [&](size_t n) { n = (n * 3 + 1) / 2; if (n > per) per = n; };
+      planes_fit((size_t)C * L);
+      for (int b = 0; b < 4; ++b) { L *= c.dec_up_rates[b]; C /= 2; if ((size_t)C * L > per) per = (size_t)C * L; if (b < 3) planes_fit((size_t)C * L); } }
     const int QDm = c.dec_heads * c.dec_head_dim;
     size_t per_front = (size_t)4 * QDm;
     if ((size_t)2 * c.dec_inter > per_front) per_front = (size_t)2 * c.dec_inter;
@@ -112,7 +114,7 @@
 static thread_local const q3_model* tl_codec_model = nullptr;
 static const void* packed_of(const float* w) { return tl_codec_model ? tl_codec_model->pk(w) : nullptr; }
 static thread_local int tl_codec_planes = 3;
-CodecScope::CodecScope(const q3_model* m) {
+CodecScope::CodecScope(const q3_model* m, bool xp) : xplanes(xp) {
     static const int env_planes = [] { const char* e = getenv("Q3_CODEC_PLANES"); const int v = e ? atoi(e) : 0; return (v == 2 || v == 3) ? v : 0; }();
     planes = env_planes ? env_planes : m->codec_planes;
     tl_codec_model = m; tl_codec_planes = planes;
@@ -192,6 +194,43 @@
     HIPC(conv1(Nn, m->outp_w, m->outp_b, C, DH, LAT, T, st));
     return Q3_OK;
 }
+enum { XPLANES_ADOPTED = 0x54, XPLANES_ALL = 0x7f };
+static unsigned codec_xplanes_mask() {
+    if (getenv("Q3_CONV_F32") || getenv("Q3_CONV_VALU")) return 0u;
+    const char* e = getenv("Q3_CODEC_XPLANES");
+    if (!e || !strcmp(e, "1")) return (unsigned)XPLANES_ADOPTED;
+    return (unsigned)strtoul(e, nullptr, 0) & (unsigned)XPLANES_ALL;
+}
+static unsigned codec_stack_planes(const q3_model* m, int L, int NPL) {
+    static const int dils[3] = {1, 3, 9};
+    const unsigned xm = codec_xplanes_mask();
+    if (!xm) return 0;
+    auto bf = [&](const float* w, int cout, int cin, int Lc, int k, int dil, int phases, bool resid) {
+        const ConvPath p = conv_pick(cout, cin, Lc, k, dil, phases, m->pk(w) != nullptr, resid, NPL, false, phases > 1);
+        if (k == 1 && !(p.pre && !p.seg && p.cis == 32)) return false;
+        return p.kernel >= CK_BF16X3_96x128_TM4 && p.kernel <= CK_BF16X3_96x128_6W && cout % 8 == 0 && cin % 8 == 0;
+    };
+    bool prod = bf(m->init_w, m->cfg.dec_dim, m->cfg.dec_latent, L, 7, 1, 1, false);
+    unsigned used = 0;
+    for (int b = 0; b < 4; ++b) {
+        const DecBlockW& Bk = m->blk[b];
+        const int Lo = L * Bk.rate, Co = Bk.cout;
+        const bool tc = bf(Bk.tw, Co, Bk.cin, L, 2, 1, Bk.rate, false);
+        bool c7 = true, c1 = true, fused = false;
+        for (int uu = 0; uu < 3; ++uu) {
+            const ResUnitW& R = Bk.res[uu];
+            fused = fused || resunit_pick(Co, Lo, dils[uu], m->pk(R.c1w) && m->pk(R.c2w) && R.a2, false, NPL).kernel != CK_NONE;
+            c7 = c7 && bf(R.c1w, Co, Co, Lo, 7, dils[uu], 1, false);
+            c1 = c1 && bf(R.c2w, Co, Co, Lo, 1, 1, 1, true);
+        }
+        const bool units = c7 && c1 && !fused;
+        if (((xm >> (2 * b)) & 1) && prod && tc) used |= 1u << (2 * b);
+        if (b < 3 && ((xm >> (2 * b + 1)) & 1) && tc && units) used |= 1u << (2 * b + 1);
+        prod = units;
+        L = Lo;
+    }
+    return used;
+}
 q3_status codec_stack_dev(const q3_model* m, CodecWS& ws, float* cur, int L, hipStream_t st, float** taps, const CodecScope& scope) {
     const int NPL = scope.planes;
     const q3_config& c = m->cfg;
@@ -218,19 +257,30 @@
         for (float* p : pool4) { bool u = false; for (const float* q : used) if (q == p) u = true; if (!u) return p; }
         return nullptr;
     };
+    static const int dils[3] = {1, 3, 9};
+    bool in_pl[5] = {false, false, false, false, false}, k7_pl[4] = {false, false, false, false};
+    {
+        const unsigned used = scope.xplanes ? codec_stack_planes(m, L, NPL) : 0u;
+        for (int b = 0; b < 4; ++b) { in_pl[b] = (used >> (2 * b)) & 1; k7_pl[b] = (used >> (2 * b + 1)) & 1; }
+    }
     float* xact = other({cur});
     {
         ConvArgs a; a.x = cur; a.w = m->init_w; a.wpk = m->pk(m->init_w); a.b = m->init_b; a.cin = LAT; a.cout = Cc; a.L = L; a.k = 7; a.dil = 1; a.planes = NPL;
         a.post_a = m->blk[0].a; a.post_ib = m->blk[0].ib;
-        if (taps && taps[Q3_DEC_INIT]) { float* raw = other({cur, xact}); a.y = raw; a.y2 = xact; HIPC(launch_conv1d(a, st)); Q3C(TAP(Q3_DEC_INIT, raw, (size_t)Cc * L)); }
-        else { a.y = xact; HIPC(launch_conv1d(a, st)); }
-    }
-    static const int dils[3] = {1, 3, 9};
+        const bool tapped = taps && taps[Q3_DEC_INIT];
+        float* raw = tapped ? other({cur, xact}) : nullptr;
+        if (in_pl[0]) { a.y = raw; a.ypl = (uint16_t*)xact; }
+        else if (tapped) { a.y = raw; a.y2 = xact; }
+        else a.y = xact;
+        HIPC(launch_conv1d(a, st));
+        if (tapped) Q3C(TAP(Q3_DEC_INIT, raw, (size_t)Cc * L));
+    }
     for (int b = 0; b < 4; ++b) {
         const DecBlockW& Bk = m->blk[b];
         float* Y = other({xact});
         float* YA = other({xact, Y});
-        HIPC(launch_transconv1d_taps(xact, Bk.tw, Bk.tb, Y, Bk.cin, Bk.cout, L, Bk.rate, 2, nullptr, nullptr, st, Bk.res[0].a1, Bk.res[0].ib1, YA, m->pk(Bk.tw), NPL));
+        HIPC(launch_transconv1d_taps(in_pl[b] ? nullptr : xact, Bk.tw, Bk.tb, Y, Bk.cin, Bk.cout, L, Bk.rate, 2, nullptr, nullptr, st, Bk.res[0].a1, Bk.res[0].ib1,
+                                     k7_pl[b] ? nullptr : YA, m->pk(Bk.tw), NPL, nullptr, in_pl[b] ? (const uint16_t*)xact : nullptr, k7_pl[b] ? (uint16_t*)YA : nullptr));
         L *= Bk.rate; Cc = Bk.cout;
         float* T2 = other({Y, YA});
         for (int uu = 0; uu < 3; ++uu) {
@@ -246,12 +296,13 @@
                 if (e != hipErrorNotSupported) HIPC(e);
             }
             {
-                ConvArgs a; a.x = YA; a.w = R.c1w; a.wpk = m->pk(R.c1w); a.b = R.c1b; a.y = T2; a.cin = Cc; a.cout = Cc; a.L = L; a.k = 7; a.dil = dils[uu]; a.planes = NPL;
+                ConvArgs a; a.x = k7_pl[b] ? nullptr : YA; a.xpl = k7_pl[b] ? (const uint16_t*)YA : nullptr; a.w = R.c1w; a.wpk = m->pk(R.c1w); a.b = R.c1b; a.y = T2; a.cin = Cc; a.cout = Cc; a.L = L; a.k = 7; a.dil = dils[uu]; a.planes = NPL;
                 a.post_a = R.a2; a.post_ib = R.ib2;
                 HIPC(launch_conv1d(a, st));
             }
             {
-                ConvArgs a; a.x = T2; a.w = R.c2w; a.wpk = m->pk(R.c2w); a.b = R.c2b; a.y = Y; a.y2 = YA; a.cin = Cc; a.cout = Cc; a.L = L; a.k = 1; a.dil = 1; a.resid = Y; a.planes = NPL;
+                const bool opl = uu < 2 ? k7_pl[b] : in_pl[b + 1];
+                ConvArgs a; a.x = T2; a.w = R.c2w; a.wpk = m->pk(R.c2w); a.b = R.c2b; a.y = Y; a.y2 = opl ? nullptr : YA; a.ypl = opl ? (uint16_t*)YA : nullptr; a.cin = Cc; a.cout = Cc; a.L = L; a.k = 1; a.dil = 1; a.resid = Y; a.planes = NPL;
                 if (uu < 2) { a.post_a = Bk.res[uu + 1].a1; a.post_ib = Bk.res[uu + 1].ib1; }
                 else if (b < 3) { a.post_a = m->blk[b + 1].a; a.post_ib = m->blk[b + 1].ib; }
                 else { a.post_a = m->fin_a; a.post_ib = m->fin_ib; }
@@ -290,6 +341,13 @@
     return codec_stack_dev(m, ws, cur, L, st, taps, scope);
 }
 
+extern "C" int q3_codec_planes_used(const q3_model* m, int n_frames) {
+    if (!m || !m->finalized || n_frames < 1) return -1;
+    int up = 1; for (int i = 0; i < 2; ++i) up *= m->cfg.dec_up_ratios[i];
+    const CodecScope scope(m);
+    return (int)codec_stack_planes(m, n_frames * up, scope.planes);
+}
+
 extern "C" q3_status q3_decode_codes(q3_model* m, const uint32_t* frames_host, int n_frames, float* pcm_host, float** taps_host) {
     if (!m || !m->finalized) return set_err(Q3_INVALID_ARG, "model not finalized");
     if (n_frames < 0 || (n_frames > 0 && (!frames_host || !pcm_host))) return set_err(Q3_INVALID_ARG, "q3_decode_codes: bad argument");
diff --git a/qwen3_tts_rs_amd/csrc/q3_codec_stream.hip b/qwen3_tts_rs_amd/csrc/q3_codec_stream.hip
--- a/qwen3_tts_rs_amd/csrc/q3_codec_stream.hip
+++ b/qwen3_tts_rs_amd/csrc/q3_codec_stream.hip
@@ -306,7 +306,7 @@
     if (on_dev) HIPC(launch_gather_frames((const uint32_t* const*)D(o_fsrc), ws.frames, N, st));
     else HIPC(q3_hipMemcpy(ws.frames, fhost.data(), fhost.size() * 4, hipMemcpyHostToDevice));
 
-    const CodecScope scope(m);
+    const CodecScope scope(m, false);
     Q3C(codec_front_quant(m, ws, N, st));
     HIPC(launch_copy_cols((const ColCopy*)D(o_xin), Np, Q, 0, 0, st));
     HIPC(launch_copy_cols((const ColCopy*)D(o_hist), 2 * nP, Q, 0, 0, st));
diff --git a/qwen3_tts_rs_amd/csrc/q3_engine.h b/qwen3_tts_rs_amd/csrc/q3_engine.h
--- a/qwen3_tts_rs_amd/csrc/q3_engine.h
+++ b/qwen3_tts_rs_amd/csrc/q3_engine.h
@@ -374,7 +374,7 @@
 Q3_HIDDEN q3_status codec_reserve(const q3_model* m, CodecWS& ws, int T, int Tf = 0);
 Q3_HIDDEN int samples_per_frame(const q3_config& c);
 Q3_HIDDEN q3_status codec_decode_dev(const q3_model* m, CodecWS& ws, int T, hipStream_t st, float** taps, int c0 = 0);
-struct Q3_HIDDEN CodecScope { int planes; explicit CodecScope(const q3_model* m); ~CodecScope(); CodecScope(const CodecScope&) = delete; };
+struct Q3_HIDDEN CodecScope { int planes; bool xplanes; explicit CodecScope(const q3_model* m, bool xplanes = true); ~CodecScope(); CodecScope(const CodecScope&) = delete; };
 using CodecAttnFn = std::function<q3_status(int layer, float* q, float* k, float* v, float* ao)>;
 Q3_HIDDEN q3_status codec_rope_table(const q3_config& c, int n, float* cs_dev, float* sn_dev);
 Q3_HIDDEN q3_status codec_front_quant(const q3_model* m, CodecWS& ws, int T, hipStream_t st);
diff --git a/qwen3_tts_rs_amd/csrc/q3_kernels.h b/qwen3_tts_rs_amd/csrc/q3_kernels.h
--- a/qwen3_tts_rs_amd/csrc/q3_kernels.h
+++ b/qwen3_tts_rs_amd/csrc/q3_kernels.h
@@ -240,7 +240,10 @@
     float* y2 = nullptr;
     const void* wpk = nullptr;
     int planes = 3;
-};
+    const uint16_t* xpl = nullptr;
+    uint16_t* ypl = nullptr;
+};
+inline size_t conv_plane_elems(int C, size_t L) { return (size_t)3 * C * L; }
 hipError_t launch_pack_conv_w(const float* w, void* out, int cout, int cin, int K, hipStream_t st);
 size_t packed_conv_w_bytes(int cout, int cin, int K);
 enum ConvKernel {
@@ -285,7 +288,8 @@
                                    int stride, int taps, const float* snake_a, const float* snake_ib, hipStream_t st,
                                    const float* post_a = nullptr, const float* post_ib = nullptr, float* y2 = nullptr,
                                    const void* wpk = nullptr,
-                                   int planes = 3, int* path = nullptr);
+                                   int planes = 3, int* path = nullptr,
+                                   const uint16_t* xpl = nullptr, uint16_t* ypl = nullptr);
 void transconv_phase_weights(const float* w, int cin, int cout, int k, int stride, float* out);
 hipError_t launch_snake_tables(const float* alpha, const float* beta, float* a, float* ib, int C, hipStream_t st);
 hipError_t launch_dwconv7(const float* x, const float* w, const float* b, float* y, int C, int L, hipStream_t st);
diff --git a/qwen3_tts_rs_amd/csrc/q3_kernels_codec.hip b/qwen3_tts_rs_amd/csrc/q3_kernels_codec.hip
--- a/qwen3_tts_rs_amd/csrc/q3_kernels_codec.hip
+++ b/qwen3_tts_rs_amd/csrc/q3_kernels_codec.hip
@@ -48,6 +48,8 @@
     size_t wpk_phase_stride;
     int phases;
     int planes;
+    const uint16_t* xpl;
+    uint16_t* ypl;
 };
 
 __global__ __launch_bounds__(256) void k_conv1d(ConvDev a) {
@@ -293,7 +295,7 @@
 
 __host__ __device__ __forceinline__ bool conv_segmented(int k, int cin) { return k == 1 && (cin & 511) == 0; }
 
-template <int K, int CO_M, int T_M, int WCO, int WT, bool PRE = false, bool SEG = false, int CIS = 32, int NP = 3>
+template <int K, int CO_M, int T_M, int WCO, int WT, bool PRE = false, bool SEG = false, int CIS = 32, int NP = 3, bool XPL = false, bool YPL = false>
 __global__ __launch_bounds__(64 * WCO * WT, (CO_M == 2 || T_M >= 8) ? 2 : 3) void k_conv_bf16x3(ConvDev a) {
     constexpr int NT = 64 * WCO * WT;
     constexpr int CO_WG = 32 * CO_M * WCO, T_WG = 32 * T_M * WT;
@@ -371,6 +373,36 @@
         constexpr int NCHK = (T_WG + (K - 1) * 9 + 63) / 64, NBF = (NOCT * NCHK + WCO * WT - 1) / (WCO * WT);
         constexpr int NB = NBF < 1 ? 1 : (NBF > 4 ? 4 : NBF);
         const int n_items = NOCT * ((W + 63) >> 6);
+        if constexpr (XPL) {
+            const size_t xps = (size_t)a.L * a.cin;
+            for (int c0 = wave; c0 < n_items; c0 += NB * WCO * WT) {
+                cu32x4_t pv[NB][NP];
+                bool ok[NB];
+#pragma unroll
+                for (int i = 0; i < NB; ++i) {
+                    const int c = c0 + i * WCO * WT;
+                    const int q = c % NOCT, tt = (c / NOCT) * 64 + lane;
+                    const int ca = ci0 + q * 8, t = t0 - halo + tt;
+                    ok[i] = c < n_items && tt < W && ca < a.cin && t >= 0 && t < a.L;
+                    const int cc = ca < a.cin ? ca : a.cin - 8, tc = t < 0 ? 0 : (t < a.L ? t : a.L - 1);
+                    const uint16_t* xr = a.xpl + ((size_t)(cc >> 3) * a.L + tc) * 8;
+#pragma unroll
+                    for (int pl = 0; pl < NP; ++pl) pv[i][pl] = *reinterpret_cast<const cu32x4_t*>(xr + pl * xps);
+                }
+#pragma unroll
+                for (int i = 0; i < NB; ++i) {
+                    const int c = c0 + i * WCO * WT;
+                    if (c >= n_items) break;
+                    const int q = c % NOCT, tt = (c / NOCT) * 64 + lane;
+                    if (tt < W) {
+                        const cu32x4_t z = {0u, 0u, 0u, 0u};
+                        unsigned char* row = smem + (unsigned)tt * XPB + q * 16;
+#pragma unroll
+                        for (int pl = 0; pl < NP; ++pl) *reinterpret_cast<cu32x4_t*>(row + pl * plane) = ok[i] ? pv[i][pl] : z;
+                    }
+                }
+            }
+        } else
         for (int c0 = wave; c0 < n_items; c0 += NB * WCO * WT) {
             float v[NB][8];
             bool ok[NB];
@@ -462,6 +494,51 @@
         for (int i = 0; i < SM; ++i)
 #pragma unroll
             for (int j = 0; j < SN; ++j) acc[i][j] = tot[i][j];
+    }
+    if constexpr (YPL) {
+        const size_t yps = (size_t)a.oL * a.cout;
+#pragma unroll
+        for (int cm = 0; cm < CO_M; ++cm)
+#pragma unroll
+            for (int tm = 0; tm < T_M; ++tm) {
+                const int t = t0 + wt * (32 * T_M) + tm * 32 + li;
+                const bool tok = t < a.L;
+                const size_t to = (size_t)(tok ? t : 0) * a.ostride + ooff;
+                float rs[16];
+                if (a.resid) {
+#pragma unroll
+                    for (int reg = 0; reg < 16; ++reg) {
+                        const int o = co0 + cm * 32 + (reg & 3) + 8 * (reg >> 2) + 4 * lk;
+                        rs[reg] = a.resid[(size_t)(o < a.cout ? o : 0) * a.oL + to];
+                    }
+                }
+#pragma unroll
+                for (int g = 0; g < 4; ++g) {
+                    const int ob = co0 + cm * 32 + 8 * g + 4 * lk;
+                    float va[4];
+#pragma unroll
+                    for (int j = 0; j < 4; ++j) {
+                        const int reg = 4 * g + j, pi = ob + j - by * CO_WG;
+                        const float bias = s_prm[0][pi], sc = s_prm[1][pi], pa = s_prm[2][pi], pib = s_prm[3][pi];
+                        float v = acc[cm][tm][reg] + bias;
+                        v = conv_act(v, a.act);
+                        if (a.scale) v = v * sc;
+                        if (a.resid) v = rs[reg] + v;
+                        if (a.act == 2) v = fminf(fmaxf(v, -1.0f), 1.0f);
+                        va[j] = snake_f(v, pa, pib);
+                        if (a.y && tok && ob < a.cout) a.y[(size_t)(ob + j) * a.oL + to] = v;
+                    }
+                    if (tok && ob < a.cout) {
+                        uint32_t h0, m0, l0, h1, m1, l1;
+                        split3_pair(va[0], va[1], h0, m0, l0); split3_pair(va[2], va[3], h1, m1, l1);
+                        uint16_t* pr = a.ypl + ((size_t)(ob >> 3) * a.oL + to) * 8 + (ob & 7);
+                        *reinterpret_cast<uint2*>(pr) = make_uint2(h0, h1);
+                        *reinterpret_cast<uint2*>(pr + yps) = make_uint2(m0, m1);
+                        if (NP == 3) *reinterpret_cast<uint2*>(pr + 2 * yps) = make_uint2(l0, l1);
+                    }
+                }
+            }
+        return;
     }
 #pragma unroll
     for (int cm = 0; cm < CO_M; ++cm) {
@@ -826,6 +903,21 @@
     ConvDev ap = a; ap.phases = phases;
     const bool segm = p.seg;
     const dim3 blk(64 * WCO * WT);
+    if (a.xpl || a.ypl) {
+#define Q3_CVP(P, X, Y) hipLaunchKernelGGL((k_conv_bf16x3<K, CO_M, T_M, WCO, WT, P, false, 32, NP, X, Y>), grid, blk, lds, st, ap)
+        if constexpr (K == 2 || K == 7) {
+            if (a.xpl && a.ypl) { if constexpr (K == 2) Q3_CVP(false, true, true); else return hipErrorInvalidValue; }
+            else if (a.xpl) Q3_CVP(false, true, false);
+            else Q3_CVP(false, false, true);
+            return hipGetLastError();
+        } else if constexpr (K1 && CO_M == 1) {
+            if (a.xpl || !p.pre || p.seg || p.cis != 32) return hipErrorInvalidValue;
+            Q3_CVP(true, false, true);
+            return hipGetLastError();
+        }
+#undef Q3_CVP
+        return hipErrorInvalidValue;
+    }
     if constexpr (K1) {
         const bool pre = p.pre;
 #define Q3_CV(P, S, C) hipLaunchKernelGGL((k_conv_bf16x3<K, CO_M, T_M, WCO, WT, P, S, C, NP>), grid, blk, lds, st, ap)
@@ -999,6 +1091,9 @@
 }
 
 static hipError_t launch_conv_path(const ConvPath& p, const ConvDev& a, int phases, hipStream_t st) {
+    if ((a.xpl || a.ypl) && (p.kernel < CK_BF16X3_96x128_TM4 || p.kernel > CK_BF16X3_96x128_6W)) return hipErrorInvalidValue;
+    if ((a.ypl && (!a.post_a || a.y2 || a.cout % 8)) || (a.xpl && (a.snake_a || a.cin % 8)) || ((uintptr_t)a.xpl & 15) || ((uintptr_t)a.ypl & 15))
+        return hipErrorInvalidValue;
     switch (p.kernel) {
         case CK_NONE: return p.refusal != hipSuccess ? p.refusal : hipErrorInvalidValue;
         case CK_OUT1_V4: hipLaunchKernelGGL(k_conv_out1_v4, dim3((a.L / 4 + 255) / 256), dim3(256), 0, st, a); break;
@@ -1044,21 +1139,22 @@
     a.x = c.x; a.w = c.w; a.b = c.b; a.y = c.y; a.cin = c.cin; a.cout = c.cout; a.L = c.L; a.k = c.k; a.dil = c.dil;
     a.snake_a = c.snake_a; a.snake_ib = c.snake_b; a.resid = c.resid; a.scale = c.scale; a.act = c.act;
     a.ostride = 1; a.ooff = 0; a.oL = c.L; a.w_phase_stride = 0; a.ooff_phase = 0;
-    a.post_a = c.post_a; a.post_ib = c.post_ib; a.y2 = c.y2;
+    a.post_a = c.post_a; a.post_ib = c.post_ib; a.y2 = c.y2; a.xpl = c.xpl; a.ypl = c.ypl;
     a.wpk = c.wpk; a.wpk_phase_stride = 0; a.planes = conv_planes(c.planes);
     return launch_conv_path(p, a, 1, st);
 }
 
 hipError_t launch_transconv1d_taps(const float* x, const float* wp, const float* b, float* y, int cin, int cout, int L,
                                    int stride, int taps, const float* snake_a, const float* snake_ib, hipStream_t st,
-                                   const float* post_a, const float* post_ib, float* y2, const void* wpk, int planes, int* path) {
+                                   const float* post_a, const float* post_ib, float* y2, const void* wpk, int planes, int* path,
+                                   const uint16_t* xpl, uint16_t* ypl) {
     const ConvPath p = conv_pick(cout, cin, L, taps, 1, stride, wpk != nullptr, false, planes, false, true);
     if (path) *path = conv_path_code(p);
     if (p.kernel == CK_NONE) return p.refusal;
     ConvDev a{};
     a.planes = conv_planes(planes);
     a.wpk = wpk; a.wpk_phase_stride = packed_conv_w_bytes(cout, cin, taps) / 16;
-    a.post_a = post_a; a.post_ib = post_ib; a.y2 = y2;
+    a.post_a = post_a; a.post_ib = post_ib; a.y2 = y2; a.xpl = xpl; a.ypl = ypl;
     a.x = x; a.w = wp; a.b = b; a.y = y; a.cin = cin; a.cout = cout; a.L = L; a.k = taps; a.dil = 1;
     a.snake_a = snake_a; a.snake_ib = snake_ib; a.resid = nullptr; a.scale = nullptr; a.act = 0;
     a.ostride = stride; a.ooff = 0; a.oL = L * stride;
diff --git a/qwen3_tts_rs_amd/csrc/q3_testapi.hip b/qwen3_tts_rs_amd/csrc/q3_testapi.hip
--- a/qwen3_tts_rs_amd/csrc/q3_testapi.hip
+++ b/qwen3_tts_rs_amd/csrc/q3_testapi.hip
@@ -589,8 +589,10 @@
 }
 extern "C" const char* q3_conv_path_name(int code) { return conv_path_name(code); }
 
-extern "C" q3_status q3_conv_ex(int device, const q3_conv_ex_args* p) {
+static q3_status conv_ex_run(int device, const q3_conv_ex_args* p, const uint16_t* xpl_h, uint16_t* ypl_h) {
     if (!p || !p->x || !p->w || !p->y) return set_err(Q3_INVALID_ARG, "q3_conv_ex: null argument");
+    if ((xpl_h || ypl_h) && (p->kind == 2 || p->cin % 8 || p->cout % 8)) return set_err(Q3_INVALID_ARG, "q3_conv_planes_ex: plane tensors belong to kinds 0 and 1 with channels in octets");
+    if (ypl_h && (p->y2 || !p->post_a)) return set_err(Q3_INVALID_ARG, "q3_conv_planes_ex: y_planes replaces y2 and needs the post snake pair");
     if (p->path) *p->path = 0;
     const int kind = p->kind, cin = p->cin, cout = p->cout, L = p->L, k = p->k, dil = p->dil;
     if (kind < 0 || kind > 2) return set_err(Q3_INVALID_ARG, "q3_conv_ex: kind 0..2");
@@ -642,6 +644,10 @@
     HIPC(pool.alloc(&y, yn)); HIPC(q3_hipMemcpy(y, p->y, yn * 4, hipMemcpyHostToDevice));
     if (p->y2) { HIPC(pool.alloc(&y2, yn)); HIPC(q3_hipMemcpy(y2, p->y2, yn * 4, hipMemcpyHostToDevice)); }
     float* yr = y + p->y_front; float* y2r = y2 ? y2 + p->y_front : nullptr;
+    uint16_t *xpl = nullptr, *ypl = nullptr;
+    const size_t xpn = conv_plane_elems(cin, (size_t)L), ypn = conv_plane_elems(cout, (size_t)L * stride);
+    if (xpl_h) { HIPC(pool.alloc(&xpl, xpn)); HIPC(q3_hipMemcpy(xpl, xpl_h, xpn * 2, hipMemcpyHostToDevice)); }
+    if (ypl_h) { HIPC(pool.alloc(&ypl, ypn)); HIPC(q3_hipMemcpy(ypl, ypl_h, ypn * 2, hipMemcpyHostToDevice)); }
     if (p->packed) {
         const int pk = kind == 1 ? taps : k;
         if (cout % 32 || cin % 16 || pk < 1) return set_err(Q3_UNSUPPORTED, "q3_conv_ex: cout %d / cin %d cannot be packed (cout %% 32, cin %% 16)", cout, cin);
@@ -660,10 +666,11 @@
         ConvArgs a;
         a.x = x; a.w = w; a.b = b; a.y = yr; a.cin = cin; a.cout = cout; a.L = L; a.k = k; a.dil = dil;
         a.snake_a = sa; a.snake_b = sb; a.resid = p->resid_in_place ? yr : res; a.scale = scale; a.act = p->act;
-        a.post_a = pa; a.post_ib = pb; a.y2 = y2r; a.wpk = wpk; a.planes = p->planes;
+        a.post_a = pa; a.post_ib = pb; a.y2 = y2r; a.wpk = wpk; a.planes = p->planes; a.xpl = xpl; a.ypl = ypl;
+        if (xpl) a.x = nullptr;
         e = launch_conv1d(a, 0, &path);
     } else if (kind == 1) {
-        e = launch_transconv1d_taps(x, w, b, yr, cin, cout, L, stride, taps, sa, sb, 0, pa, pb, y2r, wpk, p->planes, &path);
+        e = launch_transconv1d_taps(xpl ? nullptr : x, w, b, yr, cin, cout, L, stride, taps, sa, sb, 0, pa, pb, y2r, wpk, p->planes, &path, xpl, ypl);
     } else {
         ResUnitArgs r{};
         r.xa = x; r.y = yr; r.ya = p->y2_is_x ? x : y2r; r.w1pk = wpk; r.w2pk = w2pk; r.b1 = b; r.b2 = b2;
@@ -680,7 +687,12 @@
     HIPC(q3_hipDeviceSynchronize());
     HIPC(q3_hipMemcpy(p->y, y, yn * 4, hipMemcpyDeviceToHost));
     if (y2) HIPC(q3_hipMemcpy(p->y2, y2, yn * 4, hipMemcpyDeviceToHost));
-    return Q3_OK;
+    if (ypl) HIPC(q3_hipMemcpy(ypl_h, ypl, ypn * 2, hipMemcpyDeviceToHost));
+    return Q3_OK;
+}
+extern "C" q3_status q3_conv_ex(int device, const q3_conv_ex_args* p) { return conv_ex_run(device, p, nullptr, nullptr); }
+extern "C" q3_status q3_conv_planes_ex(int device, const q3_conv_ex_args* p, const uint16_t* x_planes, uint16_t* y_planes) {
+    return conv_ex_run(device, p, x_planes, y_planes);
 }
 
 static q3_status check_cl_out(const char* who, const void* x, const void* w, const void* y, int C, int L, int y_front, int y_elems) {
```

Result: no change. 2843 (median of 6 runs) (+0.1%).
